# bryanboateng/animating-gaussian-splats

Measured on AMD Instinct MI355X. Metric: Msplats/sec fwd+bwd @1080p (1M gauss), higher is better.
Workload: dtype f32; 1 GPU; C3: 1000000 Gaussians, SH3, 1920x1080, 27-camera rig, 5 view(s)/GPU/step, fwd+bwd; gaussians=1000000, image=1920x1080, sh_degree=3, parallelism=camera-dp1, streams_per_gpu=3, submission=one host thread per stream, means2D=one fresh zero leaf per render (shared.py:38-41)

## Files before the change

animating-gaussian-splats_amd/csrc/gsr_api.hip:

```cpp
#include <hip/hip_runtime.h>

#include <atomic>
#include <cstdarg>
#include <cstdio>
#include <cstdlib>
#include <cmath>
#include <cstring>
#include <chrono>
#include <condition_variable>
#include <thread>
#include <map>
#include <memory>
#include <unordered_map>
#include <mutex>
#include <string>
#include <vector>

#include "../../include/gsr.h"
#include "gsr_common.h"
#include "gsr_internal.h"
#include "gsr_host.h"

using namespace gsr;

// ... 16 lines not shown
    hipEvent_t e = nullptr;
    if (hipEventCreateWithFlags(&e, hipEventDisableSystemFence) != hipSuccess) return nullptr;
    return e;
}

}

int gsr::fail(int code, const char *fmt, ...) {
    char buf[512];
    va_list ap;
    va_start(ap, fmt);
    vsnprintf(buf, sizeof(buf), fmt, ap);
    va_end(ap);
    g_err = buf;
    return code;
}

gsr::Phase::Phase(hipStream_t s_, const char *n, bool on) : s(s_), name(n) {
    if (!on || !g_prof_on) return;
    std::lock_guard<std::mutex> lk(g_prof_mu);
    if (!g_prof_sel.empty() && g_prof_sel.find("," + std::string(n) + ",") == std::string::npos) return;
    a = ev_get(); b = ev_get();
    if (a) (void)hipEventRecord(a, s);
}
gsr::Phase::~Phase() {
    if (!a || !b) return;
    (void)hipEventRecord(b, s);
    std::lock_guard<std::mutex> lk(g_prof_mu);
    g_prof.push_back({name, a, b});
}

gsr::HostPhase::HostPhase(const char *n) : name(n), t0(hclock::now()), on(g_prof_on) {}
gsr::HostPhase::~HostPhase() {
    if (!on) return;
    const double ms = std::chrono::duration<double, std::milli>(hclock::now() - t0).count();
    std::lock_guard<std::mutex> lk(g_prof_mu);
    g_host_ms[name] += ms;
    g_host_n[name] += 1;
}

namespace {

std::vector<hipEvent_t> g_gw_evpool;
struct GradEvent {
    hipEvent_t ev = nullptr;
    ~GradEvent() { if (ev) g_gw_evpool.push_back(ev); }
};
struct GradWriter { hipStream_t s = nullptr; std::shared_ptr<GradEvent> ev; };
std::mutex g_gw_mu;
std::unordered_map<const void *, GradWriter> g_gw;
constexpr size_t kGradPruneAt = 1024;

hipError_t no_launch() { return hipSuccess; }

template <typename Launch>
hipError_t ordered_grad_write(const void *const *keys, int nkeys, hipStream_t s, Launch launch) {
    std::lock_guard<std::mutex> lk(g_gw_mu);
    const GradEvent *waited[16];
    int nw = 0;
    for (int k = 0; k < nkeys; ++k) {
        if (!keys[k]) continue;
        auto it = g_gw.find(keys[k]);
        if (it == g_gw.end() || it->second.s == s) continue;
        const GradEvent *e = it->second.ev.get();
        bool seen = false;
        for (int j = 0; j < nw; ++j) seen = seen || waited[j] == e;
        if (seen) continue;
        const hipError_t r = hipStreamWaitEvent(s, e->ev, 0);
        if (r != hipSuccess) return r;
        if (nw < 16) waited[nw++] = e;
    }
    auto ev = std::make_shared<GradEvent>();
    hipError_t r = hipSuccess;
    if (!g_gw_evpool.empty()) { ev->ev = g_gw_evpool.back(); g_gw_evpool.pop_back(); }
    else r = hipEventCreateWithFlags(&ev->ev, hipEventDisableTiming);
    if (r != hipSuccess) { ev->ev = nullptr; return r; }
    r = launch();
    if (r != hipSuccess) return r;
    r = hipEventRecord(ev->ev, s);
    if (r != hipSuccess) return r;
    for (int k = 0; k < nkeys; ++k)
        if (keys[k]) g_gw[keys[k]] = GradWriter{s, ev};
    if (g_gw.size() > kGradPruneAt) {
        for (auto it = g_gw.begin(); it != g_gw.end();)
            it = hipEventQuery(it->second.ev->ev) == hipSuccess ? g_gw.erase(it) : std::next(it);
    }
    return hipSuccess;
}

struct HostWord { uint32_t *h = nullptr; uint32_t *d = nullptr; };
HostWord pinned_word() {
    thread_local HostWord w;
    if (!w.h) {
        uint32_t *h = nullptr;
        if (hipHostMalloc((void **)&h, 4 * kHostWords, hipHostMallocMapped | hipHostMallocCoherent) != hipSuccess) return w;
        uint32_t *d = nullptr;
        if (hipHostGetDevicePointer((void **)&d, h, 0) != hipSuccess) { (void)hipHostFree(h); return w; }
        w.h = h; w.d = d;
    }
    return w;
}

constexpr uint32_t kNoValue = 0xFFFFFFFFu;

int check_common(const gsr_camera *cam, const gsr_gaussians *g, bool need_opacity) {
    if (!cam || !g) return fail(GSR_ERR_ARG, "null camera or gaussians");
    if (g->P < 0) return fail(GSR_ERR_ARG, "P must be >= 0");
    if (cam->image_width <= 0 || cam->image_height <= 0)
        return fail(GSR_ERR_ARG, "image size must be positive (got %dx%d)", cam->image_width, cam->image_height);
    const int gx = div_up(cam->image_width, kTileW), gy = div_up(cam->image_height, kTileH);
    if (gx > 65535 || gy > 65535) return fail(GSR_ERR_UNSUPPORTED, "tile grid too large");
    if (g->activations & ~(GSR_ACT_SIGMOID_OPACITY | GSR_ACT_EXP_SCALES | GSR_ACT_NORMALIZE_ROTATIONS))
        return fail(GSR_ERR_ARG, "unknown activation bits 0x%x", g->activations);
    if (g->P == 0) return GSR_OK;
    if (!g->means3D || (need_opacity && !g->opacities))
        return fail(GSR_ERR_ARG, "means3D and opacities are required");
    if ((g->shs == nullptr) == (g->colors_precomp == nullptr))
        return fail(GSR_ERR_ARG, "Please provide excatly one of either SHs or precomputed colors!");
    const bool sr = g->scales && g->rotations;
    if (sr == (g->cov3D_precomp != nullptr) || ((g->scales != nullptr) != (g->rotations != nullptr)))
        return fail(GSR_ERR_ARG, "Please provide exactly one of either scale/rotation pair or precomputed 3D covariance!");
    if (g->shs && (g->sh_coeffs <= 0 || (g->sh_degree + 1) * (g->sh_degree + 1) > g->sh_coeffs || g->sh_degree > 3 || g->sh_degree < 0))
        return fail(GSR_ERR_ARG, "invalid SH configuration: degree %d with %d coefficients", g->sh_degree, g->sh_coeffs);
    if (!cam->viewmatrix || !cam->projmatrix || !cam->bg || (g->shs && !cam->campos))
        return fail(GSR_ERR_ARG, "camera matrices / bg / campos missing");
    return GSR_OK;
}

std::atomic<int> g_exact{[] {
    const char *e = getenv("GSR_EXACT_THRESHOLDS");
    return (e && e[0] == '0') ? 0 : 1;
}()};

void fill_common(ViewIn &v, const gsr_camera *cam, const gsr_gaussians *g) {
    memset(&v, 0, sizeof(v));
    v.P = g->P; v.D = g->sh_degree; v.M = g->shs ? g->sh_coeffs : 0;
    v.W = cam->image_width; v.H = cam->image_height;
    v.gx = div_up(v.W, kTileW); v.gy = div_up(v.H, kTileH);
    v.scale_modifier = g->scale_modifier;
    v.act = g->activations;
    v.tan_fovx = cam->tan_fovx; v.tan_fovy = cam->tan_fovy;
    v.focal_y = v.H / (2.0f * v.tan_fovy);
    v.focal_x = v.W / (2.0f * v.tan_fovx);
    v.means3D = g->means3D; v.scales = g->scales; v.rotations = g->rotations; v.opacities = g->opacities;
    v.shs = g->shs; v.colors_precomp = g->colors_precomp; v.cov3D_precomp = g->cov3D_precomp;
    v.viewmatrix = cam->viewmatrix; v.projmatrix = cam->projmatrix; v.campos = cam->campos; v.bg = cam->bg;
    const bool vz = !cam->viewmatrix_stride[0] && !cam->viewmatrix_stride[1];
    const bool pz = !cam->projmatrix_stride[0] && !cam->projmatrix_stride[1];
    v.cs.v0 = vz ? 4 : cam->viewmatrix_stride[0]; v.cs.v1 = vz ? 1 : cam->viewmatrix_stride[1];
    v.cs.p0 = pz ? 4 : cam->projmatrix_stride[0]; v.cs.p1 = pz ? 1 : cam->projmatrix_stride[1];
    v.cs.c0 = cam->campos_stride ? cam->campos_stride : 1;
}

template <typename A>
void carve_saved(A &a, char *geom, char *img) {
    const GeomLayout G(a.v.P);
    a.rec = (float4 *)(geom + G.rec); a.rect = (uint2 *)(geom + G.rect);
    a.goff = (uint32_t *)(geom + G.goff); a.clampm = (uint8_t *)(geom + G.clampm);
    const ImageLayout L(a.v.W, a.v.H, a.v.P);
    a.ranges = (uint2 *)(img + L.ranges); a.pix_end = (float4 *)(img + L.pix_end);
    a.n_contrib = (uint32_t *)(img + L.n_contrib); a.tile_maxc = (uint32_t *)(img + L.tile_maxc);
    a.tile_flag = (uint32_t *)(img + L.tile_flag); a.near_rec = (float4 *)(img + L.near_rec);
    a.seg_off = (uint32_t *)(img + L.seg_off); a.meta = (uint32_t *)(img + L.meta);
    a.items_ws = (uint32_t *)(img + L.items_ws);
}
void carve_forward(FwdArgs &a, char *geom, char *img) {
    carve_saved(a, geom, img);
    const GeomLayout G(a.v.P);
    a.depth = (float *)(geom + G.depth); a.tiles = (uint32_t *)(geom + G.tiles);
    const ImageLayout L(a.v.W, a.v.H, a.v.P);
    a.tile_order_f = (uint32_t *)(img + L.tile_order_f); a.sort_lists = (uint32_t *)(img + L.sort_lists);
    a.tile_count = (uint32_t *)(img + L.tile_count); a.tile_cursor = (uint32_t *)(img + L.tile_cursor);
    a.block_sums = (uint32_t *)(img + L.block_sums); a.block_off = (uint32_t *)(img + L.block_off);
    a.chunk_off = (uint32_t *)(img + L.chunk_off); a.scan_ws = (uint32_t *)(img + L.scan_ws);
    a.tile_rank = (uint32_t *)(img + L.tile_rank); a.tsat_list = (uint32_t *)(img + L.tsat_list);
}
template <typename A>
void carve_binning(A &a, char *bin, const BinningLayout &L) {
    a.point_list = (uint32_t *)(bin + L.point_list); a.slot_emit = (uint32_t *)(bin + L.slot_emit);
    a.seg_state = (float4 *)(bin + L.seg_state);
}

struct BinRegions {
    BinningLayout arrays;
    size_t items, tmp, total;
    BinRegions(int K, int P, int T, bool with_items, bool with_merge) : arrays(K, P) {
        items = arrays.total;
        tmp = items + (with_items ? bwd_items_bytes(K, T) : 0);
        total = tmp + (with_merge ? sizeof(uint4) * (size_t)K : 0);
    }
};

int enqueue_post_scan(FwdArgs a, char *bin, int layout, uint32_t n_mid, uint32_t n_vlong, uint32_t max_n,
                      bool prepare_backward, int T, hipStream_t s, const uint32_t *spec_ok, bool phases) {
    const BinRegions R(layout, a.v.P, T, prepare_backward, n_vlong != 0);
    carve_binning(a, bin, R.arrays);
    a.pairs = (uint4 *)(bin + R.arrays.pairs);
    a.spec_ok = spec_ok;
    uint4 *tmp = n_vlong ? (uint4 *)(bin + R.tmp) : nullptr;
    uint2 *items = (uint2 *)(bin + R.items);
    { Phase ph(s, "bin_emit", phases); HIP_TRY(launch_bin_emit(a, spec_ok ? 0 : layout, s)); }
    { Phase ph(s, "tile_sort", phases); HIP_TRY(launch_tile_sort(a, n_mid, n_vlong, max_n, tmp, s)); }
    { Phase ph(s, "render_fwd", phases); HIP_TRY(launch_render_fwd(a, s)); }
    if (prepare_backward) {
        Phase ph(s, "bwd_items", phases);
        HIP_TRY(launch_bwd_items_raw(layout, T, a.v.P, a.ranges, a.tile_maxc, a.tile_flag, items, a.items_ws, s, spec_ok));
    }
    return GSR_OK;
}

enum class KWait { published, stream_error, drained };
KWait wait_published(const uint32_t *word, hipStream_t s, hipError_t *err) {
    auto last = hclock::now();
    while (__atomic_load_n(word, __ATOMIC_ACQUIRE) == kNoValue) {
        __builtin_ia32_pause();
        if (hclock::now() - last > std::chrono::microseconds(500)) {
            last = hclock::now();
            const hipError_t q = hipStreamQuery(s);
            if (q == hipErrorNotReady) continue;
            *err = q;
            if (q != hipSuccess) return KWait::stream_error;
            return __atomic_load_n(word, __ATOMIC_ACQUIRE) == kNoValue ? KWait::drained : KWait::published;
        }
    }
    return KWait::published;
}

}

extern "C" {

const char *gsr_last_error(void) { return g_err.c_str(); }

int gsr_set_exact_thresholds(int on) { return g_exact.exchange(on ? 1 : 0); }
int gsr_abi_version(void) { return GSR_ABI_VERSION; }

size_t gsr_geom_bytes(int P) { return GeomLayout(P < 0 ? 0 : P).total; }
size_t gsr_image_bytes(int W, int H, int P) { return ImageLayout(W, H, P < 0 ? 0 : P).total; }
size_t gsr_binning_bytes(int K, int P) { return BinningLayout(K, P).total; }
size_t gsr_backward_items_bytes(int K, int W, int H) {
    return bwd_items_bytes(K < 0 ? 0 : K, div_up(W < 0 ? 0 : W, kTileW) * div_up(H < 0 ? 0 : H, kTileH));
}
size_t gsr_sums_bytes(int P) { return align256(sizeof(float) * (kPartial * (size_t)(P < 0 ? 0 : P) + 1)); }
size_t gsr_scratch_bytes(int K, int W, int H) {
    return ScratchLayout(K, div_up(W < 0 ? 0 : W, kTileW) * div_up(H < 0 ? 0 : H, kTileH)).total;
}

void *gsr_prealloc_alloc(void *ctx, int which, size_t bytes) {
    gsr_prealloc *pa = (gsr_prealloc *)ctx;
    if (!pa) return nullptr;
    if (which >= 0 && which < 5 && pa->ptr[which] && pa->bytes[which] >= bytes && !(pa->used & (1 << which))) {
        pa->used |= 1 << which;
        return pa->ptr[which];
    }
    return pa->fallback ? pa->fallback(pa->fallback_ctx, which, bytes) : nullptr;
}

int gsr_buffer_offsets(int P, int W, int H, int K, size_t *out, int max_out) {
    const GeomLayout g(P);
    const ImageLayout im(W, H, P);
    const BinningLayout b(K, P);
    const size_t v[16] = {g.depth, g.rec, g.rect, g.tiles, g.goff,
                          im.ranges, im.pix_end, im.n_contrib, im.tile_maxc,
                          b.pairs, b.point_list, b.slot_emit, im.seg_off, b.seg_state, im.tile_flag,
                          im.items_ws + sizeof(uint32_t) * kTSatCtr};
    int n = 0;
    for (; n < 16 && n < max_out; ++n) out[n] = v[n];
    return n;
}

}

namespace {
struct SpecKey {
    int dev, P, W, H;
    bool operator==(const SpecKey &o) const { return dev == o.dev && P == o.P && W == o.W && H == o.H; }
};
struct SpecKeyHash {
    size_t operator()(const SpecKey &k) const {
        return ((size_t)k.dev * 1000003u) ^ ((size_t)k.P * 2654435761u) ^ ((size_t)k.W << 20) ^ (size_t)k.H;
    }
};
constexpr int kSpecWindow = 16;
constexpr size_t kSpecKeys = 64;
struct SpecStat {
    uint32_t recent[kSpecWindow] = {};
    uint32_t recent_mid[kSpecWindow] = {};
    int n = 0;
    bool long_lists = false;
    uint64_t used = 0;
    uint32_t window_max() const {
        uint32_t m = 0;
        for (int k = 0; k < std::min(n, kSpecWindow); ++k) m = std::max(m, recent[k]);
        return m;
    }
};
std::mutex g_spec_mu;
std::unordered_map<SpecKey, SpecStat, SpecKeyHash> g_spec;
uint64_t g_spec_clock = 0;
int g_spec_hits = 0, g_spec_misses = 0, g_async_calls = 0;

uint32_t spec_capacity(const SpecKey &key, uint32_t *sort_blocks = nullptr) {
    std::lock_guard<std::mutex> lk(g_spec_mu);
    auto it = g_spec.find(key);
    if (it == g_spec.end() || it->second.long_lists) return 0;
    it->second.used = ++g_spec_clock;
// ... 102 lines not shown
    for (int k = 0; k < kAsyncSlots; ++k) {
        const int j = (g_slot_next + k) % kAsyncSlots;
        if (!g_slot_busy[j]) {
            g_slot_busy[j] = 1;
            g_slot_next = (j + 1) % kAsyncSlots;
            return j;
        }
    }
    return -1;
}

void async_classify(AsyncFwd &f) {
    const uint32_t *w = slot_h(f.slot);
    f.K = __atomic_load_n(w, __ATOMIC_ACQUIRE);
    const uint32_t n_vlong = __atomic_load_n(w + 2, __ATOMIC_ACQUIRE), n_mid = __atomic_load_n(w + 1, __ATOMIC_ACQUIRE);
    if (f.K <= f.cap && n_vlong == 0) {
        f.state = 1;
        f.layout = (int)f.cap;
        f.bin = f.spec_bin;
        spec_record(f.key, f.K, false, +1, n_mid);
    } else {
        f.state = 2;
        spec_record(f.key, f.K, n_vlong > 0, -1, n_mid);
    }
}

void async_reap(std::unordered_map<uint64_t, std::shared_ptr<AsyncFwd>>::iterator it) {
    AsyncFwd &f = *it->second;
    if (f.own) {
        int cur = 0;
        (void)hipGetDevice(&cur);
        if (cur != f.dev) (void)hipSetDevice(f.dev);
        (void)hipFreeAsync(f.own, f.s);
        if (cur != f.dev) (void)hipSetDevice(cur);
        f.own = nullptr;
    }
    if (f.ev_scan) g_as_evpool.push_back(f.ev_scan);
    f.ev_scan = nullptr;
    if (f.slot >= 0 && !f.err_reported && __atomic_load_n(slot_h(f.slot) + kGateErrWord, __ATOMIC_ACQUIRE) == f.seq)
        g_async_err = "an asynchronous forward's gate timed out (seq " + std::to_string(f.seq) + "), its outputs were not final";
    if (f.slot >= 0) g_slot_busy[f.slot] = 0;
    g_as.erase(it);
}

int async_redo(AsyncFwd &f, hipStream_t H) {
    (void)hipSetDevice(f.dev);
    if (!H) return fail(GSR_ERR_HIP, "asynchronous forward: no resolver stream on device %d", f.dev);
    HIP_TRY(hipStreamWaitEvent(H, f.ev_scan, 0));
    const uint32_t *w = slot_h(f.slot);
    const uint32_t K = f.K, n_mid = w[1], n_vlong = w[2], max_n = w[3];
    const size_t bytes = BinRegions((int)K, f.a.v.P, f.T, f.prep, n_vlong != 0).total;
    void *bin = nullptr;
    if (hipMallocAsync(&bin, bytes, H) != hipSuccess || !bin)
        return fail(GSR_ERR_ALLOC, "asynchronous forward: hipMallocAsync of %zu bytes failed", bytes);
    f.own = bin;
    const int rc = enqueue_post_scan(f.a, (char *)bin, (int)K, n_mid, n_vlong, max_n, f.prep, f.T, H, nullptr, false);
    if (rc) return rc;
    HIP_TRY(hipStreamSynchronize(H));
    f.bin = bin;
    f.layout = (int)K;
    return GSR_OK;
}

void resolver_main() {
    std::unique_lock<std::mutex> lk(g_as_mu);
    for (;;) {
        for (auto it = g_as.begin(); it != g_as.end();) {
            const AsyncFwd &f = *it->second;
            if (f.released && (f.state == 1 || f.state == 3 || f.state == -1)) async_reap(it++);
            else ++it;
        }
        std::shared_ptr<AsyncFwd> next;
        for (auto &kv : g_as)
            if ((kv.second->state == 0 || kv.second->state == 2) && (!next || kv.second->id < next->id)) next = kv.second;
        if (!next) {
            if (g_resolver_stop) break;
            g_as_wake.wait(lk);
            continue;
        }
        if (next->state == 0) {
            hipEvent_t ev = next->ev_scan;
            const int dev = next->dev;
            lk.unlock();
            (void)hipSetDevice(dev);
            const hipError_t r = hipEventSynchronize(ev);
            lk.lock();
            if (next->state == 0) {
                if (r != hipSuccess || __atomic_load_n(slot_h(next->slot), __ATOMIC_ACQUIRE) == kNoValue) {
                    next->state = -1;
                    next->err = r != hipSuccess ? std::string("stream error before num_rendered was published: ") +
                                                      hipGetErrorString(r)
                                                : std::string("num_rendered was not published");
                    __atomic_store_n(slot_h(next->slot) + kGateWord, next->seq, __ATOMIC_RELEASE);
                } else {
                    async_classify(*next);
                }
                g_as_done.notify_all();
            }
            continue;
        }
        hipStream_t H = g_resolver_streams.count(next->dev) ? g_resolver_streams[next->dev] : nullptr;
        lk.unlock();
        const int rc = async_redo(*next, H);
        const std::string msg = rc ? g_err : std::string();
        if (g_hold_next_redo_ms > 0) {
            std::this_thread::sleep_for(std::chrono::milliseconds(g_hold_next_redo_ms));
            g_hold_next_redo_ms = 0;
        }
        __atomic_store_n(slot_h(next->slot) + kGateWord, next->seq, __ATOMIC_RELEASE);
        lk.lock();
        next->state = rc ? -1 : 3;
        if (rc) { next->err = msg; g_async_err = "asynchronous forward redo failed: " + msg; }
        g_as_done.notify_all();
    }
}

}

extern "C" size_t gsr_spec_binning_bytes(int P, int W, int H, int prepare_backward) {
    if (P <= 0 || W <= 0 || H <= 0) return 0;
    int dev = 0;
    (void)hipGetDevice(&dev);
    const uint32_t cap = spec_capacity(SpecKey{dev, P, W, H});
    if (!cap) return 0;
    return BinRegions((int)cap, P, div_up(W, kTileW) * div_up(H, kTileH), prepare_backward != 0, false).total;
}

namespace {
int forward_impl(const gsr_camera *cam, const gsr_gaussians *g, gsr_alloc_fn alloc, void *alloc_ctx,
                 float *out_color, float *out_depth, int *out_radii, gsr_forward_info *info, int mode,
                 void *stream) {
    HostPhase host_total("host_forward");
    int rc = check_common(cam, g, true);
    if (rc) return rc;
    if (!alloc || !out_color || !out_depth || !info || (g->P > 0 && !out_radii))
        return fail(GSR_ERR_ARG, "gsr_forward: missing output or allocator");
    {
        std::lock_guard<std::mutex> lk(g_as_mu);
        if (!g_async_err.empty()) return fail(GSR_ERR_HIP, "%s", g_async_err.c_str());
    }
    hipStream_t s = (hipStream_t)stream;
    FwdArgs a;
    memset(&a, 0, sizeof(a));
    fill_common(a.v, cam, g);
    const int P = a.v.P, T = a.v.gx * a.v.gy;
    const bool prep = g->prepare_backward != 0;
    a.exact = g_exact.load(std::memory_order_relaxed);
    a.radii = out_radii; a.out_color = out_color; a.out_depth = out_depth;
    char *geom = (char *)alloc(alloc_ctx, GSR_BUF_GEOM, GeomLayout(P).total);
    char *img = (char *)alloc(alloc_ctx, GSR_BUF_IMAGE, ImageLayout(a.v.W, a.v.H, P).total);
    if (!geom || !img) return fail(GSR_ERR_ALLOC, "allocation callback failed (geom/image)");
    carve_forward(a, geom, img);
    *info = gsr_forward_info{};
    if (P == 0) {
        const size_t npix = (size_t)a.v.W * a.v.H;
        HIP_TRY(launch_zero(out_color, 3 * npix, s));
        HIP_TRY(launch_zero(out_depth, npix, s));
        char *bin = (char *)alloc(alloc_ctx, GSR_BUF_BINNING, BinningLayout(0, 0).total);
        if (!bin) return fail(GSR_ERR_ALLOC, "allocation callback failed (binning)");
        return GSR_OK;
    }
    int dev = 0;
    (void)hipGetDevice(&dev);
    const SpecKey key{dev, P, a.v.W, a.v.H};
    uint32_t sort_blocks = kSpecSortBlocks;
    const uint32_t cap = mode ? spec_capacity(key, &sort_blocks) : 0u;
    a.spec_cap = cap;
    a.spec_sort_blocks = sort_blocks;
    std::shared_ptr<AsyncFwd> af;
    uint32_t *words_h = nullptr, *words_d = nullptr;
    if (mode == 2 && cap) {
        std::lock_guard<std::mutex> lk(g_as_mu);
        if (async_init() && resolver_stream(dev)) {
            const int slot = slot_acquire();
            if (slot >= 0) {
                af = std::make_shared<AsyncFwd>();
                af->slot = slot; af->seq = ++g_as_seq;
                words_h = slot_h(slot); words_d = slot_d(slot);
                __atomic_store_n(words_h + kGateErrWord, 0u, __ATOMIC_RELAXED);
            }
        }
    }
    struct SlotGuard {
        std::shared_ptr<AsyncFwd> *f;
        ~SlotGuard() {
            if (!*f || (*f)->id) return;
            std::lock_guard<std::mutex> lk(g_as_mu);
            g_slot_busy[(*f)->slot] = 0;
            if ((*f)->ev_scan) g_as_evpool.push_back((*f)->ev_scan);
        }
    } slot_guard{&af};
    if (!af) {
        HostWord hw = pinned_word();
        if (!hw.h) return fail(GSR_ERR_HIP, "hipHostMalloc(mapped) failed");
        words_h = hw.h; words_d = hw.d;
    }
    __atomic_store_n(words_h, kNoValue, __ATOMIC_SEQ_CST);
    { Phase ph(s, "preprocess"); HIP_TRY(launch_preprocess(a, s)); }
    { Phase ph(s, "bin_count"); HIP_TRY(launch_bin_count(a, s)); }
    { Phase ph(s, "bin_scan"); HIP_TRY(launch_bin_scan(a, words_d, s)); }
    if (af) {
        {
            std::lock_guard<std::mutex> lk(g_as_mu);
            if (!g_as_evpool.empty()) { af->ev_scan = g_as_evpool.back(); g_as_evpool.pop_back(); }
        }
        if (!af->ev_scan) HIP_TRY(hipEventCreateWithFlags(&af->ev_scan, hipEventDisableTiming | hipEventBlockingSync));
        HIP_TRY(hipEventRecord(af->ev_scan, s));
    }
    char *spec_bin = nullptr;
    if (cap) {
        spec_bin = (char *)alloc(alloc_ctx, GSR_BUF_BINNING, BinRegions((int)cap, P, T, prep, false).total);
        if (!spec_bin) return fail(GSR_ERR_ALLOC, "allocation callback failed (binning, capacity %u)", cap);
        FwdArgs sa = a;
        if (af) {
            sa.gate = words_d + kGateWord; sa.gate_seq = af->seq;
            sa.gate_err = words_d + kGateErrWord; sa.gate_timeout = g_gate_timeout;
        }
        rc = enqueue_post_scan(sa, spec_bin, (int)cap, 0, 0, 0, prep, T, s, a.meta + 1, true);
        if (rc) return rc;
    }
    if (af) {
        std::lock_guard<std::mutex> lk(g_as_mu);
        af->id = g_as_next_id++;
        af->dev = dev; af->s = s; af->cap = cap; af->T = T; af->key = key;
        af->prep = prep; af->a = a; af->spec_bin = spec_bin;
        g_as[af->id] = af;
        info->num_rendered = -1; info->binning_layout = (int)cap;
        info->speculated = 1; info->pending = af->id;
        { std::lock_guard<std::mutex> lk2(g_spec_mu); ++g_async_calls; }
        g_as_wake.notify_one();
        return GSR_OK;
    }
    {
        HostPhase hp("host_wait_K");
        hipError_t q = hipSuccess;
        const KWait w = wait_published(words_h, s, &q);
        if (w == KWait::stream_error) return fail(GSR_ERR_HIP, "stream error while waiting for num_rendered: %s", hipGetErrorString(q));
        if (w == KWait::drained) return fail(GSR_ERR_HIP, "num_rendered was not published");
    }
    const uint32_t K = __atomic_load_n(words_h, __ATOMIC_ACQUIRE);
    if (K > 0x7FFFFFFFu) return fail(GSR_ERR_UNSUPPORTED, "num_rendered overflow");
    info->num_rendered = (int)K;
    const uint32_t n_mid = __atomic_load_n(words_h + 1, __ATOMIC_ACQUIRE);
    const uint32_t n_vlong = __atomic_load_n(words_h + 2, __ATOMIC_ACQUIRE);
    const uint32_t max_n = __atomic_load_n(words_h + 3, __ATOMIC_ACQUIRE);
    if (cap && K <= cap && n_vlong == 0) {
        info->binning_layout = (int)cap;
        info->speculated = 1;
        spec_record(key, K, false, +1, n_mid);
        return GSR_OK;
    }
    char *bin = (char *)alloc(alloc_ctx, GSR_BUF_BINNING, BinRegions((int)K, P, T, prep, n_vlong != 0).total);
    if (!bin) return fail(GSR_ERR_ALLOC, "allocation callback failed (binning, K=%u)", K);
    rc = enqueue_post_scan(a, bin, (int)K, n_mid, n_vlong, max_n, prep, T, s, nullptr, true);
    if (rc) return rc;
    info->binning_layout = (int)K;
    spec_record(key, K, n_vlong > 0, cap ? -1 : 0, n_mid);
    return GSR_OK;
}
}

extern "C" {

int gsr_forward(const gsr_camera *cam, const gsr_gaussians *g, gsr_alloc_fn alloc, void *alloc_ctx,
                float *out_color, float *out_depth, int *out_radii, int *out_num_rendered,
                void *stream) {
    if (!out_num_rendered) return fail(GSR_ERR_ARG, "gsr_forward: missing output or allocator");
    *out_num_rendered = 0;
    gsr_forward_info info;
    const int rc = forward_impl(cam, g, alloc, alloc_ctx, out_color, out_depth, out_radii, &info, 0, stream);
    *out_num_rendered = info.num_rendered;
    return rc;
}

int gsr_forward_info_call(const gsr_camera *cam, const gsr_gaussians *g, gsr_alloc_fn alloc, void *alloc_ctx,
                          float *out_color, float *out_depth, int *out_radii, int speculate, gsr_forward_info *info,
                          void *stream) {
    if (!info) return fail(GSR_ERR_ARG, "gsr_forward_info_call: null info");
    return forward_impl(cam, g, alloc, alloc_ctx, out_color, out_depth, out_radii, info, speculate ? 1 : 0, stream);
}

int gsr_forward_async(const gsr_camera *cam, const gsr_gaussians *g, gsr_alloc_fn alloc, void *alloc_ctx,
                      float *out_color, float *out_depth, int *out_radii, gsr_forward_info *info, void *stream) {
    if (!info) return fail(GSR_ERR_ARG, "gsr_forward_async: null info");
    return forward_impl(cam, g, alloc, alloc_ctx, out_color, out_depth, out_radii, info, 2, stream);
}

int gsr_forward_resolve(unsigned long long handle, gsr_forward_resolution *out) {
    if (!out) return fail(GSR_ERR_ARG, "gsr_forward_resolve: null output");
    HostPhase hp("host_wait_K");
    std::unique_lock<std::mutex> lk(g_as_mu);
    auto it = g_as.find(handle);
    if (it == g_as.end()) return fail(GSR_ERR_ARG, "gsr_forward_resolve: unknown or released forward %llu", handle);
    std::shared_ptr<AsyncFwd> f = it->second;
    while (f->state == 0 || f->state == 2) {
        if (f->state == 0) {
            if (__atomic_load_n(slot_h(f->slot), __ATOMIC_ACQUIRE) != kNoValue) {
                async_classify(*f);
                if (f->state == 2) g_as_wake.notify_one();
                continue;
            }
            lk.unlock();
            hipError_t q = hipSuccess;
            const KWait w = wait_published(slot_h(f->slot), f->s, &q);
            lk.lock();
            if (w != KWait::published && f->state == 0) {
                f->state = -1;
                f->err = w == KWait::drained ? std::string("num_rendered was not published")
                                             : std::string("stream error: ") + hipGetErrorString(q);
                __atomic_store_n(slot_h(f->slot) + kGateWord, f->seq, __ATOMIC_RELEASE);
            }
            continue;
        }
        g_as_done.wait(lk);
    }
    if (f->state < 0) return fail(GSR_ERR_HIP, "asynchronous forward %llu failed: %s", handle, f->err.c_str());
    if (__atomic_load_n(slot_h(f->slot) + kGateErrWord, __ATOMIC_ACQUIRE) == f->seq) {
        f->err_reported = true;
        return fail(GSR_ERR_HIP, "asynchronous forward %llu: its gate timed out before the redo opened it; the outputs "
                    "the caller used after the forward were not final", handle);
    }
    out->num_rendered = (int)f->K;
    out->binning_layout = f->layout;
    out->binning = f->bin;
    out->redone = f->state == 3;
    return GSR_OK;
}

int gsr_forward_query(unsigned long long handle) {
    std::lock_guard<std::mutex> lk(g_as_mu);
    auto it = g_as.find(handle);
    if (it == g_as.end()) return -1;
    AsyncFwd &f = *it->second;
    if (f.state == 0 && __atomic_load_n(slot_h(f.slot), __ATOMIC_ACQUIRE) != kNoValue) {
        async_classify(f);
        if (f.state == 2) g_as_wake.notify_one();
    }
    return (f.state == 1 || f.state == 3 || f.state == -1) ? 1 : 0;
}

int gsr_forward_release(unsigned long long handle) {
    std::lock_guard<std::mutex> lk(g_as_mu);
    auto it = g_as.find(handle);
    if (it == g_as.end()) return GSR_OK;
    it->second->released = true;
    const int st = it->second->state;
    if (st == 1 || st == 3 || st == -1) async_reap(it);
    else g_as_wake.notify_one();
    return GSR_OK;
}

int gsr_async_shutdown(void) {
    std::thread t;
    {
        std::lock_guard<std::mutex> lk(g_as_mu);
        if (!g_resolver_started) return GSR_OK;
        g_resolver_stop = true;
        g_resolver_started = false;
        t = std::move(g_resolver);
    }
    g_as_wake.notify_all();
    if (t.joinable()) t.join();
    return GSR_OK;
}

int gsr_async_stats(int *calls, int *pending) {
    {
        std::lock_guard<std::mutex> lk(g_spec_mu);
        if (calls) *calls = g_async_calls;
    }
    std::lock_guard<std::mutex> lk(g_as_mu);
    if (pending) *pending = (int)g_as.size();
    return GSR_OK;
}

int gsr_spec_stats(int *hits, int *misses, int reset) {
    std::lock_guard<std::mutex> lk(g_spec_mu);
    if (hits) *hits = g_spec_hits;
    if (misses) *misses = g_spec_misses;
    if (reset) { g_spec.clear(); g_spec_hits = g_spec_misses = g_async_calls = 0; }
    return GSR_OK;
}

int gsr_debug_async_fault(int hold_next_redo_ms, int gate_timeout_ms, int clear) {
    std::lock_guard<std::mutex> lk(g_as_mu);
    g_hold_next_redo_ms = hold_next_redo_ms > 0 ? hold_next_redo_ms : 0;
    g_gate_timeout = gate_timeout_ms > 0 ? (uint64_t)gate_timeout_ms * 100000ull : kGateTimeoutTicks;
    if (clear) g_async_err.clear();
    return GSR_OK;
}

int gsr_spec_keys(void) {
    std::lock_guard<std::mutex> lk(g_spec_mu);
    return (int)g_spec.size();
}

}


namespace {
int backward_render(const gsr_camera *cam, const gsr_gaussians *g, const int *radii, int num_rendered,
                    const void *geom, const void *binning, const void *image, const float *dL_dcolor,
                    gsr_alloc_fn alloc, void *alloc_ctx, hipStream_t s, BwdArgs &a, bool sums = false) {
    if (!geom || !binning || !image || !dL_dcolor || !radii || !alloc)
        return fail(GSR_ERR_ARG, "gsr_backward: missing saved buffers / dL_dcolor / allocator");
    const bool spec = num_rendered < 0;
    if (spec && g->binning_layout <= 0) return fail(GSR_ERR_ARG, "num_rendered < 0 without the forward's binning_layout");
    memset(&a, 0, sizeof(a));
    fill_common(a.v, cam, g);
    const int P = a.v.P, T = a.v.gx * a.v.gy;
    const int layout = g->binning_layout > 0 ? g->binning_layout : num_rendered;
    if (layout < num_rendered) return fail(GSR_ERR_ARG, "binning_layout %d < num_rendered %d", layout, num_rendered);
    if (spec) num_rendered = layout;
    a.K = num_rendered;
    a.radii = radii;
// ... 180 lines not shown
```

animating-gaussian-splats_amd/csrc/gsr_bind.cpp:

```cpp
#include <torch/extension.h>
#include <ATen/hip/HIPContext.h>
#include <c10/hip/HIPCachingAllocator.h>
#include <c10/hip/HIPGuard.h>

#include <map>
#include <stdexcept>
#include <string>
#include <vector>

#include "../../include/gsr.h"

namespace py = pybind11;

namespace {

struct Fns {
    decltype(&gsr_forward_info_call) forward_info_call = nullptr;
    decltype(&gsr_forward_async) forward_async = nullptr;
    decltype(&gsr_backward_render) backward_render = nullptr;
    decltype(&gsr_backward_gaussians) backward_gaussians = nullptr;
    decltype(&gsr_backward) backward = nullptr;
    decltype(&gsr_prealloc_alloc) prealloc_alloc = nullptr;
    decltype(&gsr_spec_binning_bytes) spec_binning_bytes = nullptr;
    decltype(&gsr_geom_bytes) geom_bytes = nullptr;
    decltype(&gsr_image_bytes) image_bytes = nullptr;
    decltype(&gsr_scratch_bytes) scratch_bytes = nullptr;
    decltype(&gsr_sums_bytes) sums_bytes = nullptr;
    decltype(&gsr_last_error) last_error = nullptr;
} F;

template <typename T>
void take(const std::map<std::string, int64_t> &a, const char *name, T &dst) {
    auto it = a.find(name);
    if (it == a.end() || !it->second) throw std::runtime_error(std::string("gsr_bind: missing ") + name);
    dst = reinterpret_cast<T>(it->second);
}

void set_functions(const std::map<std::string, int64_t> &a) {
    take(a, "gsr_forward_info_call", F.forward_info_call);
    take(a, "gsr_forward_async", F.forward_async);
    take(a, "gsr_backward_render", F.backward_render);
    take(a, "gsr_backward_gaussians", F.backward_gaussians);
    take(a, "gsr_backward", F.backward);
    take(a, "gsr_prealloc_alloc", F.prealloc_alloc);
    take(a, "gsr_spec_binning_bytes", F.spec_binning_bytes);
    take(a, "gsr_geom_bytes", F.geom_bytes);
    take(a, "gsr_image_bytes", F.image_bytes);
    take(a, "gsr_scratch_bytes", F.scratch_bytes);
    take(a, "gsr_sums_bytes", F.sums_bytes);
    take(a, "gsr_last_error", F.last_error);
}

void check(int rc) {
    if (rc != 0) throw std::runtime_error("libgsr error " + std::to_string(rc) + ": " + F.last_error());
}

bool present(const at::Tensor &t) { return t.defined() && t.numel() > 0; }

const char *torch_name(at::ScalarType t) {
    switch (t) {
        case at::kDouble: return "torch.float64";
        case at::kHalf: return "torch.float16";
        case at::kBFloat16: return "torch.bfloat16";
        case at::kInt: return "torch.int32";
        case at::kLong: return "torch.int64";
        case at::kShort: return "torch.int16";
        case at::kByte: return "torch.uint8";
        case at::kChar: return "torch.int8";
        case at::kBool: return "torch.bool";
        default: return c10::toString(t);
    }
}

const float *fptr(const at::Tensor &t, std::vector<at::Tensor> &keep) {
    if (!present(t)) return nullptr;
    if (!t.is_cuda()) throw std::runtime_error("diff_gaussian_rasterization: tensors must be on the GPU (no CPU path)");
    at::Tensor c = t.contiguous();
    if (c.scalar_type() != at::kFloat)
        throw std::runtime_error(std::string("diff_gaussian_rasterization: expected float32, got ") +
                                 torch_name(c.scalar_type()));
    keep.push_back(c);
    return c.data_ptr<float>();
}

const float *mat16(const at::Tensor &m0, int stride[2], std::vector<at::Tensor> &keep) {
    if (m0.numel() != 16) throw std::runtime_error("viewmatrix/projmatrix must hold 16 floats");
    at::Tensor m = m0.scalar_type() == at::kFloat ? m0 : m0.to(at::kFloat);
    const auto sz = m.sizes();
    const bool plain = (m.dim() == 2 && sz[0] == 4 && sz[1] == 4) || (m.dim() == 3 && sz[0] == 1 && sz[1] == 4 && sz[2] == 4);
    if (!plain) m = m.reshape({4, 4});
    stride[0] = (int)m.stride(-2);
    stride[1] = (int)m.stride(-1);
    if (!m.is_cuda()) throw std::runtime_error("diff_gaussian_rasterization: tensors must be on the GPU (no CPU path)");
    keep.push_back(m);
    return m.data_ptr<float>();
}

gsr_camera camera(const at::Tensor &vm, const at::Tensor &pm, double tanfovx, double tanfovy, int H, int W,
                  const at::Tensor &campos, const at::Tensor &bg, bool prefiltered, std::vector<at::Tensor> &keep) {
    gsr_camera c;
    memset(&c, 0, sizeof(c));
    c.image_width = W;
    c.image_height = H;
    c.tan_fovx = (float)tanfovx;
    c.tan_fovy = (float)tanfovy;
    c.viewmatrix = mat16(vm, c.viewmatrix_stride, keep);
    c.projmatrix = mat16(pm, c.projmatrix_stride, keep);
    at::Tensor b = (bg.scalar_type() == at::kFloat && bg.is_contiguous()) ? bg : bg.contiguous().to(at::kFloat);
    c.bg = fptr(b, keep);
    if (present(campos)) {
        at::Tensor cp = (campos.scalar_type() == at::kFloat && campos.dim() == 1) ? campos : campos.reshape({-1}).to(at::kFloat);
        if (!cp.is_cuda()) throw std::runtime_error("diff_gaussian_rasterization: tensors must be on the GPU (no CPU path)");
        keep.push_back(cp);
        c.campos = cp.data_ptr<float>();
        c.campos_stride = (int)cp.stride(0);
    }
    c.prefiltered = prefiltered ? 1 : 0;
    return c;
}

gsr_gaussians gaussians(const at::Tensor &means3D, const at::Tensor &sh, int degree, const at::Tensor &colors,
                        const at::Tensor &opacity, const at::Tensor &scales, const at::Tensor &rotations,
                        double scale_modifier, const at::Tensor &cov3D, int activations, bool prep, int layout,
                        std::vector<at::Tensor> &keep) {
    if (means3D.dim() != 2 || means3D.size(1) != 3) throw std::runtime_error("means3D must have dimensions (num_points, 3)");
    gsr_gaussians g;
    memset(&g, 0, sizeof(g));
    g.P = (int)means3D.size(0);
    g.sh_degree = degree;
    g.sh_coeffs = present(sh) ? (int)sh.size(1) : 0;
    g.scale_modifier = (float)scale_modifier;
    g.means3D = fptr(means3D, keep);
    g.shs = fptr(sh, keep);
    g.colors_precomp = fptr(colors, keep);
    g.opacities = fptr(opacity, keep);
    g.scales = fptr(scales, keep);
    g.rotations = fptr(rotations, keep);
    g.cov3D_precomp = fptr(cov3D, keep);
    g.activations = activations;
    g.prepare_backward = prep ? 1 : 0;
    g.binning_layout = layout;
    return g;
}

struct PreAlloc {
    gsr_prealloc pa;
    at::Device dev;
    struct Given { at::Tensor base; int64_t off, bytes; };
    std::map<int, Given> given;
    std::map<int, at::Tensor> fallback;
    explicit PreAlloc(at::Device d) : dev(d) { memset(&pa, 0, sizeof(pa)); }
    void group(std::initializer_list<std::pair<int, size_t>> g, bool on) {
        if (!on) return;
        int64_t total = 0;
        std::vector<std::tuple<int, int64_t, int64_t>> offs;
        for (auto &e : g) {
            offs.emplace_back(e.first, total, (int64_t)e.second);
            total += ((int64_t)e.second + 255) & ~(int64_t)255;
        }
        if (total == 0) return;
        at::Tensor buf = at::empty({total}, at::TensorOptions().dtype(at::kByte).device(dev));
        char *base = (char *)buf.data_ptr();
        for (auto &[w, o, n] : offs)
            if (n > 0) {
                given[w] = Given{buf, o, n};
                pa.ptr[w] = base + o;
                pa.bytes[w] = (size_t)n;
            }
    }
    static void *fallback_fn(void *ctx, int which, size_t bytes) {
        auto *self = static_cast<PreAlloc *>(ctx);
        try {
            at::Tensor t = at::empty({(int64_t)std::max<size_t>(bytes, 1)}, at::TensorOptions().dtype(at::kByte).device(self->dev));
            self->fallback[which] = t;
            return t.data_ptr();
        } catch (...) {
            return nullptr;
        }
    }
    void arm() {
        pa.fallback = &PreAlloc::fallback_fn;
        pa.fallback_ctx = this;
    }
    py::tuple result() const {
        py::list taken, fb;
        for (auto &[w, g] : given)
            if ((pa.used >> w) & 1) taken.append(py::make_tuple(w, g.base, g.off, g.bytes));
        for (auto &[w, t] : fallback) fb.append(py::make_tuple(w, t));
        return py::make_tuple(taken, fb);
    }
};

void *raw_stream(at::Device dev) { return (void *)c10::hip::getCurrentHIPStream(dev.index()).stream(); }

py::tuple forward(const at::Tensor &bg, const at::Tensor &means3D, const at::Tensor &colors, const at::Tensor &opacity,
                  const at::Tensor &scales, const at::Tensor &rotations, double scale_modifier, const at::Tensor &cov3D,
                  const at::Tensor &viewmatrix, const at::Tensor &projmatrix, double tanfovx, double tanfovy, int H, int W,
                  const at::Tensor &sh, int degree, const at::Tensor &campos, bool prefiltered, int activations,
                  bool prepare_backward, bool speculate, bool nonblocking, bool prealloc) {
    std::vector<at::Tensor> keep;
    gsr_gaussians g = gaussians(means3D, sh, degree, colors, opacity, scales, rotations, scale_modifier, cov3D,
                                activations, prepare_backward, 0, keep);
    gsr_camera cam = camera(viewmatrix, projmatrix, tanfovx, tanfovy, H, W, campos, bg, prefiltered, keep);
    const at::Device dev = means3D.device();
    const int P = g.P;
    auto f32 = at::TensorOptions().dtype(at::kFloat).device(dev);
    at::Tensor color = at::empty({3, H, W}, f32), depth = at::empty({1, H, W}, f32);
    at::Tensor radii = at::empty({P}, at::TensorOptions().dtype(at::kInt).device(dev));
    c10::hip::HIPGuard guard(dev.index());
    const size_t spec = (speculate || nonblocking) && P ? F.spec_binning_bytes(P, W, H, prepare_backward ? 1 : 0) : 0;
    PreAlloc pa(dev);
    pa.group({{GSR_BUF_GEOM, F.geom_bytes(P)}, {GSR_BUF_IMAGE, F.image_bytes(W, H, P)}}, prealloc);
    pa.group({{GSR_BUF_BINNING, spec}}, prealloc);
    pa.arm();
    gsr_forward_info fi;
    memset(&fi, 0, sizeof(fi));
    void *s = raw_stream(dev);
    int rc;
    {
        py::gil_scoped_release nogil;
        rc = nonblocking ? F.forward_async(&cam, &g, F.prealloc_alloc, &pa.pa, color.data_ptr<float>(),
                                           depth.data_ptr<float>(), P ? radii.data_ptr<int>() : nullptr, &fi, s)
                         : F.forward_info_call(&cam, &g, F.prealloc_alloc, &pa.pa, color.data_ptr<float>(),
                                               depth.data_ptr<float>(), P ? radii.data_ptr<int>() : nullptr,
                                               speculate ? 1 : 0, &fi, s);
    }
    check(rc);
    return py::make_tuple(fi.num_rendered, fi.binning_layout, fi.speculated, (unsigned long long)fi.pending,
                          (int64_t)(intptr_t)fi.aux_stream, color, radii, depth, pa.result());
}

py::tuple backward_render(const at::Tensor &bg, const at::Tensor &means3D, const at::Tensor &radii,
                          const at::Tensor &colors, const at::Tensor &scales, const at::Tensor &rotations,
                          double scale_modifier, const at::Tensor &cov3D, const at::Tensor &viewmatrix,
                          const at::Tensor &projmatrix, double tanfovx, double tanfovy, const at::Tensor &dL_dcolor,
                          const at::Tensor &sh, int degree, const at::Tensor &campos, int64_t geom, int R,
                          int64_t binning, int64_t image, int activations, bool prepare_backward, int binning_layout,
                          bool prealloc) {
    std::vector<at::Tensor> keep;
    gsr_gaussians g = gaussians(means3D, sh, degree, colors, at::Tensor(), scales, rotations, scale_modifier, cov3D,
                                activations, prepare_backward, binning_layout, keep);
    const int H = (int)dL_dcolor.size(-2), W = (int)dL_dcolor.size(-1);
    gsr_camera cam = camera(viewmatrix, projmatrix, tanfovx, tanfovy, H, W, campos, bg, false, keep);
    const at::Device dev = means3D.device();
    if (g.P == 0)
        return py::make_tuple(at::empty({1}, at::TensorOptions().dtype(at::kByte).device(dev)),
                              py::make_tuple(py::list(), py::list()));
    at::Tensor dpix = dL_dcolor.contiguous().to(at::kFloat);
    c10::hip::HIPGuard guard(dev.index());
    PreAlloc pa(dev);
    pa.group({{GSR_BUF_SCRATCH, F.scratch_bytes(R >= 0 ? R : binning_layout, W, H)}}, prealloc);
    pa.group({{GSR_BUF_SUMS, F.sums_bytes(g.P)}}, prealloc);
    pa.arm();
    void *s = raw_stream(dev);
    int rc;
    {
        py::gil_scoped_release nogil;
        rc = F.backward_render(&cam, &g, radii.data_ptr<int>(), R, (const void *)geom, (const void *)binning,
                               (const void *)image, dpix.data_ptr<float>(), F.prealloc_alloc, &pa.pa, s);
    }
    check(rc);
    at::Tensor sums;
    if (auto it = pa.fallback.find(GSR_BUF_SUMS); it != pa.fallback.end()) sums = it->second;
    else {
        auto &gv = pa.given.at(GSR_BUF_SUMS);
        sums = gv.base.narrow(0, gv.off, gv.bytes);
    }
    return py::make_tuple(sums, pa.result());
}

void fill_grads(gsr_grads &gr, const std::vector<c10::optional<at::Tensor>> &outs, int acc_bits) {
    memset(&gr, 0, sizeof(gr));
    float **slot[8] = {&gr.dL_dmeans2D, &gr.dL_dcolors, &gr.dL_dopacity, &gr.dL_dmeans3D,
                       &gr.dL_dcov3D, &gr.dL_dsh, &gr.dL_dscales, &gr.dL_drotations};
    for (int k = 0; k < 8 && k < (int)outs.size(); ++k)
        if (outs[k].has_value() && present(*outs[k])) *slot[k] = outs[k]->data_ptr<float>();
    gr.accumulate = acc_bits;
}

void backward(const at::Tensor &bg, const at::Tensor &means3D, const at::Tensor &radii, const at::Tensor &colors,
              const at::Tensor &scales, const at::Tensor &rotations, double scale_modifier, const at::Tensor &cov3D,
              const at::Tensor &viewmatrix, const at::Tensor &projmatrix, double tanfovx, double tanfovy,
              const at::Tensor &dL_dcolor, const at::Tensor &sh, int degree, const at::Tensor &campos, int64_t geom,
              int R, int64_t binning, int64_t image, int activations, bool prepare_backward, int binning_layout,
              const std::vector<c10::optional<at::Tensor>> &outs, int acc_bits, bool prealloc) {
    std::vector<at::Tensor> keep;
    gsr_gaussians g = gaussians(means3D, sh, degree, colors, at::Tensor(), scales, rotations, scale_modifier, cov3D,
                                activations, prepare_backward, binning_layout, keep);
    const int H = (int)dL_dcolor.size(-2), W = (int)dL_dcolor.size(-1);
    gsr_camera cam = camera(viewmatrix, projmatrix, tanfovx, tanfovy, H, W, campos, bg, false, keep);
    if (g.P == 0) return;
    const at::Device dev = means3D.device();
    at::Tensor dpix = dL_dcolor.contiguous().to(at::kFloat);
    c10::hip::HIPGuard guard(dev.index());
    PreAlloc pa(dev);
    pa.group({{GSR_BUF_SCRATCH, F.scratch_bytes(R, W, H)}}, prealloc);
    pa.arm();
    gsr_grads gr;
    fill_grads(gr, outs, acc_bits);
    void *s = raw_stream(dev);
    int rc;
    {
        py::gil_scoped_release nogil;
        rc = F.backward(&cam, &g, radii.data_ptr<int>(), R, (const void *)geom, (const void *)binning,
                        (const void *)image, dpix.data_ptr<float>(), nullptr, F.prealloc_alloc, &pa.pa, &gr, s);
    }
    check(rc);
}

void record(const at::Tensor &t, const c10::hip::HIPStream &s) {
    if (t.defined() && t.is_cuda() && t.storage().data_ptr().get())
        c10::hip::HIPCachingAllocator::recordStream(t.storage().data_ptr(), s);
}

std::string dev_str(const at::Device &d) { return d.str(); }

void backward_views(const py::list &views, const at::Tensor &means3D, const at::Tensor &colors,
                    const at::Tensor &scales, const at::Tensor &rotations, double scale_modifier, const at::Tensor &cov3D,
                    const at::Tensor &sh, int degree, int activations, const std::vector<c10::optional<at::Tensor>> &outs,
                    int acc_bits) {
    std::vector<at::Tensor> keep;
    gsr_gaussians g = gaussians(means3D, sh, degree, colors, at::Tensor(), scales, rotations, scale_modifier, cov3D,
                                activations, false, 0, keep);
    const int P = g.P;
    const int nv = (int)views.size();
    if (P == 0 || nv == 0) return;
    const at::Device dev = means3D.device();
    c10::hip::HIPGuard guard(dev.index());
    const c10::hip::HIPStream cs = c10::hip::getCurrentHIPStream(dev.index());
    std::vector<gsr_camera> cams(nv);
    std::vector<gsr_view_grad> vg(nv);
    for (int k = 0; k < nv; ++k) {
        const py::dict v = views[k].cast<py::dict>();
        cams[k] = camera(v["viewmatrix"].cast<at::Tensor>(), v["projmatrix"].cast<at::Tensor>(),
                         v["tanfovx"].cast<double>(), v["tanfovy"].cast<double>(), v["image_height"].cast<int>(),
                         v["image_width"].cast<int>(),
                         v["campos"].is_none() ? at::Tensor() : v["campos"].cast<at::Tensor>(),
                         v["bg"].cast<at::Tensor>(), false, keep);
        float *m2p = nullptr;
        if (v.contains("means2D_grad") && !v["means2D_grad"].is_none()) {
            const at::Tensor m2 = v["means2D_grad"].cast<at::Tensor>();
            if (m2.dim() != 2 || m2.size(0) != P || m2.size(1) != 3 || m2.scalar_type() != at::kFloat ||
                !m2.is_contiguous() || m2.device() != dev)
                throw std::runtime_error("views[" + std::to_string(k) + "]['means2D_grad']: expected a contiguous float32 (" +
                                         std::to_string(P) + ", 3) tensor on " + dev_str(dev));
            record(m2, cs);
            m2p = m2.data_ptr<float>();
        }
        const at::Tensor radii = v["radii"].cast<at::Tensor>(), scratch = v["scratch"].cast<at::Tensor>();
        record(radii, cs);
        record(scratch, cs);
        if (v.contains("keep"))
            for (auto h : v["keep"]) record(h.cast<at::Tensor>(), cs);
        const py::object gb = v["geomBuffer"];
        const void *geom;
        if (py::isinstance<py::int_>(gb)) geom = (const void *)gb.cast<int64_t>();
        else {
            const at::Tensor gt = gb.cast<at::Tensor>();
            record(gt, cs);
            geom = gt.data_ptr();
        }
        vg[k].cam = &cams[k];
        vg[k].radii = radii.data_ptr<int>();
        vg[k].geom = geom;
        vg[k].scratch = scratch.data_ptr();
        vg[k].num_rendered = v["num_rendered"].cast<int>();
        vg[k].dL_dmeans2D = m2p;
        vg[k].accumulate_means2D = (v.contains("accumulate_means2D") && v["accumulate_means2D"].cast<bool>()) ? 1 : 0;
    }
    gsr_grads gr;
    fill_grads(gr, outs, acc_bits);
    void *s = (void *)cs.stream();
    int rc;
    {
        py::gil_scoped_release nogil;
        rc = F.backward_gaussians(nv, vg.data(), &g, &gr, s);
    }
    check(rc);
}

}

PYBIND11_MODULE(TORCH_EXTENSION_NAME, m) {
    m.doc() = "native argument marshalling for diff_gaussian_rasterization._C (libgsr's C ABI)";
    m.def("set_functions", &set_functions);
    m.def("abi_version", []() { return (int)GSR_ABI_VERSION; });
    m.def("forward", &forward);
    m.def("backward_render", &backward_render);
    m.def("backward_views", &backward_views);
    m.def("backward", &backward);
}
```

animating-gaussian-splats_amd/csrc/gsr_forward.hip:

```cpp
#include "gsr_common.h"
#include "gsr_internal.h"

#include <algorithm>
#include <type_traits>

namespace gsr {

#ifdef GSR_TRACE
__device__ uint64_t *g_trace_fwd;
#ifdef GSR_TRACE
__device__ inline uint64_t trace_fwd_work(uint64_t batches, uint64_t walk, uint64_t evals) {
    return (batches << 40) | ((walk < 0xFFFFFull ? walk : 0xFFFFFull) << 20) | (evals < 0xFFFFFull ? evals : 0xFFFFFull);
}
#endif
__device__ uint64_t *g_trace_emit;
#define GSR_EMIT_STAMP(k)                                                                        \
    do {                                                                                         \
        if (g_trace_emit && threadIdx.x == 0)                                                    \
            g_trace_emit[4 * blockIdx.x + (k)] = __builtin_amdgcn_s_memrealtime();               \
    } while (0)
#else
#define GSR_EMIT_STAMP(k) do {} while (0)
#endif

template <int MC>
__global__ __launch_bounds__(256) void k_preprocess(
    int P, int D, int M, const float *__restrict__ means3D, const float *__restrict__ scales,
    float scale_modifier, const float *__restrict__ rotations, const float *__restrict__ opacities,
    const float *__restrict__ shs, const float *__restrict__ colors_precomp,
    const float *__restrict__ cov3D_precomp, const float *__restrict__ viewmatrix,
    const float *__restrict__ projmatrix, const float *__restrict__ campos, int W, int H,
    float tan_fovx, float tan_fovy, float focal_x, float focal_y, int gx, int gy,
    int *__restrict__ radii, float *__restrict__ depth_out, float4 *__restrict__ rec_out,
    uint2 *__restrict__ rect_out, uint32_t *__restrict__ tiles_out, int act, CamStrides cs,
    uint32_t *__restrict__ tile_count, int T, uint8_t *__restrict__ clamp_out) {
    extern __shared__ __attribute__((aligned(16))) float s_sh[];
    constexpr int RL = 3 * MC, RS = sh_row_stride(MC);
    const int i0 = blockIdx.x * kShBlock;
    const int i = i0 + threadIdx.x;
    for (int t = i; t < T; t += (int)gridDim.x * kShBlock) tile_count[t] = 0;
    const int ic = min(i, P - 1);
    const float3 p = make_float3(means3D[3 * ic], means3D[3 * ic + 1], means3D[3 * ic + 2]);
    float3 s_in = make_float3(0.f, 0.f, 0.f);
    float4 q_in = make_float4(0.f, 0.f, 0.f, 0.f);
    if (!cov3D_precomp) {
        s_in = make_float3(scales[3 * ic], scales[3 * ic + 1], scales[3 * ic + 2]);
        q_in = make_float4(rotations[4 * ic], rotations[4 * ic + 1], rotations[4 * ic + 2], rotations[4 * ic + 3]);
    }
    const float o_in = opacities[ic];
    if constexpr (MC > 0) {
        sh_rows_to_lds<MC>(shs + (size_t)i0 * RL, min(kShBlock, P - i0), s_sh);
        __syncthreads();
    }
    if (i >= P) return;
    float vm[16], pm[16];
    load_mat16(viewmatrix, cs.v0, cs.v1, vm);
    load_mat16(projmatrix, cs.p0, cs.p1, pm);
    radii[i] = 0;
    tiles_out[i] = 0;
    rect_out[i] = make_uint2(0, 0);
    const float4 ph = xform4x4(p, pm);
    const float3 pv = xform4x3(p, vm);
    if (pv.z <= 0.2f) return;
    const float pw = 1.0f / (ph.w + 0.0000001f);
    const float ppx = ph.x * pw, ppy = ph.y * pw;
    float c3[6];
    if (cov3D_precomp) {
#pragma unroll
        for (int k = 0; k < 6; ++k) c3[k] = cov3D_precomp[6 * i + k];
    } else {
        float3 s = s_in;
        float4 q = q_in;
        if (act & GSR_ACT_EXP_SCALES) s = act_exp3(s);
        if (act & GSR_ACT_NORMALIZE_ROTATIONS) q = act_normalize(q, quat_norm(q));
        cov3d_from_scale_rot(s, scale_modifier, q, c3);
    }
    const float3 cv = cov2d(p, focal_x, focal_y, tan_fovx, tan_fovy, c3, vm);
    const float det = cv.x * cv.z - cv.y * cv.y;
    if (det == 0.0f) return;
    const float det_inv = 1.f / det;
    const float mid = 0.5f * (cv.x + cv.z);
    const float l1 = mid + sqrtf(fmaxf(0.1f, mid * mid - det));
    const float l2 = mid - sqrtf(fmaxf(0.1f, mid * mid - det));
    const float my_radius = ceilf(3.f * sqrtf(fmaxf(l1, l2)));
    const float pix_x = ndc2pix(ppx, W), pix_y = ndc2pix(ppy, H);
    int x0, y0, x1, y1;
    get_rect(pix_x, pix_y, (int)my_radius, gx, gy, x0, y0, x1, y1);
    if ((x1 - x0) * (y1 - y0) == 0) return;
    float3 rgb;
    if (colors_precomp) {
        rgb = make_float3(colors_precomp[3 * i], colors_precomp[3 * i + 1], colors_precomp[3 * i + 2]);
    } else {
        bool cl[3];
        const float3 cp = load_campos(campos, cs.c0);
        if (MC > 0) rgb = sh_to_rgb(D, p, cp, s_sh + threadIdx.x * RS, cl);
        else rgb = sh_to_rgb(D, p, cp, shs + (size_t)i * M * 3, cl);
        clamp_out[i] = clamp_bits(cl);
    }
    radii[i] = (int)my_radius;
    depth_out[i] = pv.z;
    const float o = (act & GSR_ACT_SIGMOID_OPACITY) ? act_sigmoid(o_in) : o_in;
    const float ca = cv.z * det_inv, cb = -cv.y * det_inv, cc = cv.x * det_inv;
    const float tau2 = o >= 1.0f / 255.0f ? 2.f * log2f(255.f * o) : -1.f;
    float4 *r = rec_out + (size_t)kRecF4 * i;
    r[0] = make_float4(pix_x, pix_y, -0.5f * GSR_LOG2E * ca, -GSR_LOG2E * cb);
    r[1] = make_float4(-0.5f * GSR_LOG2E * cc, o, pv.z, tau2);
    r[2] = make_float4(rgb.x, rgb.y, rgb.z, pv.z);
    r[3] = make_float4(ca, cb, cc, 0.f);
    rect_out[i] = pack_rect(x0, y0, x1, y1);
    tiles_out[i] = (uint32_t)((y1 - y0) * (x1 - x0));
}

template <bool USE_LDS>
__global__ __launch_bounds__(kBinThreads) void k_bin_count(int P, int CH, int T, int gx,
                                                   const uint2 *__restrict__ rects,
                                                   const uint32_t *__restrict__ tiles,
                                                   uint32_t *__restrict__ tile_count,
                                                   uint32_t *__restrict__ block_sums,
                                                   uint32_t *__restrict__ chunk_off,
                                                   uint32_t *__restrict__ items_ws,
                                                   uint32_t *__restrict__ scan_ws) {
    extern __shared__ __attribute__((aligned(16))) uint32_t s_hist[];
    __shared__ uint32_t s_red[16];
    const int b = blockIdx.x;
    if (b == 0) {
        for (int i = threadIdx.x; i < kItemsWsWords; i += blockDim.x) items_ws[i] = 0;
        if (scan_ws)
            for (int i = threadIdx.x; i < kScanWsWords; i += blockDim.x) scan_ws[i] = 0;
    }
    const int g0 = b * CH, g1 = min(P, g0 + CH);
    if (USE_LDS) {
        for (int t = threadIdx.x; t < T; t += blockDim.x) s_hist[t] = 0;
        __syncthreads();
    }
    uint32_t my_sum = 0;
    for (int g = g0 + threadIdx.x; g < g1; g += blockDim.x) {
        const uint32_t n = tiles[g];
        if (n == 0) continue;
        my_sum += n;
        const uint2 r = rects[g];
        const int x0 = r.x & 0xFFFF, y0 = r.x >> 16, x1 = r.y & 0xFFFF, y1 = r.y >> 16;
        for (int y = y0; y < y1; ++y)
            for (int x = x0; x < x1; ++x) {
                if (USE_LDS) atomicAdd(&s_hist[y * gx + x], 1u);
                else atomicAdd(&tile_count[y * gx + x], 1u);
            }
    }
    uint32_t tot;
    block_excl_scan_u32(my_sum, s_red, &tot);
    if (threadIdx.x == 0) block_sums[b] = tot;
    if (USE_LDS) {
        __syncthreads();
        uint32_t *row = chunk_off + (size_t)b * T;
        for (int t = threadIdx.x; t < T; t += blockDim.x) row[t] = s_hist[t];
    }
}

constexpr int kColW = 32, kColG = 32, kColR = 16;
static_assert(kColG * kColR >= 512, "BinGrid makes at most 512 chunks");
static_assert(kColW <= 64 && kMaxLdsTiles <= kColW * kScanBlocksMax, "look-back: one wave per block, <= kScanBlocksMax blocks");
__global__ __launch_bounds__(kColW * kColG) void k_bin_colscan(
    int T, int NB, uint32_t *__restrict__ chunk_off, uint32_t *__restrict__ tile_count, uint2 *__restrict__ ranges,
    uint32_t *__restrict__ tile_cursor, uint32_t *__restrict__ seg_off, uint32_t *__restrict__ sort_lists,
    uint32_t *__restrict__ tile_rank, uint32_t *__restrict__ ws, const uint32_t *__restrict__ block_sums,
    uint32_t *__restrict__ block_off, uint32_t *__restrict__ meta, uint32_t *host_words, uint32_t cap, int ks) {
    __shared__ uint32_t s_part[kColG][kColW + 1];
    __shared__ uint32_t s_tile[kColW];
    __shared__ uint32_t s_blk, s_last;
    __shared__ uint32_t s_red[16];
    __shared__ uint32_t s_lpt[kOrderBuckets];
    uint64_t *look = reinterpret_cast<uint64_t *>(ws);
    uint32_t *ctr = ws + 2 * kScanBlocksMax, *lpt = ctr + kScanCtr;
    if (threadIdx.x == 0) s_blk = blockIdx.x;
    for (int i = threadIdx.x; i < kOrderBuckets; i += blockDim.x) s_lpt[i] = 0;
    __syncthreads();
    const int blk = (int)s_blk;
    const int col = threadIdx.x % kColW, grp = threadIdx.x / kColW;
    const int t = blk * kColW + col;
    const int R = div_up(NB, kColG);
    const int r0 = min(NB, grp * R), r1 = min(NB, r0 + R);
    uint32_t *p = chunk_off + t;
    uint32_t v[kColR];
    uint32_t sum = 0;
#pragma unroll
    for (int k = 0; k < kColR; ++k) {
        v[k] = (t < T && r0 + k < r1) ? p[(size_t)(r0 + k) * T] : 0u;
        sum += v[k];
    }
    s_part[grp][col] = sum;
    __syncthreads();
    uint32_t pre = 0, tot = 0;
#pragma unroll
    for (int k = 0; k < kColG; ++k) {
        const uint32_t c = s_part[k][col];
        pre += k < grp ? c : 0u;
        tot += c;
    }
    if (t < T) {
        if (grp == 0) tile_count[t] = tot;
#pragma unroll
        for (int k = 0; k < kColR; ++k) {
            if (r0 + k < r1) p[(size_t)(r0 + k) * T] = pre;
            pre += v[k];
        }
    }
    if (grp == 0) s_tile[col] = t < T ? tot : 0u;
    __syncthreads();
    if (threadIdx.x < 64) {
        const int lane = threadIdx.x;
        const uint32_t cnt = lane < kColW ? s_tile[lane] : 0u, sb = seg_bounds(cnt, ks);
        const uint32_t ic = wave_incl_scan_u32(cnt), is = wave_incl_scan_u32(sb);
        const uint32_t agg_c = (uint32_t)__builtin_amdgcn_readlane((int)ic, 63);
        const uint32_t agg_s = (uint32_t)__builtin_amdgcn_readlane((int)is, 63);
        if (lane == 0)
            __hip_atomic_store(&look[blk], (blk == 0 ? kScanInc : kScanAgg) | ((uint64_t)agg_s << 32) | agg_c,
                               __ATOMIC_RELAXED, __HIP_MEMORY_SCOPE_AGENT);
        uint32_t ex_c = 0, ex_s = 0;
        for (int base = blk - 1; base >= 0; base -= 64) {
            const int j = base - lane;
            uint64_t w;
            uint64_t inc, zero;
            for (;;) {
                w = j >= 0 ? __hip_atomic_load(&look[j], __ATOMIC_RELAXED, __HIP_MEMORY_SCOPE_AGENT) : kScanInc;
                inc = __ballot((w >> 62) == 2u);
                zero = __ballot((w >> 62) == 0u);
                const uint64_t upto = inc ? (~0ull >> (63 - __builtin_ctzll(inc))) : ~0ull;
                if (!(zero & upto)) break;
                __builtin_amdgcn_s_sleep(1);
            }
            const int first = inc ? __builtin_ctzll(inc) : 64;
            const uint32_t wc = lane <= first ? (uint32_t)w : 0u;
            const uint32_t ws_ = lane <= first ? (uint32_t)(w >> 32) & 0x3FFFFFFFu : 0u;
            ex_c += (uint32_t)__builtin_amdgcn_readlane((int)wave_incl_scan_u32(wc), 63);
            ex_s += (uint32_t)__builtin_amdgcn_readlane((int)wave_incl_scan_u32(ws_), 63);
            if (inc) break;
        }
        if (lane == 0 && blk > 0)
            __hip_atomic_store(&look[blk], kScanInc | ((uint64_t)(ex_s + agg_s) << 32) | (ex_c + agg_c),
                               __ATOMIC_RELAXED, __HIP_MEMORY_SCOPE_AGENT);
        const int tl = blk * kColW + lane;
        const uint32_t bkt = lpt_bucket(cnt);
        const bool mine = lane < kColW && tl < T;
        const uint32_t local = mine ? atomicAdd(&s_lpt[bkt], 1u) : 0u;
        wave_lds_sync();
        if (mine && local == 0) s_lpt[bkt] = atomicAdd(&lpt[bkt], s_lpt[bkt]);
        wave_lds_sync();
        if (mine) tile_rank[tl] = s_lpt[bkt] + local;
        if (mine) {
            const uint32_t ex = ex_c + ic - cnt;
            ranges[tl] = cnt ? make_uint2(ex, ex + cnt) : make_uint2(0, 0);
            tile_cursor[tl] = ex;
            seg_off[tl] = ex_s + is - sb;
            if (cnt > (uint32_t)kSortCap) {
                sort_lists[T - 1 - atomicAdd(&ctr[3], 1u)] = (uint32_t)tl;
                atomicMax(&ctr[4], cnt);
            } else if (cnt > (uint32_t)kFwdSortCap) {
                sort_lists[atomicAdd(&ctr[2], 1u)] = (uint32_t)tl;
            }
        }
    }
    drain_vmem();
    __builtin_amdgcn_fence(__ATOMIC_RELEASE, "workgroup");
    __syncthreads();
// ... 674 lines not shown
                            near_rec[(size_t)kNearCap * tile + slot] =
                                make_float4(__uint_as_float(((uint32_t)idx << 8) | pix_key), x.power, x.G, x.alpha);
                    }
                }
                take(e, ok, b, c, j);
            }
        };
#ifdef GSR_TRACE
        const uint64_t tr_w0 = __builtin_amdgcn_s_memrealtime();
        tr_batches += 1;
        tr_entries += (uint64_t)__builtin_popcountll(m);
#endif
        if (clamp) walk(std::true_type{});
        else walk(std::false_type{});
#ifdef GSR_TRACE
        tr_walk += __builtin_amdgcn_s_memrealtime() - tr_w0;
#endif
        if (((live >> wv) & 1u) && !__ballot(thr < kThrDone) && lane == 0) atomicAnd(&s_live, ~(1u << wv));
    }
    if (EXACT && inside && Tt < kTSat * (1.0f + t_window(last))) {
        const uint32_t slot = atomicAdd(tsat_n, 1u);
        if (slot < tsat_cap) {
            uint4 *r = reinterpret_cast<uint4 *>(tsat_list) + 2 * (size_t)slot;
            r[0] = make_uint4((uint32_t)(py * W + px), rg.x, (uint32_t)n, last);
            r[1] = make_uint4(__float_as_uint(C01.x), __float_as_uint(C01.y), __float_as_uint(C2D.x), __float_as_uint(C2D.y));
        }
    }
    if (inside) {
        const int pid = py * W + px;
        pix_end[pid] = make_float4(C01.x, C01.y, C2D.x, Tt);
        n_contrib[pid] = last;
        out_color[pid] = C01.x + Tt * bg[0];
        out_color[H * W + pid] = C01.y + Tt * bg[1];
        out_color[2 * H * W + pid] = C2D.x + Tt * bg[2];
        out_depth[pid] = C2D.y;
    }
    uint32_t mx = last;
#pragma unroll
    for (int d = 16; d > 0; d >>= 1) mx = max(mx, (uint32_t)__shfl_xor((int)mx, d, 64));
    __syncthreads();
    if (threadIdx.x < 4) s_u.st.q[threadIdx.x] = 0;
    __syncthreads();
    if ((lane & 31) == 0) atomicMax(&s_u.st.q[2 * (wv >> 1) + (lane >> 5)], mx);
    lds_barrier();
    if (threadIdx.x < 4) tile_maxc[4 * tile + threadIdx.x] = s_u.st.q[threadIdx.x];
    if (threadIdx.x == 0) tile_flag[tile] = EXACT ? s_near : 0u;
#ifdef GSR_TRACE
    trace_wave(g_trace_fwd, 4 * blockIdx.x + wv, t_start, trace_fwd_work(tr_batches, tr_walk, tr_entries));
    if (g_trace_fwd && lane == 0)
        g_trace_fwd[4 * (4 * blockIdx.x + wv) + 2] |= (tr_sorted - t_start) << 40;
#endif
}

#ifndef GSR_TSAT_BLOCKS
#define GSR_TSAT_BLOCKS 4096
#endif
constexpr int kTSatBlocks = GSR_TSAT_BLOCKS;
__global__ __launch_bounds__(kTSatThreads) void k_render_tsat(
    int W, int H, const uint32_t *__restrict__ point_list, const float4 *__restrict__ rec,
    const float *__restrict__ bg, float *__restrict__ out_color, float *__restrict__ out_depth,
    float4 *__restrict__ pix_end, uint32_t *__restrict__ n_contrib, const uint32_t *__restrict__ seg_off,
    float4 *__restrict__ seg_state, const uint32_t *__restrict__ tsat_n, const uint32_t *__restrict__ tsat_list,
    uint32_t tsat_cap, const uint32_t *__restrict__ spec_ok, int ks, int gx) {
    constexpr int NT = kTSatThreads;
    __shared__ float4 s_buf[(3 * NT + 4 + 3) / 4];
    __shared__ uint32_t s_rc[4];
    if (spec_ok && *spec_ok == 0u) return;
    const uint32_t cnt = min(*tsat_n, tsat_cap);
#ifdef GSR_TRACE
    const uint64_t tr_b = __builtin_amdgcn_s_memrealtime();
#endif
    float *s_q = reinterpret_cast<float *>(s_buf), *s_a = s_q + NT + 4;
    uint32_t *s_pos = reinterpret_cast<uint32_t *>(s_a + NT);
    for (uint32_t i = blockIdx.x; i < cnt; i += gridDim.x) {
#ifdef GSR_TRACE
        const uint64_t tr_i = __builtin_amdgcn_s_memrealtime();
#endif
        const uint4 *rp = reinterpret_cast<const uint4 *>(tsat_list) + 2 * (size_t)i;
        const uint4 r0 = rp[0], r1 = rp[1];
        const uint32_t pid = r0.x, start = r0.y;
        const int n = (int)r0.z, nf = (int)r0.w;
        const int px = (int)(pid % (uint32_t)W), py = (int)(pid / (uint32_t)W);
        const int tile = (py / kTileH) * gx + px / kTileW;
        float T = 1.0f;
        uint32_t nex = 0;
        float4 E = make_float4(0.f, 0.f, 0.f, 0.f);
        tsat_chain(nf, point_list + start, (float)px, (float)py, rec, s_rc, s_q, s_a, s_pos, T, nex, E);
#ifdef GSR_TRACE
        const uint64_t tr_c = __builtin_amdgcn_s_memrealtime();
#endif
        if (threadIdx.x == 0) {
            s_rc[0] = nex;
            s_rc[1] = __float_as_uint(T);
            s_q[0] = E.x; s_q[1] = E.y; s_q[2] = E.z; s_q[3] = E.w;
        }
        __syncthreads();
        tsat_store(px, py, W, H, n,
                   make_float4(__uint_as_float(r1.x), __uint_as_float(r1.y), __uint_as_float(r1.z), 0.f),
                   __uint_as_float(r1.w), __uint_as_float(s_rc[1]), s_rc[0],
                   make_float4(s_q[0], s_q[1], s_q[2], s_q[3]), bg, out_color, out_depth, pix_end, n_contrib,
                   seg_off[tile], seg_state, ks, nullptr);
        __syncthreads();
#ifdef GSR_TRACE
        const uint32_t ntile = (uint32_t)gx * (uint32_t)((H + kTileH - 1) / kTileH);
        if (g_trace_fwd && threadIdx.x == 0 && i < 4u * ntile) {
            uint64_t *o = g_trace_fwd + 16 * (size_t)ntile + 4 * (size_t)i;
            o[0] = tr_i;
            o[1] = __builtin_amdgcn_s_memrealtime();
            o[2] = (uint64_t)(uint32_t)nf | ((uint64_t)(uint32_t)n << 32);
            o[3] = (tr_c - tr_i) | ((tr_i - tr_b) << 32);
        }
#endif
    }
}

__global__ void k_zero_f32(float *p, size_t n) {
    const size_t i = (size_t)blockIdx.x * blockDim.x + threadIdx.x;
    if (i < n) p[i] = 0.f;
}

__global__ void k_mark_visible(int P, const float *__restrict__ means3D,
                               const float *__restrict__ viewmatrix, uint8_t *__restrict__ present) {
    const int i = blockIdx.x * blockDim.x + threadIdx.x;
    if (i >= P) return;
    float vm[16];
#pragma unroll
    for (int k = 0; k < 16; ++k) vm[k] = viewmatrix[k];
    const float3 pv = xform4x3(make_float3(means3D[3 * i], means3D[3 * i + 1], means3D[3 * i + 2]), vm);
    present[i] = !(pv.z <= 0.2f);
}

template <int MC>
static void preprocess_mc(const FwdArgs &a, hipStream_t s) {
    k_preprocess<MC><<<div_up(a.v.P, kShBlock), kShBlock, sizeof(float) * kShBlock * (MC ? sh_row_stride(MC) : 0), s>>>(
        a.v.P, a.v.D, a.v.M, a.v.means3D, a.v.scales, a.v.scale_modifier, a.v.rotations, a.v.opacities, a.v.shs,
        a.v.colors_precomp, a.v.cov3D_precomp, a.v.viewmatrix, a.v.projmatrix, a.v.campos, a.v.W, a.v.H, a.v.tan_fovx,
        a.v.tan_fovy, a.v.focal_x, a.v.focal_y, a.v.gx, a.v.gy, a.radii, a.depth, a.rec, a.rect, a.tiles, a.v.act, a.v.cs,
        a.tile_count, a.v.gx * a.v.gy, a.clampm);
}

hipError_t launch_preprocess(const FwdArgs &a, hipStream_t s) {
    if (a.v.P == 0) return hipSuccess;
    const int mc = a.v.shs ? a.v.M : 0;
    switch (mc) {
        case 16: preprocess_mc<16>(a, s); break;
        case 9: preprocess_mc<9>(a, s); break;
        case 4: preprocess_mc<4>(a, s); break;
        case 1: preprocess_mc<1>(a, s); break;
        default: preprocess_mc<0>(a, s); break;
    }
    return hipGetLastError();
}

hipError_t launch_bin_count(const FwdArgs &a, hipStream_t s) {
    const BinGrid bg(a.v.P);
    const int T = a.v.gx * a.v.gy;
    if (bg.NB == 0) return hipSuccess;
    if (T <= kMaxLdsTiles)
        k_bin_count<true><<<bg.NB, kBinThreads, sizeof(uint32_t) * T, s>>>(a.v.P, bg.CH, T, a.v.gx, a.rect, a.tiles, a.tile_count, a.block_sums, a.chunk_off, a.items_ws, a.scan_ws);
    else
        k_bin_count<false><<<bg.NB, kBinThreads, 0, s>>>(a.v.P, bg.CH, T, a.v.gx, a.rect, a.tiles, a.tile_count, a.block_sums, nullptr, a.items_ws, nullptr);
    return hipGetLastError();
}

hipError_t launch_bin_scan(const FwdArgs &a, uint32_t *host_words, hipStream_t s) {
    const BinGrid bg(a.v.P);
    const int T = a.v.gx * a.v.gy;
    if (T <= kMaxLdsTiles && bg.NB > 0)
        k_bin_colscan<<<div_up(T, kColW), kColW * kColG, 0, s>>>(T, bg.NB, a.chunk_off, a.tile_count, a.ranges,
                                                                a.tile_cursor, a.seg_off, a.sort_lists, a.tile_rank,
                                                                a.scan_ws, a.block_sums, a.block_off, a.meta,
                                                                host_words, a.spec_cap, seg_log2(a.v.P));
    else
        k_bin_scan<<<1, 1024, 0, s>>>(T, bg.NB, a.tile_count, a.ranges, a.tile_cursor,
                                      a.block_sums, a.block_off, a.meta, host_words, a.tile_order_f,
                                      a.sort_lists, a.seg_off, a.spec_cap, seg_log2(a.v.P));
    return hipGetLastError();
}

hipError_t launch_bin_emit(const FwdArgs &a, int K, hipStream_t s) {
    const BinGrid bg(a.v.P);
    const int T = a.v.gx * a.v.gy;
    if (bg.NB == 0) return hipSuccess;
    if (T <= kMaxLdsTiles)
        k_bin_emit<true><<<bg.NB, kBinThreads, sizeof(uint32_t) * T, s>>>(a.v.P, bg.CH, T, a.v.gx, a.rect, a.tiles, a.depth, a.block_off, a.tile_cursor, a.goff, a.pairs, (uint32_t)K, a.chunk_off, a.spec_ok,
                                                                           a.tile_count, a.tile_rank, a.scan_ws + 2 * kScanBlocksMax + kScanCtr, a.tile_order_f);
    else
        k_bin_emit<false><<<bg.NB, kBinThreads, 0, s>>>(a.v.P, bg.CH, T, a.v.gx, a.rect, a.tiles, a.depth, a.block_off, a.tile_cursor, a.goff, a.pairs, (uint32_t)K, a.chunk_off, a.spec_ok,
                                                        nullptr, nullptr, nullptr, nullptr);
    return hipGetLastError();
}

hipError_t launch_tile_sort(const FwdArgs &a, uint32_t n_mid, uint32_t n_vlong, uint32_t max_n, uint4 *tmp,
                            hipStream_t s) {
    const int T = a.v.gx * a.v.gy;
    if (a.spec_ok) {
        const int nb = a.spec_sort_blocks ? (int)a.spec_sort_blocks : kSpecSortBlocks;
        k_tile_sort<<<std::min(T, nb), 512, 0, s>>>(a.v.gx, a.sort_lists, a.ranges, a.pairs, a.point_list,
                                                                 a.slot_emit, 0u, a.spec_ok);
        return hipGetLastError();
    }
    if (n_mid) k_tile_sort<<<n_mid, 512, 0, s>>>(a.v.gx, a.sort_lists, a.ranges, a.pairs, a.point_list, a.slot_emit,
                                                 n_mid, nullptr);
    if (n_vlong) {
        const dim3 grid((unsigned)div_up((int)max_n, kSortCap), n_vlong);
        k_chunk_sort<<<grid, 512, 0, s>>>(T, a.sort_lists, a.ranges, a.pairs);
        const uint4 *src = a.pairs;
        uint4 *dst = tmp;
        for (uint32_t L = kSortCap; L < max_n; L *= 2) {
            const int final_pass = 2 * (size_t)L >= max_n;
            k_merge_pass<<<grid, 512, 0, s>>>(T, a.sort_lists, a.ranges, L, src, dst, final_pass, a.point_list,
                                              a.slot_emit);
            const uint4 *t = dst;
            dst = const_cast<uint4 *>(src);
            src = t;
        }
    }
    return hipGetLastError();
}

hipError_t launch_render_fwd(const FwdArgs &a, hipStream_t s) {
    const int T = a.v.gx * a.v.gy;
    auto k = a.exact ? k_render_fwd<true> : k_render_fwd<false>;
    k<<<T, 256, 0, s>>>(a.v.W, a.v.H, a.v.gx, T, a.tile_order_f, a.ranges, a.pairs,
                        a.point_list, a.slot_emit, a.rec, a.v.bg, a.out_color, a.out_depth, a.pix_end, a.n_contrib,
                        a.tile_maxc, a.seg_off, a.seg_state, a.spec_ok, seg_log2(a.v.P), a.gate, a.gate_seq,
                        a.gate_err, a.gate_timeout, a.tile_flag, a.near_rec, a.items_ws + kTSatCtr, a.tsat_list,
                        tsat_capacity(a.v.W * a.v.H));
    if (a.exact)
        k_render_tsat<<<kTSatBlocks, kTSatThreads, 0, s>>>(a.v.W, a.v.H, a.point_list, a.rec, a.v.bg, a.out_color, a.out_depth,
                                                 a.pix_end, a.n_contrib, a.seg_off, a.seg_state, a.items_ws + kTSatCtr,
                                                 a.tsat_list, tsat_capacity(a.v.W * a.v.H), a.spec_ok, seg_log2(a.v.P),
                                                 a.v.gx);
    return hipGetLastError();
}

hipError_t launch_zero(float *p, size_t n, hipStream_t s) {
    if (n == 0) return hipSuccess;
    k_zero_f32<<<(unsigned)((n + 255) / 256), 256, 0, s>>>(p, n);
    return hipGetLastError();
}

hipError_t launch_mark_visible(int P, const float *means3D, const float *viewmatrix, uint8_t *present,
                               hipStream_t s) {
    if (P == 0) return hipSuccess;
    k_mark_visible<<<div_up(P, 256), 256, 0, s>>>(P, means3D, viewmatrix, present);
    return hipGetLastError();
}

}

#ifdef GSR_TRACE
extern "C" int gsr_debug_trace_fwd(void *buf) {
    return hipMemcpyToSymbol(HIP_SYMBOL(gsr::g_trace_fwd), &buf, sizeof(buf)) == hipSuccess ? 0 : 2;
}
extern "C" int gsr_debug_trace_emit(void *buf) {
    return hipMemcpyToSymbol(HIP_SYMBOL(gsr::g_trace_emit), &buf, sizeof(buf)) == hipSuccess ? 0 : 2;
}
#endif
```

animating-gaussian-splats_amd/csrc/gsr_internal.h:

```cpp
#pragma once
#include <hip/hip_runtime.h>
#include <stdint.h>

namespace gsr {

struct ViewIn {
    int P, D, M, W, H, gx, gy, act;
    float scale_modifier, tan_fovx, tan_fovy, focal_x, focal_y;
    const float *means3D, *scales, *rotations, *opacities, *shs, *colors_precomp, *cov3D_precomp;
    const float *viewmatrix, *projmatrix, *campos, *bg;
    CamStrides cs;
};

struct FwdArgs {
    ViewIn v;
    float *depth; float4 *rec; uint2 *rect; uint32_t *tiles; uint32_t *goff; uint8_t *clampm;
    uint2 *ranges; float4 *pix_end; uint32_t *n_contrib; uint32_t *tile_maxc;
    uint32_t *tile_order_f; uint32_t *seg_off; uint32_t *sort_lists; uint32_t *tile_count;
    uint32_t *tile_cursor; uint32_t *block_sums; uint32_t *block_off; uint32_t *meta; uint32_t *chunk_off;
    uint32_t *items_ws; uint32_t *scan_ws; uint32_t *tile_rank;
    uint32_t *tile_flag; float4 *near_rec;
    uint32_t *tsat_list;
    uint4 *pairs; uint32_t *point_list; uint32_t *slot_emit; float4 *seg_state;
    int *radii; float *out_color; float *out_depth;
    uint32_t spec_cap; const uint32_t *spec_ok;
    uint32_t spec_sort_blocks;
    const uint32_t *gate; uint32_t gate_seq; uint32_t *gate_err; uint64_t gate_timeout;
    int exact;
};
constexpr int kSpecSortBlocks = 512;

struct BwdArgs {
    ViewIn v;
    int K;
    const int *radii;
    const float4 *rec; const uint2 *rect; const uint8_t *clampm;
    const uint32_t *goff; const uint2 *ranges; const float4 *pix_end; const uint32_t *n_contrib;
    const uint32_t *tile_maxc; const uint32_t *tile_flag; const float4 *near_rec; const uint32_t *seg_off; const uint32_t *meta; uint32_t *items_ws;
    const uint32_t *point_list; const uint32_t *slot_emit; const float4 *seg_state;
    uint2 *items; uint32_t max_items;
    float4 *part;
    const float *dL_dcolor;
    float *dL_dmeans2D, *dL_dcolors, *dL_dopacity, *dL_dmeans3D, *dL_dcov3D, *dL_dsh, *dL_dscales,
        *dL_drot;
    int accm;
    const uint32_t *spec_ok;
};

hipError_t launch_preprocess(const FwdArgs &a, hipStream_t s);
hipError_t launch_bin_count(const FwdArgs &a, hipStream_t s);
hipError_t launch_bin_scan(const FwdArgs &a, uint32_t *host_words, hipStream_t s);
hipError_t launch_bin_emit(const FwdArgs &a, int K, hipStream_t s);
hipError_t launch_tile_sort(const FwdArgs &a, uint32_t n_mid, uint32_t n_vlong, uint32_t max_n, uint4 *tmp,
                            hipStream_t s);
hipError_t launch_render_fwd(const FwdArgs &a, hipStream_t s);
hipError_t launch_zero(float *p, size_t n, hipStream_t s);
hipError_t launch_mark_visible(int P, const float *means3D, const float *viewmatrix, uint8_t *present,
                               hipStream_t s);

hipError_t launch_bwd_items(const BwdArgs &a, hipStream_t s);
hipError_t launch_bwd_items_raw(int K, int T, int P, const uint2 *ranges, const uint32_t *tile_maxc,
                                const uint32_t *tile_flag, uint2 *items, uint32_t *ws, hipStream_t s,
                                const uint32_t *spec_ok = nullptr);
hipError_t launch_render_bwd(const BwdArgs &a, hipStream_t s);
hipError_t launch_gauss_bwd(const BwdArgs &a, hipStream_t s);
hipError_t launch_sum_records(int P, const uint32_t *goff, const float4 *part, float *sums, hipStream_t s,
                              const uint32_t *spec_ok, const float *viewmatrix, const float *projmatrix,
                              const float *campos, CamStrides cs, int W, int H);

constexpr int kMultiViews = 8;
struct MultiView {
    const float *viewmatrix, *projmatrix, *campos;
    CamStrides cs;
    float tan_fovx, tan_fovy, focal_x, focal_y;
    const int *radii;
    const float4 *rec;
    const uint8_t *clampm;
    const float *sums;
    float *dL_dmeans2D;
    int acc2;
};
struct MultiArgs {
    int P, D, M, nv, act, accm;
    float scale_modifier;
    const float *means3D, *scales, *rotations, *shs, *cov3D_precomp;
    float *dL_dcolors, *dL_dopacity, *dL_dmeans3D, *dL_dcov3D, *dL_dsh, *dL_dscales, *dL_drot;
    MultiView v[kMultiViews];
};
hipError_t launch_gauss_bwd_multi(const MultiArgs &a, hipStream_t s);

struct SsimWindow { float w[11]; };
size_t ssim_partials(int planes, int H, int W);
hipError_t launch_ssim_fwd(int planes, int H, int W, const float *img1, const float *img2, const SsimWindow &w,
                           float *maps, float2 *partial, float *out_l1, float *out_ssim, hipStream_t s);
hipError_t launch_ssim_bwd(int planes, int H, int W, const float *img1, const float *img2, const SsimWindow &w,
                           const float *maps, const float *g_l1, const float *g_ssim, float *dimg1,
                           hipStream_t s);

hipError_t launch_knn(int n, const float *pts, int k, int *out_idx, double *out_d2, hipStream_t s);
int rigid_blocks(int F);
hipError_t launch_rigid_fwd(int F, int k, const float *means, const float *quats, const int *fg_rows,
                            const int *nbr_rows, const float *weights, const float *prev_off, const float *prev_inv,
                            double *partial, float *save_u, float *save_m, float *save_q, float *out_loss,
                            hipStream_t s);
hipError_t launch_rigid_bwd(int P, int F, int k, const int *row_to_fg, const int *rev_off, const int *rev_edge,
                            const float *save_u, const float *save_m, const float *save_q, const float *g_loss,
                            float *dmeans, float *dquats, hipStream_t s);

struct DensArgs {
    int P, prune_big;
    float grad_threshold, small_scale, big_scale, remove_opacity, inv_split_div;
    const float *grad_accum, *vis_count, *log_scales, *opacity_logits, *rotations;
};
struct DensColumn {
    int width, role;
    const float *src, *m_src, *v_src;
    float *dst, *m_dst, *v_dst;
};
constexpr int kDensMaxColumns = 8;
struct DensColumns { int n; DensColumn c[kDensMaxColumns]; };
struct DensWorkspace {
    int NB;
    size_t flags, bsum, boff, totals, total;
    explicit DensWorkspace(int P);
};
hipError_t launch_dens_radii(int P, const int *radii, float *max_radii, uint8_t *visible, hipStream_t s);
hipError_t launch_dens_grads(int P, const uint8_t *visible, const float *m2grad, float *grad_accum,
                             float *vis_count, hipStream_t s);
hipError_t launch_dens_plan(const DensArgs &a, char *ws, hipStream_t s);
hipError_t launch_dens_stds(const DensArgs &a, const char *ws, float *stds, hipStream_t s);
hipError_t launch_dens_apply(const DensArgs &a, const char *ws, const float *samples, const DensColumns &cols,
                             hipStream_t s);

struct AdamTensor {
    float *param; const float *grad; float *exp_avg; float *exp_avg_sq;
    long long n; float step_size, bc2_sqrt; int vec4;
};
constexpr int kAdamMaxTensors = 16;
struct AdamTable {
    int n; float w1, b2, omb2, eps;
    AdamTensor t[kAdamMaxTensors];
    int block_start[kAdamMaxTensors + 1];
};
int adam_blocks(long long n);
hipError_t launch_adam(const AdamTable &tab, hipStream_t s);

hipError_t launch_views_pack(int frames, int HW, const uint8_t *rgb, const uint8_t *seg, float *img, float *msk,
                             hipStream_t s);

}
```

animating-gaussian-splats_amd/diff_gaussian_rasterization/_C.py:

```python
from __future__ import annotations

import ctypes
import os
import threading

import torch

_HERE = os.path.dirname(os.path.abspath(__file__))
LIB_PATH = os.environ.get("GSR_LIB", os.path.join(_HERE, "libgsr.so"))

GSR_BUF_GEOM, GSR_BUF_BINNING, GSR_BUF_IMAGE, GSR_BUF_SCRATCH, GSR_BUF_SUMS = 0, 1, 2, 3, 4
EXPORTED_SYMBOLS = (
    "gsr_forward", "gsr_backward", "gsr_mark_visible", "gsr_geom_bytes", "gsr_image_bytes",
    "gsr_binning_bytes", "gsr_scratch_bytes", "gsr_last_error", "gsr_abi_version",
    "gsr_profile_enable", "gsr_profile_select", "gsr_profile_reset", "gsr_profile_read", "gsr_buffer_offsets",
    "gsr_ssim_scratch_bytes", "gsr_l1_ssim_forward", "gsr_l1_ssim_backward",
    "gsr_densify_update_radii", "gsr_densify_accumulate_grads", "gsr_densify_workspace_bytes",
    "gsr_densify_plan", "gsr_densify_split_stds", "gsr_densify_apply", "gsr_adam_step", "gsr_views_pack",
    "gsr_grad_fence", "gsr_backward_render", "gsr_backward_gaussians", "gsr_backward_items_bytes",
    "gsr_forward_info_call", "gsr_spec_stats", "gsr_sums_bytes", "gsr_prealloc_alloc", "gsr_spec_binning_bytes",
    "gsr_forward_async", "gsr_forward_resolve", "gsr_forward_release", "gsr_forward_query", "gsr_async_stats",
    "gsr_spec_keys", "gsr_async_shutdown", "gsr_debug_async_fault", "gsr_set_exact_thresholds",
    "gsr_knn", "gsr_rigidity_scratch_bytes", "gsr_rigidity_forward", "gsr_rigidity_backward",
)


class _Camera(ctypes.Structure):
    _fields_ = [("image_width", ctypes.c_int), ("image_height", ctypes.c_int),
                ("tan_fovx", ctypes.c_float), ("tan_fovy", ctypes.c_float),
                ("viewmatrix", ctypes.c_void_p), ("projmatrix", ctypes.c_void_p),
                ("campos", ctypes.c_void_p), ("bg", ctypes.c_void_p),
                ("prefiltered", ctypes.c_int), ("viewmatrix_stride", ctypes.c_int * 2),
                ("projmatrix_stride", ctypes.c_int * 2), ("campos_stride", ctypes.c_int)]


class _Gaussians(ctypes.Structure):
    _fields_ = [("P", ctypes.c_int), ("sh_degree", ctypes.c_int), ("sh_coeffs", ctypes.c_int),
                ("scale_modifier", ctypes.c_float), ("means3D", ctypes.c_void_p),
                ("shs", ctypes.c_void_p), ("colors_precomp", ctypes.c_void_p),
                ("opacities", ctypes.c_void_p), ("scales", ctypes.c_void_p),
                ("rotations", ctypes.c_void_p), ("cov3D_precomp", ctypes.c_void_p),
                ("activations", ctypes.c_int), ("prepare_backward", ctypes.c_int),
                ("binning_layout", ctypes.c_int)]


class _ForwardInfo(ctypes.Structure):
    _fields_ = [("num_rendered", ctypes.c_int), ("binning_layout", ctypes.c_int), ("speculated", ctypes.c_int),
                ("pending", ctypes.c_ulonglong), ("aux_stream", ctypes.c_void_p)]


class _Resolution(ctypes.Structure):
    _fields_ = [("num_rendered", ctypes.c_int), ("binning_layout", ctypes.c_int), ("binning", ctypes.c_void_p),
                ("redone", ctypes.c_int)]


class _Grads(ctypes.Structure):
    _fields_ = [(n, ctypes.c_void_p) for n in (
        "dL_dmeans2D", "dL_dcolors", "dL_dopacity", "dL_dmeans3D", "dL_dcov3D", "dL_dsh",
        "dL_dscales", "dL_drotations")] + [("accumulate", ctypes.c_int)]


class _ViewGrad(ctypes.Structure):
    _fields_ = [("cam", ctypes.POINTER(_Camera)), ("radii", ctypes.c_void_p), ("geom", ctypes.c_void_p),
                ("scratch", ctypes.c_void_p), ("num_rendered", ctypes.c_int),
                ("dL_dmeans2D", ctypes.c_void_p), ("accumulate_means2D", ctypes.c_int)]


_ALLOC_FN = ctypes.CFUNCTYPE(ctypes.c_void_p, ctypes.c_void_p, ctypes.c_int, ctypes.c_size_t)


class _Prealloc(ctypes.Structure):
    _fields_ = [("ptr", ctypes.c_void_p * 5), ("bytes", ctypes.c_size_t * 5), ("fallback", _ALLOC_FN),
                ("fallback_ctx", ctypes.c_void_p), ("used", ctypes.c_int)]


_lib = None
_PREALLOC_FN = None


def load_library():
    global _lib
    if _lib is not None:
        return _lib
    if not os.path.exists(LIB_PATH):
        raise RuntimeError(
            f"libgsr.so not found at {LIB_PATH}: build it with `make -C animating-gaussian-splats_amd/csrc` "
            "(or __graft_entry__.build()); the rasterizer has no CPU fallback")
    L = ctypes.CDLL(LIB_PATH)
    vp, i, f = ctypes.c_void_p, ctypes.c_int, ctypes.c_float
    L.gsr_forward.restype = i
    L.gsr_forward.argtypes = [ctypes.POINTER(_Camera), ctypes.POINTER(_Gaussians), _ALLOC_FN, vp,
                              vp, vp, vp, ctypes.POINTER(i), vp]
    L.gsr_forward_info_call.restype = i
    L.gsr_forward_info_call.argtypes = [ctypes.POINTER(_Camera), ctypes.POINTER(_Gaussians), _ALLOC_FN, vp,
                                        vp, vp, vp, i, ctypes.POINTER(_ForwardInfo), vp]
    L.gsr_spec_stats.restype = i
    L.gsr_spec_stats.argtypes = [ctypes.POINTER(i), ctypes.POINTER(i), i]
    L.gsr_spec_keys.restype = i
    L.gsr_spec_keys.argtypes = []
    L.gsr_forward_async.restype = i
    L.gsr_forward_async.argtypes = [ctypes.POINTER(_Camera), ctypes.POINTER(_Gaussians), _ALLOC_FN, vp,
                                    vp, vp, vp, ctypes.POINTER(_ForwardInfo), vp]
    L.gsr_forward_resolve.restype = i
    L.gsr_forward_resolve.argtypes = [ctypes.c_ulonglong, ctypes.POINTER(_Resolution)]
    L.gsr_forward_release.restype = i
    L.gsr_forward_release.argtypes = [ctypes.c_ulonglong]
    L.gsr_forward_query.restype = i
    L.gsr_forward_query.argtypes = [ctypes.c_ulonglong]
    L.gsr_async_stats.restype = i
    L.gsr_async_stats.argtypes = [ctypes.POINTER(i), ctypes.POINTER(i)]
    L.gsr_async_shutdown.restype = i
    L.gsr_async_shutdown.argtypes = []
    L.gsr_debug_async_fault.restype = i
    L.gsr_debug_async_fault.argtypes = [i, i, i]
    import atexit
    atexit.register(L.gsr_async_shutdown)
    L.gsr_backward.restype = i
    L.gsr_backward.argtypes = [ctypes.POINTER(_Camera), ctypes.POINTER(_Gaussians), vp, i, vp, vp, vp,
                               vp, vp, _ALLOC_FN, vp, ctypes.POINTER(_Grads), vp]
    L.gsr_backward_render.restype = i
    L.gsr_backward_render.argtypes = [ctypes.POINTER(_Camera), ctypes.POINTER(_Gaussians), vp, i, vp, vp, vp,
                                      vp, _ALLOC_FN, vp, vp]
    L.gsr_backward_gaussians.restype = i
    L.gsr_backward_gaussians.argtypes = [i, ctypes.POINTER(_ViewGrad), ctypes.POINTER(_Gaussians),
                                         ctypes.POINTER(_Grads), vp]
    L.gsr_grad_fence.restype = i
    L.gsr_grad_fence.argtypes = [ctypes.POINTER(vp), i, vp]
    L.gsr_mark_visible.restype = i
    L.gsr_mark_visible.argtypes = [i, vp, vp, vp, vp, vp]
    L.gsr_geom_bytes.restype = ctypes.c_size_t
    L.gsr_geom_bytes.argtypes = [i]
    L.gsr_binning_bytes.restype = ctypes.c_size_t
    L.gsr_binning_bytes.argtypes = [i, i]
    L.gsr_sums_bytes.restype = ctypes.c_size_t
    L.gsr_sums_bytes.argtypes = [i]
    for n in ("gsr_scratch_bytes", "gsr_backward_items_bytes"):
        getattr(L, n).restype = ctypes.c_size_t
        getattr(L, n).argtypes = [i, i, i]
    L.gsr_image_bytes.restype = ctypes.c_size_t
    L.gsr_image_bytes.argtypes = [i, i, i]
    L.gsr_last_error.restype = ctypes.c_char_p
    L.gsr_last_error.argtypes = []
    L.gsr_abi_version.restype = i
    L.gsr_profile_enable.argtypes = [i]
    L.gsr_profile_enable.restype = i
    L.gsr_profile_reset.restype = i
    L.gsr_profile_select.argtypes = [ctypes.c_char_p]
    L.gsr_profile_select.restype = i
    L.gsr_profile_read.argtypes = [ctypes.c_char_p, ctypes.POINTER(ctypes.c_double), ctypes.POINTER(i)]
    L.gsr_profile_read.restype = i
    L.gsr_buffer_offsets.restype = i
    L.gsr_buffer_offsets.argtypes = [i, i, i, i, ctypes.POINTER(ctypes.c_size_t), i]
    L.gsr_ssim_scratch_bytes.restype = ctypes.c_size_t
    L.gsr_ssim_scratch_bytes.argtypes = [i, i, i]
    L.gsr_l1_ssim_forward.restype = i
    L.gsr_l1_ssim_forward.argtypes = [i, i, i, vp, vp, vp, vp, vp, vp]
    L.gsr_l1_ssim_backward.restype = i
    L.gsr_l1_ssim_backward.argtypes = [i, i, i, vp, vp, vp, vp, vp, vp, vp]
    L.gsr_spec_binning_bytes.restype = ctypes.c_size_t
    L.gsr_spec_binning_bytes.argtypes = [i, i, i, i]
    L.gsr_set_exact_thresholds.restype = i
    L.gsr_set_exact_thresholds.argtypes = [i]
    L.gsr_knn.restype = i
    L.gsr_knn.argtypes = [i, vp, i, vp, vp, vp]
    L.gsr_rigidity_scratch_bytes.restype = ctypes.c_size_t
    L.gsr_rigidity_scratch_bytes.argtypes = [i, i, i]
    L.gsr_rigidity_forward.restype = i
    L.gsr_rigidity_forward.argtypes = [i, i, i, vp, vp, vp, vp, vp, vp, vp, vp, i, vp, vp]
    L.gsr_rigidity_backward.restype = i
    L.gsr_rigidity_backward.argtypes = [i, i, i, vp, vp, vp, vp, vp, vp, vp, vp]
    if L.gsr_abi_version() != ABI_VERSION:
        raise RuntimeError(f"libgsr.so ABI {L.gsr_abi_version()} != binding ABI {ABI_VERSION}: rebuild it")
    global _PREALLOC_FN
    _PREALLOC_FN = _ALLOC_FN(ctypes.cast(L.gsr_prealloc_alloc, ctypes.c_void_p).value)
    _lib = L
    return L


ABI_VERSION = 21
ACT_SIGMOID_OPACITY, ACT_EXP_SCALES, ACT_NORMALIZE_ROTATIONS = 1, 2, 4
ACT_ALL = ACT_SIGMOID_OPACITY | ACT_EXP_SCALES | ACT_NORMALIZE_ROTATIONS


def set_exact_thresholds(on: bool) -> bool:
    return bool(load_library().gsr_set_exact_thresholds(int(bool(on))))


def _check(rc):
    if rc != 0:
        msg = _lib.gsr_last_error().decode(errors="replace")
        raise RuntimeError(f"libgsr error {rc}: {msg}")


def _ptr(t):
    if t is None or t.numel() == 0:
        return None
    if not t.is_cuda:
        raise RuntimeError("diff_gaussian_rasterization: tensors must be on the GPU (no CPU path)")
    if t.dtype != torch.float32:
        raise RuntimeError(f"diff_gaussian_rasterization: expected float32, got {t.dtype}")
    return t.data_ptr()


def _bp(b):
    return b if isinstance(b, int) else b.data_ptr()


def _f32(t):
    return t.contiguous() if t is not None and t.numel() else t


_tls = threading.local()


def _fallback_alloc(_ctx, which, nbytes):
    try:
        t = torch.empty(max(int(nbytes), 1), dtype=torch.uint8, device=_tls.device)
    except Exception:
        return None
    _tls.buffers[int(which)] = t
    return t.data_ptr()


_FALLBACK_FN = _ALLOC_FN(_fallback_alloc)
_PREALLOC_ON = os.environ.get("GSR_PREALLOC", "1") != "0"


class _PreAllocator:

    def __init__(self, device, groups):
        self.device = device
        self.pa = _Prealloc()
        self.given = {}
        for group in groups if _PREALLOC_ON else ():
            offs, total = [], 0
            for which, nbytes in group:
                offs.append((which, total, nbytes))
                total += (int(nbytes) + 255) & ~255
            if total == 0:
                continue
            buf = torch.empty(total, dtype=torch.uint8, device=device)
            base = buf.data_ptr()
            for which, o, nbytes in offs:
                if nbytes > 0:
                    self.given[which] = (buf, o, int(nbytes))
                    self.pa.ptr[which] = base + o
                    self.pa.bytes[which] = int(nbytes)
        self.pa.fallback = _FALLBACK_FN
        self.cb = _PREALLOC_FN
        self.ctx = ctypes.byref(self.pa)
        self._views = None

    def __enter__(self):
        self.prev = getattr(_tls, "buffers", None), getattr(_tls, "device", None)
        _tls.buffers, _tls.device = {}, self.device
        return self

    def __exit__(self, *exc):
        got = _tls.buffers
        _tls.buffers, _tls.device = self.prev
        used = self.pa.used
        self._took({w: g for w, g in self.given.items() if (used >> w) & 1}, got)
        return False

    def _took(self, taken, fallback):
        self.taken, self.fallback = taken, fallback
        self.ptrs = {w: b.data_ptr() + o for w, (b, o, _) in taken.items()}
        self.ptrs.update({w: t.data_ptr() for w, t in fallback.items()})
        bases = {id(g[0]): g[0] for g in taken.values()}
        bases.update({id(t): t for t in fallback.values()})
        self.bases = list(bases.values())
        self._views = None

    def base_of(self, which):
        if which in self.fallback:
            return self.fallback[which]
        g = self.taken.get(which)
        return g[0] if g is not None else None

    @property
    def buffers(self):
        if self._views is None:
            v = {w: b.narrow(0, o, n) for w, (b, o, n) in self.taken.items()}
            v.update(self.fallback)
            self._views = v
        return self._views


class _NativeAlloc(_PreAllocator):

    def __init__(self, res):
        taken, fallback = res
        self._took({w: (b, o, n) for w, b, o, n in taken}, dict(fallback))


_native_mod = None
_NATIVE_PARTS = int(os.environ.get("GSR_NATIVE_BIND", "15"))
_EMPTY = torch.empty(0)


def _native():
    global _native_mod
    if _native_mod is None:
        _native_mod = False
        path = os.path.join(_HERE, "gsr_bind.so")
        if _NATIVE_PARTS and os.path.exists(path):
            import importlib.machinery
            import importlib.util
            L = load_library()
            import warnings
            try:
                spec = importlib.util.spec_from_file_location(
                    "gsr_bind", path, loader=importlib.machinery.ExtensionFileLoader("gsr_bind", path))
                m = importlib.util.module_from_spec(spec)
                spec.loader.exec_module(m)
                abi = m.abi_version() if hasattr(m, "abi_version") else None
            except (ImportError, OSError) as err:
                warnings.warn(f"gsr_bind.so not loadable ({err}); binding libgsr through ctypes instead")
                return None
            if abi != L.gsr_abi_version():
                warnings.warn(f"gsr_bind.so built for ABI {abi}, libgsr.so is ABI {L.gsr_abi_version()}: "
                              "binding libgsr through ctypes instead (rebuild gsr_bind)")
                return None
            m.set_functions({n: ctypes.cast(L[n], ctypes.c_void_p).value for n in (
                "gsr_forward_info_call", "gsr_forward_async", "gsr_backward_render", "gsr_backward_gaussians",
                "gsr_backward", "gsr_prealloc_alloc",
                "gsr_spec_binning_bytes", "gsr_geom_bytes", "gsr_image_bytes", "gsr_scratch_bytes",
                "gsr_sums_bytes", "gsr_last_error")})
            _native_mod = m
    return _native_mod or None


_get_device = torch._C._cuda_getDevice
_raw_stream = torch._C._cuda_getCurrentRawStream


class _device_guard:

    def __init__(self, dev):
        self.idx = dev.index if dev.index is not None else _get_device()
        self.prev = None

    def __enter__(self):
        cur = _get_device()
        if cur != self.idx:
            self.prev = cur
            torch.cuda.set_device(self.idx)
        return self

    def __exit__(self, *exc):
        if self.prev is not None:
            torch.cuda.set_device(self.prev)
        return False


def _stream_ptr(device):
    return ctypes.c_void_p(_raw_stream(device.index if device.index is not None else _get_device()))


_CAM_CACHE = {}
_CAM_CACHE_MAX = 512


def _camera(viewmatrix, projmatrix, tan_fovx, tan_fovy, image_height, image_width, campos, bg,
            prefiltered, keep):
    key = (id(viewmatrix), id(projmatrix), id(campos), id(bg), image_width, image_height, tan_fovx, tan_fovy,
           prefiltered)
    e = _CAM_CACHE.get(key)
    if e is not None:
        cam, refs, ptrs = e
        if (refs[0] is viewmatrix and refs[1] is projmatrix and refs[2] is campos and refs[3] is bg and
                ptrs == (viewmatrix.data_ptr(), projmatrix.data_ptr(),
                         campos.data_ptr() if campos is not None else 0, bg.data_ptr())):
            return cam
    vm, vs = _mat16(viewmatrix)
    pm, ps = _mat16(projmatrix)
    bg_ = bg if bg.dtype == torch.float32 and bg.is_contiguous() else bg.contiguous().float()
    cp, cs = None, 0
    if campos is not None and campos.numel():
        cp = campos if campos.dtype == torch.float32 and campos.dim() == 1 else campos.reshape(-1).float()
        cs = cp.stride(0)
    keep += [vm, pm, bg_, cp]
    cam = _Camera(int(image_width), int(image_height), float(tan_fovx), float(tan_fovy),
                  _ptr(vm), _ptr(pm), _ptr(cp) if cp is not None else None,
                  _ptr(bg_), int(bool(prefiltered)))
    cam.viewmatrix_stride[0], cam.viewmatrix_stride[1] = vs
    cam.projmatrix_stride[0], cam.projmatrix_stride[1] = ps
    cam.campos_stride = cs
    if vm is viewmatrix and pm is projmatrix and bg_ is bg and (cp is campos):
        if len(_CAM_CACHE) >= _CAM_CACHE_MAX:
            _CAM_CACHE.clear()
        _CAM_CACHE[key] = (cam, (viewmatrix, projmatrix, campos, bg),
                           (viewmatrix.data_ptr(), projmatrix.data_ptr(),
                            campos.data_ptr() if campos is not None else 0, bg.data_ptr()))
    return cam


def _mat16(m):
    if m.numel() != 16:
        raise RuntimeError("viewmatrix/projmatrix must hold 16 floats")
    if m.dtype != torch.float32:
        m = m.float()
    if m.shape in ((4, 4), (1, 4, 4)):
        return m, (m.stride(-2), m.stride(-1))
    m2 = m.reshape(4, 4)
    return m2, (m2.stride(0), m2.stride(1))


def _gaussians(means3D, sh, degree, colors, opacity, scales, rotations, scale_modifier, cov3D, keep,
               activations=0, prepare_backward=False, binning_layout=0):
    if means3D.ndimension() != 2 or means3D.size(1) != 3:
        raise RuntimeError("means3D must have dimensions (num_points, 3)")
    P = means3D.size(0)
    ts = [_f32(x) for x in (means3D, sh, colors, opacity, scales, rotations, cov3D)]
    keep += ts
    means3D, sh, colors, opacity, scales, rotations, cov3D = ts
    M = sh.size(1) if sh is not None and sh.numel() else 0
    return _Gaussians(P, int(degree), M, float(scale_modifier), _ptr(means3D), _ptr(sh), _ptr(colors),
                      _ptr(opacity), _ptr(scales), _ptr(rotations), _ptr(cov3D),
                      int(activations), int(bool(prepare_backward)), int(binning_layout or 0)), P, M


class AsyncForward:
    __slots__ = ("handle", "_res")

    def __init__(self, handle):
        self.handle = int(handle)
        self._res = None

    def __del__(self):
        _release_async(self.handle)

    def ready(self):
        return self._res is not None or load_library().gsr_forward_query(self.handle) > 0

    def resolve(self):
        if self._res is None:
            r = _Resolution()
            _check(load_library().gsr_forward_resolve(self.handle, ctypes.byref(r)))
            self._res = (r.num_rendered, r.binning_layout, r.binning, bool(r.redone))
        return self._res[:3]

    @property
    def redone(self):
        return self._res[3] if self._res is not None else None


def _release_async(handle):
    if _lib is not None:
        _lib.gsr_forward_release(handle)


def debug_async_fault(hold_next_redo_ms=0, gate_timeout_ms=0, clear=False):
    _check(load_library().gsr_debug_async_fault(int(hold_next_redo_ms), int(gate_timeout_ms), int(bool(clear))))


def async_stats():
    c, p = ctypes.c_int(0), ctypes.c_int(0)
    _check(load_library().gsr_async_stats(ctypes.byref(c), ctypes.byref(p)))
    return c.value, p.value


def rasterize_gaussians(background, means3D, colors, opacity, scales, rotations, scale_modifier,
                        cov3D_precomp, viewmatrix, projmatrix, tan_fovx, tan_fovy, image_height,
                        image_width, sh, degree, campos, prefiltered, debug=False, activations=0,
                        prepare_backward=False, speculate=False, info=None, nonblocking=False):
    fi, color, radii, depth, alloc, pending = _forward(
        background, means3D, colors, opacity, scales, rotations, scale_modifier, cov3D_precomp, viewmatrix,
        projmatrix, tan_fovx, tan_fovy, image_height, image_width, sh, degree, campos, prefiltered, activations,
        prepare_backward, speculate, nonblocking)
    if info is not None:
        info.update(num_rendered=fi.num_rendered, binning_layout=fi.binning_layout, speculated=bool(fi.speculated),
                    pending=pending)
    b = alloc.buffers
    return fi.num_rendered, color, radii, b[GSR_BUF_GEOM], b[GSR_BUF_BINNING], b[GSR_BUF_IMAGE], depth


def _forward(background, means3D, colors, opacity, scales, rotations, scale_modifier, cov3D_precomp, viewmatrix,
             projmatrix, tan_fovx, tan_fovy, image_height, image_width, sh, degree, campos, prefiltered, activations,
             prepare_backward, speculate, nonblocking):
    L = load_library()
    nat = _native() if _NATIVE_PARTS & 1 else None
    if nat is not None:
        e = _EMPTY
        (K, layout, spec, pend, aux, color, radii, depth, res) = nat.forward(
            background, means3D, e if colors is None else colors, e if opacity is None else opacity,
            e if scales is None else scales,
            e if rotations is None else rotations, float(scale_modifier), e if cov3D_precomp is None else cov3D_precomp,
            viewmatrix, projmatrix, float(tan_fovx), float(tan_fovy), int(image_height), int(image_width),
            e if sh is None else sh, int(degree), e if campos is None else campos, bool(prefiltered),
            int(activations), bool(prepare_backward), bool(speculate), bool(nonblocking), _PREALLOC_ON)
        fi = _ForwardInfo(K, layout, spec, pend, aux or None)
        alloc = _NativeAlloc(res)
    else:
        fi, color, radii, depth, alloc = _forward_ctypes(
            L, background, means3D, colors, opacity, scales, rotations, scale_modifier, cov3D_precomp, viewmatrix,
            projmatrix, tan_fovx, tan_fovy, image_height, image_width, sh, degree, campos, prefiltered, activations,
            prepare_backward, speculate, nonblocking)
    pending = AsyncForward(fi.pending) if fi.pending else None
    return fi, color, radii, depth, alloc, pending


def _forward_ctypes(L, background, means3D, colors, opacity, scales, rotations, scale_modifier, cov3D_precomp,
                    viewmatrix, projmatrix, tan_fovx, tan_fovy, image_height, image_width, sh, degree, campos,
                    prefiltered, activations, prepare_backward, speculate, nonblocking):
    keep = []
    g, P, _ = _gaussians(means3D, sh, degree, colors, opacity, scales, rotations, scale_modifier,
                         cov3D_precomp, keep, activations, prepare_backward)
    cam = _camera(viewmatrix, projmatrix, tan_fovx, tan_fovy, image_height, image_width, campos,
                  background, prefiltered, keep)
    dev = means3D.device
    H, W = int(image_height), int(image_width)
    color = torch.empty((3, H, W), dtype=torch.float32, device=dev)
    depth = torch.empty((1, H, W), dtype=torch.float32, device=dev)
    radii = torch.empty((P,), dtype=torch.int32, device=dev)
    fi = _ForwardInfo(0, 0, 0)
    with _device_guard(dev):
        spec = L.gsr_spec_binning_bytes(P, W, H, int(bool(prepare_backward))) if (speculate or nonblocking) and P else 0
        alloc = _PreAllocator(dev, [[(GSR_BUF_GEOM, L.gsr_geom_bytes(P)), (GSR_BUF_IMAGE, L.gsr_image_bytes(W, H, P))],
                                    [(GSR_BUF_BINNING, spec)]])
        with alloc:
            if nonblocking:
                _check(L.gsr_forward_async(ctypes.byref(cam), ctypes.byref(g), alloc.cb, alloc.ctx, color.data_ptr(),
                                           depth.data_ptr(), radii.data_ptr() if P else None, ctypes.byref(fi),
                                           _stream_ptr(dev)))
            else:
                _check(L.gsr_forward_info_call(ctypes.byref(cam), ctypes.byref(g), alloc.cb, alloc.ctx,
                                               color.data_ptr(), depth.data_ptr(), radii.data_ptr() if P else None,
                                               int(bool(speculate)), ctypes.byref(fi), _stream_ptr(dev)))
    return fi, color, radii, depth, alloc


_EXT_STREAMS = {}


def _external_stream(ptr, dev):
    key = (dev.index if dev.index is not None else torch.cuda.current_device(), int(ptr))
    st = _EXT_STREAMS.get(key)
    if st is None:
        d = torch.device("cuda", key[0])
        st = torch.cuda.default_stream(d) if key[1] == 0 else torch.cuda.ExternalStream(key[1], device=d)
        _EXT_STREAMS[key] = st
    return st


def speculation_stats(reset=False):
    h, m = ctypes.c_int(0), ctypes.c_int(0)
    _check(load_library().gsr_spec_stats(ctypes.byref(h), ctypes.byref(m), int(bool(reset))))
    return h.value, m.value


def _grad_outputs(P, M, dev, colors, cov3D_precomp, scales, rotations, skip_unused, accumulate_into,
                  skip=(), overwrite=()):
    e = lambda *s: torch.empty(s, dtype=torch.float32, device=dev)
    has = lambda t: t is not None and t.numel() > 0
    keep_col = not skip_unused or has(colors)
    keep_cov = not skip_unused or has(cov3D_precomp)
    keep_sr = not skip_unused or (has(scales) and has(rotations))
    shapes = [(P, 3), (P, 3) if keep_col else (0,), (P, 1), (P, 3), (P, 6) if keep_cov else (0,),
              (P, M, 3), (P, 3) if keep_sr else (0,), (P, 4) if keep_sr else (0,)]
    acc = list(accumulate_into or ()) + [None] * 8
    out = []
    acc_bits = given = 0
    for k, shp in enumerate(shapes):
        t = acc[k]
        if k in skip:
            out.append(None)
            continue
        if t is None or shp == (0,):
            out.append(e(*shp))
            continue
        if tuple(t.shape) != shp or t.dtype != torch.float32 or not t.is_contiguous() or t.device != dev:
            raise RuntimeError(f"accumulate_into[{k}]: expected a contiguous float32 {shp} tensor on {dev}")
        out.append(t)
        given |= 1 << k
        if k not in overwrite:
            acc_bits |= 1 << k
    out = tuple(out)
    if given:
        cs = torch.cuda.current_stream(dev)
        for k in range(8):
            if given >> k & 1:
                out[k].record_stream(cs)
    return out, acc_bits


def rasterize_gaussians_backward(background, means3D, radii, colors, scales, rotations,
                                 scale_modifier, cov3D_precomp, viewmatrix, projmatrix, tan_fovx,
                                 tan_fovy, dL_dout_color, sh, degree, campos, geomBuffer, R,
                                 binningBuffer, imageBuffer, debug=False, dL_dout_depth=None,
                                 activations=0, skip_unused=False, accumulate_into=None,
                                 prepare_backward=False, needed=None, binning_layout=0, binning_ptr=None):
    L = load_library()
    nat = _native() if _NATIVE_PARTS & 8 else None
    if nat is not None:
        if means3D.ndimension() != 2 or means3D.size(1) != 3:
            raise RuntimeError("means3D must have dimensions (num_points, 3)")
        P, dev = means3D.size(0), means3D.device
        M = sh.size(1) if sh is not None and sh.numel() else 0
        skip = tuple(k for k in range(8) if needed is not None and not needed[k])
        out, acc_bits = _grad_outputs(P, M, dev, colors, cov3D_precomp, scales, rotations, skip_unused,
                                      accumulate_into, skip=skip)
        e = _EMPTY
        nat.backward(background, means3D, radii, e if colors is None else colors, e if scales is None else scales,
                     e if rotations is None else rotations, float(scale_modifier),
                     e if cov3D_precomp is None else cov3D_precomp, viewmatrix, projmatrix, float(tan_fovx),
                     float(tan_fovy), dL_dout_color, e if sh is None else sh, int(degree),
                     e if campos is None else campos, _bp(geomBuffer), int(R), binning_ptr or _bp(binningBuffer),
                     _bp(imageBuffer), int(activations), bool(prepare_backward), int(binning_layout or 0),
                     list(out), int(acc_bits), _PREALLOC_ON)
        return out
    keep = []
    g, P, M = _gaussians(means3D, sh, degree, colors, torch.empty(0, device=means3D.device), scales,
                         rotations, scale_modifier, cov3D_precomp, keep, activations, prepare_backward,
                         binning_layout)
    H, W = dL_dout_color.shape[-2], dL_dout_color.shape[-1]
    cam = _camera(viewmatrix, projmatrix, tan_fovx, tan_fovy, H, W, campos, background, False, keep)
    dev = means3D.device
    skip = tuple(k for k in range(8) if needed is not None and not needed[k])
    out, acc_bits = _grad_outputs(P, M, dev, colors, cov3D_precomp, scales, rotations, skip_unused,
                                  accumulate_into, skip=skip)
    if P == 0:
        return out
    dpix = dL_dout_color.contiguous().float()
    keep.append(dpix)
    grads = _Grads(*[t.data_ptr() if t is not None and t.numel() else None for t in out], acc_bits)
    alloc = _PreAllocator(dev, [[(GSR_BUF_SCRATCH, L.gsr_scratch_bytes(int(R), W, H))]])
    with _device_guard(dev), alloc:
        _check(L.gsr_backward(ctypes.byref(cam), ctypes.byref(g), radii.data_ptr(), int(R),
                              _bp(geomBuffer), binning_ptr or _bp(binningBuffer), _bp(imageBuffer),
                              dpix.data_ptr(), None, alloc.cb, alloc.ctx, ctypes.byref(grads), _stream_ptr(dev)))
    return out


def rasterize_gaussians_backward_render(background, means3D, radii, colors, scales, rotations,
                                        scale_modifier, cov3D_precomp, viewmatrix, projmatrix, tan_fovx,
                                        tan_fovy, dL_dout_color, sh, degree, campos, geomBuffer, R,
                                        binningBuffer, imageBuffer, activations=0, prepare_backward=False,
                                        binning_layout=0, binning_ptr=None):
    L = load_library()
    nat = _native() if _NATIVE_PARTS & 2 else None
    if nat is not None:
        e = _EMPTY
        sums, _ = nat.backward_render(
            background, means3D, radii, e if colors is None else colors, e if scales is None else scales,
            e if rotations is None else rotations, float(scale_modifier), e if cov3D_precomp is None else cov3D_precomp,
            viewmatrix, projmatrix, float(tan_fovx), float(tan_fovy), dL_dout_color, e if sh is None else sh,
            int(degree), e if campos is None else campos, _bp(geomBuffer), int(R),
            binning_ptr or _bp(binningBuffer), _bp(imageBuffer), int(activations), bool(prepare_backward),
            int(binning_layout or 0), _PREALLOC_ON)
        return sums
    keep = []
    g, P, _ = _gaussians(means3D, sh, degree, colors, torch.empty(0, device=means3D.device), scales,
                         rotations, scale_modifier, cov3D_precomp, keep, activations, prepare_backward,
                         binning_layout)
    H, W = dL_dout_color.shape[-2], dL_dout_color.shape[-1]
    cam = _camera(viewmatrix, projmatrix, tan_fovx, tan_fovy, H, W, campos, background, False, keep)
    dev = means3D.device
    if P == 0:
        return torch.empty(1, dtype=torch.uint8, device=dev)
    dpix = dL_dout_color.contiguous().float()
    keep.append(dpix)
    alloc = _PreAllocator(dev, [[(GSR_BUF_SCRATCH, L.gsr_scratch_bytes(int(R) if R >= 0 else int(binning_layout), W, H))],
                                [(GSR_BUF_SUMS, L.gsr_sums_bytes(P))]])
    with _device_guard(dev), alloc:
        _check(L.gsr_backward_render(ctypes.byref(cam), ctypes.byref(g), radii.data_ptr(), int(R),
                                     _bp(geomBuffer), binning_ptr or _bp(binningBuffer), _bp(imageBuffer),
                                     dpix.data_ptr(), alloc.cb, alloc.ctx, _stream_ptr(dev)))
    return alloc.buffers[GSR_BUF_SUMS]


def rasterize_gaussians_backward_views(views, means3D, colors, scales, rotations, scale_modifier,
                                       cov3D_precomp, sh, degree, activations=0, skip_unused=True,
                                       accumulate_into=None, overwrite=(), needed=None):
    L = load_library()
    keep = []
    dev = means3D.device
    g, P, M = _gaussians(means3D, sh, degree, colors, torch.empty(0, device=dev), scales, rotations,
                         scale_modifier, cov3D_precomp, keep, activations)
    skip = (0,) + tuple(k for k in range(1, 8) if needed is not None and not needed[k])
    out, acc_bits = _grad_outputs(P, M, dev, colors, cov3D_precomp, scales, rotations, skip_unused,
                                  accumulate_into, skip=skip, overwrite=overwrite)
    if P == 0 or not views:
# ... 114 lines not shown
```

animating-gaussian-splats_amd/diff_gaussian_rasterization/__init__.py:

```python
from __future__ import annotations

import os
import threading
import weakref
from typing import NamedTuple

import torch
import torch.nn as nn
from torch.autograd.graph import get_gradient_edge

from . import _C

__all__ = ["GaussianRasterizationSettings", "GaussianRasterizer", "rasterize_gaussians",
           "rasterize_parameters", "set_deferred_backward", "set_speculative_forward", "set_async_forward", "async_forward", "set_exact_thresholds",
           "pending_views", "clear_pending"]


class GaussianRasterizationSettings(NamedTuple):
    image_height: int
    image_width: int
    tanfovx: float
    tanfovy: float
    bg: torch.Tensor
    scale_modifier: float
    viewmatrix: torch.Tensor
    projmatrix: torch.Tensor
    sh_degree: int
    campos: torch.Tensor
    prefiltered: bool
    debug: bool = False


def _engine_accumulates(t, node=None):
    try:
        return bool(torch._C._will_engine_execute_node(node if node is not None else get_gradient_edge(t).node))
    except RuntimeError:
        return False


def _tensor_positions(args):
    pos, k = {}, 0
    for i, a in enumerate(args):
        if isinstance(a, torch.Tensor):
            pos[i] = k
            k += 1
    return pos


def _input_nodes(ctx, inputs):
    nf = ctx.next_functions
    pos = ctx.tensor_pos
    return [nf[pos[i]][0] if i in pos and pos[i] < len(nf) else None for i in inputs]


def _accumulation_target(t, node=None, create=False):
    if t is None or not isinstance(t, torch.Tensor) or t.numel() == 0 or not t.is_leaf or not t.requires_grad:
        return None
    g = t.grad
    if g is None and not (create and t.dtype == torch.float32 and t.is_contiguous()):
        return None
    if g is not None and (g.dtype != torch.float32 or not g.is_contiguous() or g.shape != t.shape or g.requires_grad):
        return None
    if t._backward_hooks or getattr(t, "_post_accumulate_grad_hooks", None):
        return None
    if torch.is_grad_enabled() or not _engine_accumulates(t, node):
        return None
    if g is None:
        if not _defer["fresh"]:
            t.grad = g = torch.zeros_like(t)
            return g
        return _Fresh(t)
    return g


class _Fresh:
    __slots__ = ("leaf",)

    def __init__(self, leaf):
        self.leaf = leaf


def _fresh_target(t, created, post):
    if not isinstance(t, _Fresh):
        return t, False
    leaf = t.leaf
    g = leaf.grad
    if g is None:
        leaf.grad = g = torch.empty_like(leaf, memory_format=torch.contiguous_format)
        created.add(id(leaf))
    elif id(leaf) not in created and (g.dtype != torch.float32 or not g.is_contiguous() or
                                      g.shape != leaf.shape or g.requires_grad):
        tmp = torch.zeros_like(leaf, memory_format=torch.contiguous_format)
        post.append((leaf, tmp))
        return tmp, False
    return g, id(leaf) in created


_defer = {"on": os.environ.get("GSR_DEFER_BACKWARD", "1") != "0",
          "fresh": os.environ.get("GSR_FRESH_GRADS", "1") != "0",
          "speculate": os.environ.get("GSR_SPECULATE", "1") != "0",
          "async": os.environ.get("GSR_ASYNC_FORWARD", "0") == "1",
          "spec_half": os.environ.get("GSR_SPEC_RENDER_HALF", "1") != "0"}
_async_tls = threading.local()
_pending_lock = threading.Lock()
_pending = {}
_queued = set()
_spec_half_stats = {"queued": 0, "redone": 0}


def set_deferred_backward(on: bool) -> bool:
    prev = _defer["on"]
    _defer["on"] = bool(on)
    return prev


def set_speculative_forward(on: bool) -> bool:
    prev = _defer["speculate"]
    _defer["speculate"] = bool(on)
    return prev


def set_exact_thresholds(on: bool) -> bool:
    return _C.set_exact_thresholds(on)


def set_async_forward(on: bool) -> bool:
    prev = _defer["async"]
    _defer["async"] = bool(on)
    return prev


class async_forward:

    def __init__(self, on: bool = True):
        self.on = bool(on)

    def __enter__(self):
        self.prev = getattr(_async_tls, "on", None)
        _async_tls.on = self.on
        return self

    def __exit__(self, *exc):
        _async_tls.on = self.prev
        return False


def _async_on():
    o = getattr(_async_tls, "on", None)
    return _defer["async"] if o is None else o


def _buffer_ptrs(alloc):
    p = alloc.ptrs
    return p[_C.GSR_BUF_GEOM], p[_C.GSR_BUF_BINNING], p[_C.GSR_BUF_IMAGE]


def _resolved(ctx):
    if ctx.pending is not None:
        return ctx.pending.resolve()
    return ctx.num_rendered, ctx.binning_layout, None


def pending_views() -> int:
    with _pending_lock:
        return sum(len(g["views"]) for g in _pending.values())


def clear_pending() -> None:
    with _pending_lock:
        _pending.clear()
        _queued.clear()


def _drop_task(task):
    with _pending_lock:
        for k in [k for k in _pending if k[0] == task]:
            del _pending[k]
        _queued.discard(task)


class _TaskFlush:
    __slots__ = ("task", "__weakref__")

    def __init__(self, task):
        self.task = task

    def __call__(self):
        _flush_pending(self.task)


def _queue_flush(task):
    cb = _TaskFlush(task)
    weakref.finalize(cb, _drop_task, task)
    torch.autograd.Variable._execution_engine.queue_callback(cb)


def _flush_pending(task):
    with _pending_lock:
        groups = [g for (t, _), g in _pending.items() if t == task]
        for k in [k for k in _pending if k[0] == task]:
            del _pending[k]
        _queued.discard(task)
    created, post = set(), []
    for grp in groups:
        _run_group(grp, created, post)
    for leaf, tmp in post:
        leaf.grad = leaf.grad + tmp


def _run_group(grp, created, post):
    dev = grp["device"]
    with torch.cuda.device(dev):
        cur = torch.cuda.current_stream(dev)
        for v in grp["views"]:
            pend = v.pop("spec", None)
            if pend is not None:
                K, _, _ = pend.resolve()
                if pend.redone:
                    v["scratch"] = None
                    _spec_half_stats["redone"] += 1
                else:
                    v["num_rendered"] = K
                    v.pop("render_fn")
            if v["scratch"] is None:
                with torch.cuda.stream(_C._external_stream(v["stream"], dev)):
                    v["scratch"], v["num_rendered"] = v.pop("render_fn")()
        cur_ptr = cur.cuda_stream
        for s in grp["streams"]:
            if s != cur_ptr:
                cur.wait_stream(_C._external_stream(s, dev))
        (means3D, colors, scales, rotations, scale_modifier, cov3D, sh, degree, act) = grp["gauss"]
        targets, over = [None] * 8, []
        for k in range(1, 8):
            targets[k], ow = _fresh_target(grp["targets"][k], created, post)
            if ow:
                over.append(k)
        views = []
        for v in grp["views"]:
            m2, ow = _fresh_target(v["means2D_grad"], created, post)
            views.append(dict(v, means2D_grad=m2, accumulate_means2D=not ow))
            if ow:
                created.discard(id(v["means2D_grad"].leaf))
        needed = [k == 0 or grp["targets"][k] is not None for k in range(8)]
        _C.rasterize_gaussians_backward_views(views, means3D, colors, scales, rotations,
                                              scale_modifier, cov3D, sh, degree, activations=act,
                                              skip_unused=True, accumulate_into=targets, overwrite=over,
                                              needed=needed)
        for k in over:
            created.discard(id(grp["targets"][k].leaf))


def _try_defer(ctx, gauss, radii, geomBuffer, leaf_inputs, nodes, need, render_fn, keep=()):
    if not _defer["on"]:
        return False
    means3D, colors, scales, rotations, scale_modifier, cov3D, sh, degree, act = gauss
    P = means3D.shape[0]
    if P == 0 or not means3D.is_cuda or (sh.numel() and sh.shape[1] not in (1, 4, 9, 16)):
        return False
    task = torch._C._current_graph_task_id()
    if task < 0:
        return False
    op = ctx.leaves[2]
    if need[leaf_inputs[2]] and (op is None or tuple(op.shape) != (P, 1)):
        return False
    targets = [None] * 8
    for k, (t, i, node) in enumerate(zip(ctx.leaves, leaf_inputs, nodes)):
        if i is None or not need[i]:
            continue
        tgt = _accumulation_target(t, node, create=True)
        if tgt is None:
            return False
        targets[k] = tgt
    rs = ctx.raster_settings
    dix = means3D.device.index
    stream = _C._raw_stream(dix if dix is not None else _C._get_device())
    spec = None
    if ctx.pending is None or ctx.pending.ready():
        scratch, K = render_fn()
    elif _defer["spec_half"]:
        scratch, K = render_fn(True)
        spec = ctx.pending
        _spec_half_stats["queued"] += 1
    else:
        scratch, K = None, -1
    ptr = lambda t: t.data_ptr() if t is not None and t.numel() else 0
    tkey = lambda t: ("fresh", id(t.leaf)) if isinstance(t, _Fresh) else ptr(t)
    key = (means3D.device, P, ptr(means3D), ptr(scales), ptr(rotations), ptr(cov3D), ptr(sh), ptr(colors),
           int(degree), float(scale_modifier), int(act)) + tuple(tkey(t) for t in targets[1:])
    view = {"viewmatrix": rs.viewmatrix, "projmatrix": rs.projmatrix, "tanfovx": rs.tanfovx,
            "tanfovy": rs.tanfovy, "image_height": rs.image_height, "image_width": rs.image_width,
            "campos": rs.campos, "bg": rs.bg, "radii": radii, "geomBuffer": geomBuffer, "scratch": scratch,
            "num_rendered": K, "means2D_grad": targets[0], "accumulate_means2D": True, "stream": stream,
            "keep": keep}
    if scratch is None or spec is not None:
        view["render_fn"] = render_fn
    if spec is not None:
        view["spec"] = spec
    with _pending_lock:
        grp = _pending.get((task, key))
        if grp is None:
            grp = _pending[(task, key)] = {"device": means3D.device, "views": [], "gauss": gauss,
                                           "targets": targets, "streams": []}
        grp["views"].append(view)
        if stream not in grp["streams"]:
            grp["streams"].append(stream)
        queue = task not in _queued
        _queued.add(task)
    if queue:
        _queue_flush(task)
    return True


def rasterize_gaussians(means3D, means2D, sh, colors_precomp, opacities, scales, rotations,
                        cov3Ds_precomp, raster_settings):
    args = (means3D, means2D, sh, colors_precomp, opacities, scales, rotations, cov3Ds_precomp)
    return _RasterizeGaussians.apply(*args, raster_settings, torch.is_grad_enabled())


class _RasterizeGaussians(torch.autograd.Function):
    @staticmethod
    def forward(ctx, means3D, means2D, sh, colors_precomp, opacities, scales, rotations,
                cov3Ds_precomp, raster_settings, grad_mode=False):
        rs = raster_settings
        args = (rs.bg, means3D, colors_precomp, opacities, scales, rotations, rs.scale_modifier,
                cov3Ds_precomp, rs.viewmatrix, rs.projmatrix, rs.tanfovx, rs.tanfovy,
                rs.image_height, rs.image_width, sh, rs.sh_degree, rs.campos, rs.prefiltered)
        ctx.prep = bool(grad_mode) and any(ctx.needs_input_grad)
        fi, color, radii, depth, alloc, pending = _C._forward(
            *args, 0, ctx.prep, _defer["speculate"], _async_on())
        ctx.raster_settings = rs
        ctx.num_rendered = fi.num_rendered
        ctx.binning_layout = fi.binning_layout
        ctx.pending = pending
        ctx.bufs = _buffer_ptrs(alloc)
        ctx.leaves = (means2D, colors_precomp, opacities, means3D, cov3Ds_precomp, sh, scales, rotations)
        ctx.tensor_pos = _tensor_positions((means3D, means2D, sh, colors_precomp, opacities, scales,
                                            rotations, cov3Ds_precomp))
        ctx.save_for_backward(colors_precomp, means3D, scales, rotations, cov3Ds_precomp, radii, sh,
                              *alloc.bases)
        ctx.mark_non_differentiable(radii)
        ctx.set_materialize_grads(False)
        return color, radii, depth

    @staticmethod
    def backward(ctx, grad_out_color, _grad_radii, grad_depth):
        if grad_out_color is None:
            return (None,) * 10
        rs = ctx.raster_settings
        saved = ctx.saved_tensors
        colors_precomp, means3D, scales, rotations, cov3Ds_precomp, radii, sh = saved[:7]
        bases = saved[7:]
        geomBuffer, binningBuffer, imgBuffer = ctx.bufs

        def args_kw(spec=False):
            K, layout, bptr = (-1, ctx.binning_layout, None) if spec else _resolved(ctx)
            return ((rs.bg, means3D, radii, colors_precomp, scales, rotations, rs.scale_modifier,
                     cov3Ds_precomp, rs.viewmatrix, rs.projmatrix, rs.tanfovx, rs.tanfovy, grad_out_color,
                     sh, rs.sh_degree, rs.campos, geomBuffer, K, binningBuffer, imgBuffer),
                    {"prepare_backward": ctx.prep, "binning_layout": layout, "binning_ptr": bptr})

        def render_half(spec=False):
            a, k = args_kw(spec)
            return _C.rasterize_gaussians_backward_render(*a, **k), a[17]
        inputs = (1, 3, 4, 0, 7, 2, 5, 6)
        nodes = _input_nodes(ctx, inputs)
        gauss = (means3D, colors_precomp, scales, rotations, rs.scale_modifier, cov3Ds_precomp, sh,
                 rs.sh_degree, 0)
        if _try_defer(ctx, gauss, radii, geomBuffer, inputs, nodes, ctx.needs_input_grad, render_half, bases):
            return (None,) * 10
        args, kw = args_kw()
        need = [ctx.needs_input_grad[i] for i in inputs]
        acc = [_accumulation_target(t, node) if n else None for t, n, node in zip(ctx.leaves, need, nodes)]
        g = list(_C.rasterize_gaussians_backward(*args, skip_unused=True, accumulate_into=acc, needed=need, **kw))
        for k, t in enumerate(acc):
            if t is not None:
                g[k] = None
        (grad_means2D, grad_colors_precomp, grad_opacities, grad_means3D, grad_cov3Ds_precomp,
         grad_sh, grad_scales, grad_rotations) = g
        return (grad_means3D, grad_means2D, grad_sh, grad_colors_precomp, grad_opacities,
                grad_scales, grad_rotations, grad_cov3Ds_precomp, None, None)


class GaussianRasterizer(nn.Module):
    def __init__(self, raster_settings):
        super().__init__()
        self.raster_settings = raster_settings

    def markVisible(self, positions):
        with torch.no_grad():
            rs = self.raster_settings
            visible = _C.mark_visible(positions, rs.viewmatrix, rs.projmatrix)
        return visible

    def forward(self, means3D, means2D, opacities, shs=None, colors_precomp=None, scales=None,
                rotations=None, cov3D_precomp=None):
        rs = self.raster_settings
        if (shs is None and colors_precomp is None) or (shs is not None and colors_precomp is not None):
            raise Exception('Please provide excatly one of either SHs or precomputed colors!')
        if ((scales is None or rotations is None) and cov3D_precomp is None) or \
                ((scales is not None or rotations is not None) and cov3D_precomp is not None):
            raise Exception('Please provide exactly one of either scale/rotation pair or precomputed 3D covariance!')
        empty = torch.Tensor([])
        if shs is None:
            shs = empty
        if colors_precomp is None:
            colors_precomp = empty
        if scales is None:
            scales = empty
        if rotations is None:
            rotations = empty
        if cov3D_precomp is None:
            cov3D_precomp = empty
        return rasterize_gaussians(means3D, means2D, shs, colors_precomp, opacities, scales,
                                   rotations, cov3D_precomp, rs)


def rasterize_parameters(params, raster_settings, means2D=None, shs=None):
    means = params["means"]
    if means2D is None:
        means2D = torch.empty(0, device=means.device)
    colors = params["colors"] if shs is None else torch.empty(0, device=means.device)
    if shs is None:
        shs = torch.empty(0, device=means.device)
    return _RasterizeGaussianParameters.apply(means, means2D, shs, colors, params["opacity_logits"],
                                              params["log_scales"], params["rotation_quaternions"],
                                              raster_settings, torch.is_grad_enabled())


class _RasterizeGaussianParameters(torch.autograd.Function):
    @staticmethod
    def forward(ctx, means, means2D, sh, colors, opacity_logits, log_scales, quaternions, raster_settings,
                grad_mode=False):
        rs = raster_settings
        empty = torch.empty(0, device=means.device)
        ctx.prep = bool(grad_mode) and any(ctx.needs_input_grad)
        fi, color, radii, depth, alloc, pending = _C._forward(
            rs.bg, means, colors, opacity_logits, log_scales, quaternions, rs.scale_modifier, empty,
            rs.viewmatrix, rs.projmatrix, rs.tanfovx, rs.tanfovy, rs.image_height, rs.image_width, sh,
            rs.sh_degree, rs.campos, rs.prefiltered, _C.ACT_ALL, ctx.prep, _defer["speculate"], _async_on())
        ctx.raster_settings = rs
        ctx.num_rendered = fi.num_rendered
        ctx.binning_layout = fi.binning_layout
        ctx.pending = pending
        ctx.bufs = _buffer_ptrs(alloc)
        ctx.opacity_shape = opacity_logits.shape
        ctx.leaves = (means2D, colors, opacity_logits, means, None, sh, log_scales, quaternions)
        ctx.tensor_pos = _tensor_positions((means, means2D, sh, colors, opacity_logits, log_scales, quaternions))
        ctx.save_for_backward(colors, means, log_scales, quaternions, radii, sh, *alloc.bases)
        ctx.mark_non_differentiable(radii)
        ctx.set_materialize_grads(False)
        return color, radii, depth

    @staticmethod
    def backward(ctx, grad_out_color, _grad_radii, _grad_depth):
        if grad_out_color is None:
            return (None,) * 9
        rs = ctx.raster_settings
        saved = ctx.saved_tensors
        colors, means, log_scales, quaternions, radii, sh = saved[:6]
        bases = saved[6:]
        geomBuffer, binningBuffer, imgBuffer = ctx.bufs
        empty = torch.empty(0, device=means.device)
        need = ctx.needs_input_grad
        inputs = (1, 3, 4, 0, None, 2, 5, 6)
        nodes = _input_nodes(ctx, [i for i in inputs if i is not None])
        nodes.insert(4, None)
        gauss = (means, colors, log_scales, quaternions, rs.scale_modifier, empty, sh, rs.sh_degree, _C.ACT_ALL)
        def render_half(spec=False):
            K, layout, bptr = (-1, ctx.binning_layout, None) if spec else _resolved(ctx)
            return _C.rasterize_gaussians_backward_render(
                rs.bg, means, radii, colors, log_scales, quaternions, rs.scale_modifier, empty,
                rs.viewmatrix, rs.projmatrix, rs.tanfovx, rs.tanfovy, grad_out_color, sh,
                rs.sh_degree, rs.campos, geomBuffer, K, binningBuffer, imgBuffer,
                activations=_C.ACT_ALL, prepare_backward=ctx.prep, binning_layout=layout, binning_ptr=bptr), K
        if _try_defer(ctx, gauss, radii, geomBuffer, inputs, nodes, need, render_half, bases):
            return (None,) * 9
        K, layout, bptr = _resolved(ctx)
        acc = [_accumulation_target(t, node) if i is not None and need[i] else None
               for t, i, node in zip(ctx.leaves, inputs, nodes)]
        if acc[2] is not None and acc[2].shape != (means.shape[0], 1):
            acc[2] = None
        needed = [i is not None and need[i] for i in inputs]
        (g_means2D, g_colors, g_opacity, g_means, _g_cov3D, g_sh, g_scales, g_rot) = \
            _C.rasterize_gaussians_backward(
                rs.bg, means, radii, colors, log_scales, quaternions, rs.scale_modifier, empty,
                rs.viewmatrix, rs.projmatrix, rs.tanfovx, rs.tanfovy, grad_out_color, sh, rs.sh_degree,
                rs.campos, geomBuffer, K, binningBuffer, imgBuffer,
                activations=_C.ACT_ALL, skip_unused=True, accumulate_into=acc, prepare_backward=ctx.prep,
                needed=needed, binning_layout=layout, binning_ptr=bptr)
        done = [t is not None or not n for t, n in zip(acc, needed)]
        return (None if done[3] else g_means, None if (done[0] or not need[1]) else g_means2D,
                None if (done[5] or not sh.numel()) else g_sh,
                None if (done[1] or not colors.numel()) else g_colors,
                None if done[2] else g_opacity.view(ctx.opacity_shape),
                None if done[6] else g_scales, None if done[7] else g_rot, None, None)
```

animating-gaussian-splats_amd/splat_step.py:

```python
from __future__ import annotations

import os
from concurrent.futures import ThreadPoolExecutor
from contextlib import nullcontext as _nullcontext
from typing import Callable, Sequence

import torch

from diff_gaussian_rasterization import GaussianRasterizer, async_forward


class RenderStep:
    def __init__(self, device, cams: Sequence, inputs_of: Callable, dl: torch.Tensor, streams: Sequence,
                 threads: bool = True, shape: str = "summed", rotate: bool | None = None):
        if shape not in ("summed", "per_view"):
            raise ValueError(f"shape: 'summed' or 'per_view', got {shape!r}")
        self.device, self.cams, self.inputs_of, self.dl = device, cams, inputs_of, dl
        self.streams = list(streams)
        self.shape = shape
        self.rotate = os.environ.get("GSR_STREAM_ROTATE", "1") != "0" if rotate is None else rotate
        self.calls = 0
        self.pool = ([ThreadPoolExecutor(max_workers=1) for _ in self.streams]
                     if threads and len(self.streams) > 1 else None)

    def close(self):
        if self.pool is not None:
            for ex in self.pool:
                ex.shutdown()
            self.pool = None

    def _forwards(self, vs, s):
        torch.cuda.set_device(self.device)
        with torch.cuda.stream(s):
            return [GaussianRasterizer(raster_settings=self.cams[ci])(**self.inputs_of(ci))[0] for ci in vs]

    def _fwd_bwd(self, vs, s):
        torch.cuda.set_device(self.device)
        with torch.cuda.stream(s):
            for ci in vs:
                img = GaussianRasterizer(raster_settings=self.cams[ci])(**self.inputs_of(ci))[0]
                img.backward(self.dl)

    def __call__(self, views: Sequence[int], solo: bool = False):
        ns = 1 if solo else len(self.streams)
        pool = None if solo else self.pool
        off = self.calls % ns if self.rotate else 0
        self.calls += 1
        streams = self.streams[off:ns] + self.streams[:off] if ns > 1 else self.streams[:1]
        with async_forward(True) if pool is None and ns > 1 else _nullcontext():
            return self._run(views, ns, pool, streams)

    def _run(self, views, ns, pool, streams):
        if self.shape == "summed":
            if pool is not None:
                futs = [pool[self.streams.index(streams[k])].submit(self._forwards, views[k::ns], streams[k])
                        for k in range(min(ns, len(views)))]
                imgs = [None] * len(views)
                for k, f in enumerate(futs):
                    imgs[k::ns] = f.result()
            else:
                imgs = []
                prev_dev = torch.cuda.current_device()
                torch.cuda.set_device(self.device)
                cur = torch.cuda.current_stream(self.device)
                try:
                    for k, ci in enumerate(views):
                        torch.cuda.set_stream(streams[k % ns])
                        imgs.append(GaussianRasterizer(raster_settings=self.cams[ci])(**self.inputs_of(ci))[0])
                finally:
                    torch.cuda.set_stream(cur)
                    torch.cuda.set_device(prev_dev)
            torch.autograd.backward(imgs, [self.dl] * len(imgs))
            return [img.detach() for img in imgs]
        elif pool is not None:
            futs = [pool[self.streams.index(streams[k])].submit(self._fwd_bwd, views[k::ns], streams[k])
                    for k in range(min(ns, len(views)))]
            for f in futs:
                f.result()
        else:
            for k, ci in enumerate(views):
                self._fwd_bwd([ci], streams[k % ns])
        return None
```

include/gsr.h:

```cpp
#ifndef GSR_H
#define GSR_H

#include <stddef.h>
#include <stdint.h>

#ifdef __cplusplus
extern "C" {
#endif

#define GSR_ABI_VERSION 21

enum gsr_status {
    GSR_OK = 0,
    GSR_ERR_ARG = 1,
    GSR_ERR_HIP = 2,
    GSR_ERR_ALLOC = 3,
    GSR_ERR_UNSUPPORTED = 4
};

enum gsr_buffer { GSR_BUF_GEOM = 0, GSR_BUF_BINNING = 1, GSR_BUF_IMAGE = 2, GSR_BUF_SCRATCH = 3,
                  GSR_BUF_SUMS = 4  };

typedef void *(*gsr_alloc_fn)(void *ctx, int which, size_t bytes);

typedef struct gsr_camera {
    int image_width;
    int image_height;
    float tan_fovx;
    float tan_fovy;
    const float *viewmatrix;
    const float *projmatrix;
    const float *campos;
    const float *bg;
    int prefiltered;
    int viewmatrix_stride[2];
    int projmatrix_stride[2];
    int campos_stride;
} gsr_camera;

enum gsr_activation {
    GSR_ACT_NONE = 0,
    GSR_ACT_SIGMOID_OPACITY = 1,
    GSR_ACT_EXP_SCALES = 2,
    GSR_ACT_NORMALIZE_ROTATIONS = 4
};

typedef struct gsr_gaussians {
    int P;
    int sh_degree;
    int sh_coeffs;
    float scale_modifier;
    const float *means3D;
    const float *shs;
    const float *colors_precomp;
    const float *opacities;
    const float *scales;
    const float *rotations;
    const float *cov3D_precomp;
    int activations;
    int prepare_backward;
    int binning_layout;
} gsr_gaussians;

enum gsr_grad_bits {
    GSR_GRAD_MEANS2D = 1, GSR_GRAD_COLORS = 2, GSR_GRAD_OPACITY = 4, GSR_GRAD_MEANS3D = 8,
    GSR_GRAD_COV3D = 16, GSR_GRAD_SH = 32, GSR_GRAD_SCALES = 64, GSR_GRAD_ROTATIONS = 128
};

typedef struct gsr_grads {
    float *dL_dmeans2D;
    float *dL_dcolors;
    float *dL_dopacity;
    float *dL_dmeans3D;
    float *dL_dcov3D;
    float *dL_dsh;
    float *dL_dscales;
    float *dL_drotations;
    int accumulate;
} gsr_grads;

int gsr_forward(const gsr_camera *cam, const gsr_gaussians *g, gsr_alloc_fn alloc, void *alloc_ctx,
                float *out_color, float *out_depth, int *out_radii, int *out_num_rendered,
                void *stream);

typedef struct gsr_forward_info {
    int num_rendered;
    int binning_layout;
    int speculated;
    unsigned long long pending;
    void *aux_stream;
} gsr_forward_info;
int gsr_forward_info_call(const gsr_camera *cam, const gsr_gaussians *g, gsr_alloc_fn alloc, void *alloc_ctx,
                          float *out_color, float *out_depth, int *out_radii, int speculate, gsr_forward_info *info,
                          void *stream);
int gsr_spec_stats(int *hits, int *misses, int reset);
int gsr_spec_keys(void);

typedef struct gsr_forward_resolution {
    int num_rendered;
    int binning_layout;
    void *binning;
    int redone;
} gsr_forward_resolution;
int gsr_forward_async(const gsr_camera *cam, const gsr_gaussians *g, gsr_alloc_fn alloc, void *alloc_ctx,
                      float *out_color, float *out_depth, int *out_radii, gsr_forward_info *info, void *stream);
int gsr_forward_resolve(unsigned long long handle, gsr_forward_resolution *out);
int gsr_forward_release(unsigned long long handle);
int gsr_forward_query(unsigned long long handle);
int gsr_async_stats(int *calls, int *pending);
int gsr_async_shutdown(void);
int gsr_debug_async_fault(int hold_next_redo_ms, int gate_timeout_ms, int clear);

int gsr_backward(const gsr_camera *cam, const gsr_gaussians *g, const int *radii, int num_rendered,
                 const void *geom, const void *binning, const void *image, const float *dL_dcolor,
                 const float *dL_ddepth, gsr_alloc_fn alloc, void *alloc_ctx, gsr_grads *out,
                 void *stream);

typedef struct gsr_view_grad {
    const gsr_camera *cam;
    const int *radii;
    const void *geom;
    const void *scratch;
    int num_rendered;
    float *dL_dmeans2D;
    int accumulate_means2D;
} gsr_view_grad;

int gsr_backward_render(const gsr_camera *cam, const gsr_gaussians *g, const int *radii, int num_rendered,
                        const void *geom, const void *binning, const void *image, const float *dL_dcolor,
                        gsr_alloc_fn alloc, void *alloc_ctx, void *stream);
int gsr_backward_gaussians(int nviews, const gsr_view_grad *views, const gsr_gaussians *g, gsr_grads *out,
                           void *stream);

int gsr_grad_fence(const void *const *grads, int n, void *stream);

int gsr_mark_visible(int P, const float *means3D, const float *viewmatrix, const float *projmatrix,
                     uint8_t *present, void *stream);

size_t gsr_geom_bytes(int P);
size_t gsr_image_bytes(int width, int height, int P);
size_t gsr_binning_bytes(int num_rendered, int P);
size_t gsr_scratch_bytes(int num_rendered, int width, int height);
size_t gsr_sums_bytes(int P);
size_t gsr_backward_items_bytes(int num_rendered, int width, int height);

typedef struct gsr_prealloc {
    void *ptr[5];
    size_t bytes[5];
    gsr_alloc_fn fallback;
    void *fallback_ctx;
    int used;
} gsr_prealloc;
void *gsr_prealloc_alloc(void *ctx, int which, size_t bytes);
size_t gsr_spec_binning_bytes(int P, int width, int height, int prepare_backward);

int gsr_buffer_offsets(int P, int width, int height, int num_rendered, size_t *out, int max_out);

const char *gsr_last_error(void);
int gsr_abi_version(void);

int gsr_set_exact_thresholds(int on);

size_t gsr_ssim_scratch_bytes(int planes, int height, int width);
int gsr_l1_ssim_forward(int planes, int height, int width, const float *img1, const float *img2,
                        void *scratch, float *out_l1, float *out_ssim, void *stream);
int gsr_l1_ssim_backward(int planes, int height, int width, const float *img1, const float *img2,
                         const void *scratch, const float *dL_dl1, const float *dL_dssim,
                         float *dL_dimg1, void *stream);

int gsr_knn(int n, const float *points, int k, int *out_indices, double *out_sq_distances, void *stream);
size_t gsr_rigidity_scratch_bytes(int F, int k, int save_for_backward);
int gsr_rigidity_forward(int P, int F, int k, const float *means, const float *rotation_quaternions,
                         const int *foreground_rows, const int *neighbor_rows, const float *weights,
                         const float *previous_offsets, const float *previous_inverted_rotations, void *scratch,
                         int save_for_backward, float *out_loss, void *stream);
int gsr_rigidity_backward(int P, int F, int k, const int *row_to_foreground, const int *reverse_offsets,
                          const int *reverse_edges, const void *scratch, const float *dL_dloss, float *dL_dmeans,
                          float *dL_drotation_quaternions, void *stream);

enum gsr_densify_role {
    GSR_DENS_OTHER = 0,
    GSR_DENS_MEANS = 1,
    GSR_DENS_LOG_SCALES = 2
};

typedef struct gsr_densify_settings {
    int P;
    float grad_threshold;
    float small_scale;
    float big_scale;
    float remove_opacity;
    int prune_big;
    float split_divisor;
    const float *grad_accum;
    const float *vis_count;
    const float *log_scales;
    const float *opacity_logits;
    const float *rotation_quaternions;
} gsr_densify_settings;

typedef struct gsr_densify_counts {
    int n_keep_orig;
    int n_keep_clone;
    int n_split;
    int n_keep_split;
    int P_out;
} gsr_densify_counts;

typedef struct gsr_densify_column {
    int width;
    int role;
    const float *src, *exp_avg, *exp_avg_sq;
    float *dst, *dst_exp_avg, *dst_exp_avg_sq;
} gsr_densify_column;

int gsr_densify_update_radii(int P, const int *radii, float *max_radii, uint8_t *visible, void *stream);
int gsr_densify_accumulate_grads(int P, const uint8_t *visible, const float *means2D_grad,
                                 float *grad_accum, float *vis_count, void *stream);
size_t gsr_densify_workspace_bytes(int P);
int gsr_densify_plan(const gsr_densify_settings *s, void *workspace, gsr_densify_counts *counts,
                     void *stream);
int gsr_densify_split_stds(const gsr_densify_settings *s, const void *workspace, float *stds, void *stream);
int gsr_densify_apply(const gsr_densify_settings *s, const void *workspace, const gsr_densify_counts *counts,
                      const float *samples, int ncols, const gsr_densify_column *cols, void *stream);

typedef struct gsr_adam_tensor {
    float *param;
    const float *grad;
    float *exp_avg;
    float *exp_avg_sq;
    long long numel;
    double lr;
    double step;
} gsr_adam_tensor;

int gsr_adam_step(int ntensors, const gsr_adam_tensor *tensors, double beta1, double beta2, double eps,
                  void *stream);

int gsr_views_pack(int frames, int H, int W, const uint8_t *rgb, const uint8_t *seg, float *images,
                   float *seg_masks, void *stream);

int gsr_profile_enable(int on);
int gsr_profile_select(const char *phases);
int gsr_profile_reset(void);
int gsr_profile_read(const char *phase, double *total_ms, int *count);

#ifdef __cplusplus
}
#endif
#endif
```

Baseline: 1420 Msplats/s.

## Batch per-view preprocessing into one multi-view kernel shared across streams

Adds gsr_preprocess_views, which runs preprocessing for several cameras in one multi-view kernel launch. Each Gaussian's per-Gaussian data (covariance, SH) is loaded once and projected into several views, filling each view's geometry buffer. Forward calls then pick up the prefilled buffer through an event wait instead of launching their own preprocess, and signature checks guard against rendering stale geometry. The aim is fewer launches and less repeated reading of Gaussian attributes. In exchange, preprocessing is serialized on the first stream ahead of all views, so it can delay the other streams, and it adds host-side bookkeeping.

```diff
diff --git a/animating-gaussian-splats_amd/csrc/gsr_api.hip b/animating-gaussian-splats_amd/csrc/gsr_api.hip
--- a/animating-gaussian-splats_amd/csrc/gsr_api.hip
+++ b/animating-gaussian-splats_amd/csrc/gsr_api.hip
@@ -192,6 +192,62 @@
     v.cs.c0 = cam->campos_stride ? cam->campos_stride : 1;
 }
 
+std::mutex g_pre_pool_mu;
+std::vector<hipEvent_t> g_pre_evpool;
+struct PreEvent {
+    hipEvent_t ev = nullptr;
+    ~PreEvent() {
+        if (!ev) return;
+        std::lock_guard<std::mutex> lk(g_pre_pool_mu);
+        g_pre_evpool.push_back(ev);
+    }
+};
+struct PreSig {
+    gsr_camera cam;
+    gsr_gaussians g;
+    const int *radii;
+};
+void pre_sig(PreSig &sg, const gsr_camera *cam, const gsr_gaussians *g, const int *radii) {
+    memset(&sg, 0, sizeof(sg));
+    sg.cam.image_width = cam->image_width; sg.cam.image_height = cam->image_height;
+    sg.cam.tan_fovx = cam->tan_fovx; sg.cam.tan_fovy = cam->tan_fovy;
+    sg.cam.viewmatrix = cam->viewmatrix; sg.cam.projmatrix = cam->projmatrix;
+    sg.cam.campos = g->shs ? cam->campos : nullptr;
+    for (int k = 0; k < 2; ++k) {
+        sg.cam.viewmatrix_stride[k] = cam->viewmatrix_stride[k];
+        sg.cam.projmatrix_stride[k] = cam->projmatrix_stride[k];
+    }
+    sg.cam.campos_stride = g->shs ? cam->campos_stride : 0;
+    sg.g.P = g->P; sg.g.sh_degree = g->shs ? g->sh_degree : 0; sg.g.sh_coeffs = g->shs ? g->sh_coeffs : 0;
+    sg.g.scale_modifier = g->scale_modifier;
+    sg.g.means3D = g->means3D; sg.g.shs = g->shs; sg.g.colors_precomp = g->colors_precomp;
+    sg.g.opacities = g->opacities; sg.g.scales = g->scales; sg.g.rotations = g->rotations;
+    sg.g.cov3D_precomp = g->cov3D_precomp;
+    sg.g.activations = g->activations;
+    sg.radii = radii;
+}
+struct PreFill { hipStream_t s = nullptr; std::shared_ptr<PreEvent> ev; PreSig sig; };
+std::mutex g_pre_mu;
+std::unordered_map<const void *, PreFill> g_pre;
+int g_pre_launches = 0, g_pre_consumed = 0;
+
+int pre_take(const void *geom, const gsr_camera *cam, const gsr_gaussians *g, const int *radii, PreFill *out) {
+    std::lock_guard<std::mutex> lk(g_pre_mu);
+    auto it = g_pre.find(geom);
+    if (it == g_pre.end()) return GSR_OK;
+    PreSig sg;
+    pre_sig(sg, cam, g, radii);
+    *out = std::move(it->second);
+    g_pre.erase(it);
+    if (memcmp(&sg, &out->sig, sizeof(sg)) != 0) {
+        out->ev.reset();
+        return fail(GSR_ERR_ARG, "the GEOM buffer was preprocessed (gsr_preprocess_views) from other cameras / Gaussians / "
+                                 "radii than this forward's: refusing to render stale geometry");
+    }
+    ++g_pre_consumed;
+    return GSR_OK;
+}
+
 template <typename A>
 void carve_saved(A &a, char *geom, char *img) {
     const GeomLayout G(a.v.P);
@@ -600,6 +656,9 @@
     if (!geom || !img) return fail(GSR_ERR_ALLOC, "allocation callback failed (geom/image)");
     carve_forward(a, geom, img);
     *info = gsr_forward_info{};
+    PreFill pre;
+    rc = pre_take(geom, cam, g, out_radii, &pre);
+    if (rc) return rc;
     if (P == 0) {
         const size_t npix = (size_t)a.v.W * a.v.H;
         HIP_TRY(launch_zero(out_color, 3 * npix, s));
@@ -644,7 +703,13 @@
         words_h = hw.h; words_d = hw.d;
     }
     __atomic_store_n(words_h, kNoValue, __ATOMIC_SEQ_CST);
-    { Phase ph(s, "preprocess"); HIP_TRY(launch_preprocess(a, s)); }
+    if (pre.ev) {
+        if (pre.s != s) HIP_TRY(hipStreamWaitEvent(s, pre.ev->ev, 0));
+        if (T > kMaxLdsTiles) HIP_TRY(hipMemsetAsync(a.tile_count, 0, sizeof(uint32_t) * (size_t)T, s));
+    } else {
+        Phase ph(s, "preprocess");
+        HIP_TRY(launch_preprocess(a, s));
+    }
     { Phase ph(s, "bin_count"); HIP_TRY(launch_bin_count(a, s)); }
     { Phase ph(s, "bin_scan"); HIP_TRY(launch_bin_scan(a, words_d, s)); }
     if (af) {
@@ -709,6 +774,87 @@
 }
 
 extern "C" {
+
+int gsr_preprocess_views(int nviews, const gsr_camera *const *cams, const gsr_gaussians *g, void *const *geom,
+                         int *const *radii, void *stream) {
+    HostPhase host_total("host_preprocess");
+    if (nviews < 0 || (nviews > 0 && (!cams || !geom || !radii)))
+        return fail(GSR_ERR_ARG, "gsr_preprocess_views: bad view list");
+    for (int v = 0; v < nviews; ++v) {
+        const int rc = check_common(cams[v], g, true);
+        if (rc) return rc;
+        if (g->P > 0 && (!geom[v] || !radii[v])) return fail(GSR_ERR_ARG, "gsr_preprocess_views: view %d lacks geom / radii", v);
+        for (int w = 0; w < v; ++w)
+            if (g->P > 0 && (geom[w] == geom[v] || radii[w] == radii[v]))
+                return fail(GSR_ERR_ARG, "gsr_preprocess_views: views %d and %d share a geom / radii buffer", w, v);
+    }
+    if (nviews == 0 || g->P == 0) return GSR_OK;
+    hipStream_t s = (hipStream_t)stream;
+    PreMultiArgs m;
+    memset(&m, 0, sizeof(m));
+    m.P = g->P; m.D = g->sh_degree; m.M = g->shs ? g->sh_coeffs : 0; m.act = g->activations;
+    m.scale_modifier = g->scale_modifier;
+    m.means3D = g->means3D; m.scales = g->scales; m.rotations = g->rotations; m.opacities = g->opacities;
+    m.shs = g->shs; m.colors_precomp = g->colors_precomp; m.cov3D_precomp = g->cov3D_precomp;
+    const GeomLayout G(g->P);
+    int launches = 0;
+    for (int v0 = 0; v0 < nviews; v0 += kMultiViews) {
+        m.nv = std::min(kMultiViews, nviews - v0);
+        for (int k = 0; k < m.nv; ++k) {
+            ViewIn f;
+            fill_common(f, cams[v0 + k], g);
+            PreView &pv = m.v[k];
+            pv.viewmatrix = f.viewmatrix; pv.projmatrix = f.projmatrix; pv.campos = f.campos; pv.cs = f.cs;
+            pv.W = f.W; pv.H = f.H; pv.gx = f.gx; pv.gy = f.gy;
+            pv.tan_fovx = f.tan_fovx; pv.tan_fovy = f.tan_fovy; pv.focal_x = f.focal_x; pv.focal_y = f.focal_y;
+            char *gb = (char *)geom[v0 + k];
+            pv.radii = radii[v0 + k];
+            pv.depth = (float *)(gb + G.depth); pv.rec = (float4 *)(gb + G.rec); pv.rect = (uint2 *)(gb + G.rect);
+            pv.tiles = (uint32_t *)(gb + G.tiles); pv.clampm = (uint8_t *)(gb + G.clampm);
+        }
+        Phase ph(s, "preprocess");
+        HIP_TRY(launch_preprocess_multi(m, s));
+        ++launches;
+    }
+    auto ev = std::make_shared<PreEvent>();
+    {
+        std::lock_guard<std::mutex> lk(g_pre_pool_mu);
+        if (!g_pre_evpool.empty()) { ev->ev = g_pre_evpool.back(); g_pre_evpool.pop_back(); }
+    }
+    if (!ev->ev) HIP_TRY(hipEventCreateWithFlags(&ev->ev, hipEventDisableTiming));
+    HIP_TRY(hipEventRecord(ev->ev, s));
+    std::vector<PreFill> dropped;
+    {
+        std::lock_guard<std::mutex> lk(g_pre_mu);
+        g_pre_launches += launches;
+        for (int v = 0; v < nviews; ++v) {
+            PreFill f;
+            f.s = s; f.ev = ev;
+            pre_sig(f.sig, cams[v], g, radii[v]);
+            auto it = g_pre.find(geom[v]);
+            if (it != g_pre.end()) { dropped.push_back(std::move(it->second)); it->second = std::move(f); }
+            else g_pre.emplace(geom[v], std::move(f));
+        }
+    }
+    return GSR_OK;
+}
+
+int gsr_preprocess_release(const void *geom) {
+    PreFill f;
+    std::lock_guard<std::mutex> lk(g_pre_mu);
+    auto it = g_pre.find(geom);
+    if (it == g_pre.end()) return GSR_OK;
+    f = std::move(it->second);
+    g_pre.erase(it);
+    return GSR_OK;
+}
+
+int gsr_preprocess_stats(int *launches, int *consumed) {
+    std::lock_guard<std::mutex> lk(g_pre_mu);
+    if (launches) *launches = g_pre_launches;
+    if (consumed) *consumed = g_pre_consumed;
+    return GSR_OK;
+}
 
 int gsr_forward(const gsr_camera *cam, const gsr_gaussians *g, gsr_alloc_fn alloc, void *alloc_ctx,
                 float *out_color, float *out_depth, int *out_radii, int *out_num_rendered,
diff --git a/animating-gaussian-splats_amd/csrc/gsr_bind.cpp b/animating-gaussian-splats_amd/csrc/gsr_bind.cpp
--- a/animating-gaussian-splats_amd/csrc/gsr_bind.cpp
+++ b/animating-gaussian-splats_amd/csrc/gsr_bind.cpp
@@ -17,6 +17,7 @@
 struct Fns {
     decltype(&gsr_forward_info_call) forward_info_call = nullptr;
     decltype(&gsr_forward_async) forward_async = nullptr;
+    decltype(&gsr_preprocess_views) preprocess_views = nullptr;
     decltype(&gsr_backward_render) backward_render = nullptr;
     decltype(&gsr_backward_gaussians) backward_gaussians = nullptr;
     decltype(&gsr_backward) backward = nullptr;
@@ -39,6 +40,7 @@
 void set_functions(const std::map<std::string, int64_t> &a) {
     take(a, "gsr_forward_info_call", F.forward_info_call);
     take(a, "gsr_forward_async", F.forward_async);
+    take(a, "gsr_preprocess_views", F.preprocess_views);
     take(a, "gsr_backward_render", F.backward_render);
     take(a, "gsr_backward_gaussians", F.backward_gaussians);
     take(a, "gsr_backward", F.backward);
@@ -191,26 +193,47 @@
     }
 };
 
+void record(const at::Tensor &t, const c10::hip::HIPStream &s) {
+    if (t.defined() && t.is_cuda() && t.storage().data_ptr().get())
+        c10::hip::HIPCachingAllocator::recordStream(t.storage().data_ptr(), s);
+}
+
 void *raw_stream(at::Device dev) { return (void *)c10::hip::getCurrentHIPStream(dev.index()).stream(); }
 
 py::tuple forward(const at::Tensor &bg, const at::Tensor &means3D, const at::Tensor &colors, const at::Tensor &opacity,
                   const at::Tensor &scales, const at::Tensor &rotations, double scale_modifier, const at::Tensor &cov3D,
                   const at::Tensor &viewmatrix, const at::Tensor &projmatrix, double tanfovx, double tanfovy, int H, int W,
                   const at::Tensor &sh, int degree, const at::Tensor &campos, bool prefiltered, int activations,
-                  bool prepare_backward, bool speculate, bool nonblocking, bool prealloc) {
+                  bool prepare_backward, bool speculate, bool nonblocking, bool prealloc,
+                  const c10::optional<at::Tensor> &pre_geom, const c10::optional<at::Tensor> &pre_radii) {
     std::vector<at::Tensor> keep;
     gsr_gaussians g = gaussians(means3D, sh, degree, colors, opacity, scales, rotations, scale_modifier, cov3D,
                                 activations, prepare_backward, 0, keep);
     gsr_camera cam = camera(viewmatrix, projmatrix, tanfovx, tanfovy, H, W, campos, bg, prefiltered, keep);
     const at::Device dev = means3D.device();
     const int P = g.P;
+    const bool pre = pre_geom.has_value() && pre_radii.has_value() && P > 0;
     auto f32 = at::TensorOptions().dtype(at::kFloat).device(dev);
     at::Tensor color = at::empty({3, H, W}, f32), depth = at::empty({1, H, W}, f32);
-    at::Tensor radii = at::empty({P}, at::TensorOptions().dtype(at::kInt).device(dev));
+    at::Tensor radii = pre ? *pre_radii : at::empty({P}, at::TensorOptions().dtype(at::kInt).device(dev));
     c10::hip::HIPGuard guard(dev.index());
     const size_t spec = (speculate || nonblocking) && P ? F.spec_binning_bytes(P, W, H, prepare_backward ? 1 : 0) : 0;
     PreAlloc pa(dev);
-    pa.group({{GSR_BUF_GEOM, F.geom_bytes(P)}, {GSR_BUF_IMAGE, F.image_bytes(W, H, P)}}, prealloc);
+    if (pre) {
+        const size_t gb = F.geom_bytes(P);
+        if ((size_t)pre_geom->numel() < gb || pre_geom->scalar_type() != at::kByte || pre_radii->numel() != P ||
+            pre_radii->scalar_type() != at::kInt || pre_geom->device() != dev || pre_radii->device() != dev)
+            throw std::runtime_error("preprocessed view: GEOM / radii do not fit this forward's Gaussians");
+        const c10::hip::HIPStream cs = c10::hip::getCurrentHIPStream(dev.index());
+        record(*pre_geom, cs);
+        record(*pre_radii, cs);
+        pa.given[GSR_BUF_GEOM] = PreAlloc::Given{*pre_geom, 0, (int64_t)gb};
+        pa.pa.ptr[GSR_BUF_GEOM] = pre_geom->data_ptr();
+        pa.pa.bytes[GSR_BUF_GEOM] = gb;
+        pa.group({{GSR_BUF_IMAGE, F.image_bytes(W, H, P)}}, true);
+    } else {
+        pa.group({{GSR_BUF_GEOM, F.geom_bytes(P)}, {GSR_BUF_IMAGE, F.image_bytes(W, H, P)}}, prealloc);
+    }
     pa.group({{GSR_BUF_BINNING, spec}}, prealloc);
     pa.arm();
     gsr_forward_info fi;
@@ -228,6 +251,44 @@
     check(rc);
     return py::make_tuple(fi.num_rendered, fi.binning_layout, fi.speculated, (unsigned long long)fi.pending,
                           (int64_t)(intptr_t)fi.aux_stream, color, radii, depth, pa.result());
+}
+
+py::list preprocess_views(const py::list &cams, const at::Tensor &means3D, const at::Tensor &colors,
+                          const at::Tensor &opacity, const at::Tensor &scales, const at::Tensor &rotations,
+                          double scale_modifier, const at::Tensor &cov3D, const at::Tensor &sh, int degree,
+                          int activations) {
+    std::vector<at::Tensor> keep;
+    gsr_gaussians g = gaussians(means3D, sh, degree, colors, opacity, scales, rotations, scale_modifier, cov3D,
+                                activations, false, 0, keep);
+    const int nv = (int)cams.size(), P = g.P;
+    const at::Device dev = means3D.device();
+    c10::hip::HIPGuard guard(dev.index());
+    std::vector<gsr_camera> cs(nv);
+    std::vector<const gsr_camera *> cp(nv);
+    std::vector<void *> geom(nv);
+    std::vector<int *> rad(nv);
+    py::list out;
+    const int64_t gb = (int64_t)F.geom_bytes(P);
+    for (int k = 0; k < nv; ++k) {
+        const py::tuple c = cams[k].cast<py::tuple>();
+        cs[k] = camera(c[0].cast<at::Tensor>(), c[1].cast<at::Tensor>(), c[2].cast<double>(), c[3].cast<double>(),
+                       c[4].cast<int>(), c[5].cast<int>(), c[6].is_none() ? at::Tensor() : c[6].cast<at::Tensor>(),
+                       c[7].cast<at::Tensor>(), false, keep);
+        cp[k] = &cs[k];
+        at::Tensor gt = at::empty({std::max<int64_t>(gb, 1)}, at::TensorOptions().dtype(at::kByte).device(dev));
+        at::Tensor rt = at::empty({P}, at::TensorOptions().dtype(at::kInt).device(dev));
+        geom[k] = gt.data_ptr();
+        rad[k] = P ? rt.data_ptr<int>() : nullptr;
+        out.append(py::make_tuple(gt, rt));
+    }
+    void *s = raw_stream(dev);
+    int rc;
+    {
+        py::gil_scoped_release nogil;
+        rc = F.preprocess_views(nv, cp.data(), &g, geom.data(), rad.data(), s);
+    }
+    check(rc);
+    return out;
 }
 
 py::tuple backward_render(const at::Tensor &bg, const at::Tensor &means3D, const at::Tensor &radii,
@@ -306,11 +367,6 @@
                         (const void *)image, dpix.data_ptr<float>(), nullptr, F.prealloc_alloc, &pa.pa, &gr, s);
     }
     check(rc);
-}
-
-void record(const at::Tensor &t, const c10::hip::HIPStream &s) {
-    if (t.defined() && t.is_cuda() && t.storage().data_ptr().get())
-        c10::hip::HIPCachingAllocator::recordStream(t.storage().data_ptr(), s);
 }
 
 std::string dev_str(const at::Device &d) { return d.str(); }
@@ -386,6 +442,7 @@
     m.def("set_functions", &set_functions);
     m.def("abi_version", []() { return (int)GSR_ABI_VERSION; });
     m.def("forward", &forward);
+    m.def("preprocess_views", &preprocess_views);
     m.def("backward_render", &backward_render);
     m.def("backward_views", &backward_views);
     m.def("backward", &backward);
diff --git a/animating-gaussian-splats_amd/csrc/gsr_forward.hip b/animating-gaussian-splats_amd/csrc/gsr_forward.hip
--- a/animating-gaussian-splats_amd/csrc/gsr_forward.hip
+++ b/animating-gaussian-splats_amd/csrc/gsr_forward.hip
@@ -22,6 +22,63 @@
 #else
 #define GSR_EMIT_STAMP(k) do {} while (0)
 #endif
+
+template <typename ShPtr, typename Cov3, typename Opa>
+__device__ inline void preprocess_view(int i, int D, const float3 p, const float *__restrict__ colors_precomp, ShPtr sh,
+                                       const float *__restrict__ viewmatrix, const float *__restrict__ projmatrix,
+                                       const float *__restrict__ campos, CamStrides cs, int W, int H, float tan_fovx,
+                                       float tan_fovy, float focal_x, float focal_y, int gx, int gy,
+                                       int *__restrict__ radii, float *__restrict__ depth_out,
+                                       float4 *__restrict__ rec_out, uint2 *__restrict__ rect_out,
+                                       uint32_t *__restrict__ tiles_out, uint8_t *__restrict__ clamp_out, Cov3 cov3,
+                                       Opa opa) {
+    float vm[16], pm[16];
+    load_mat16(viewmatrix, cs.v0, cs.v1, vm);
+    load_mat16(projmatrix, cs.p0, cs.p1, pm);
+    radii[i] = 0;
+    tiles_out[i] = 0;
+    rect_out[i] = make_uint2(0, 0);
+    const float4 ph = xform4x4(p, pm);
+    const float3 pv = xform4x3(p, vm);
+    if (pv.z <= 0.2f) return;
+    const float pw = 1.0f / (ph.w + 0.0000001f);
+    const float ppx = ph.x * pw, ppy = ph.y * pw;
+    float c3[6];
+    cov3(c3);
+    const float3 cv = cov2d(p, focal_x, focal_y, tan_fovx, tan_fovy, c3, vm);
+    const float det = cv.x * cv.z - cv.y * cv.y;
+    if (det == 0.0f) return;
+    const float det_inv = 1.f / det;
+    const float mid = 0.5f * (cv.x + cv.z);
+    const float l1 = mid + sqrtf(fmaxf(0.1f, mid * mid - det));
+    const float l2 = mid - sqrtf(fmaxf(0.1f, mid * mid - det));
+    const float my_radius = ceilf(3.f * sqrtf(fmaxf(l1, l2)));
+    const float pix_x = ndc2pix(ppx, W), pix_y = ndc2pix(ppy, H);
+    int x0, y0, x1, y1;
+    get_rect(pix_x, pix_y, (int)my_radius, gx, gy, x0, y0, x1, y1);
+    if ((x1 - x0) * (y1 - y0) == 0) return;
+    float3 rgb;
+    if (colors_precomp) {
+        rgb = make_float3(colors_precomp[3 * i], colors_precomp[3 * i + 1], colors_precomp[3 * i + 2]);
+    } else {
+        bool cl[3];
+        const float3 cp = load_campos(campos, cs.c0);
+        rgb = sh_to_rgb(D, p, cp, sh, cl);
+        clamp_out[i] = clamp_bits(cl);
+    }
+    radii[i] = (int)my_radius;
+    depth_out[i] = pv.z;
+    const float o = opa();
+    const float ca = cv.z * det_inv, cb = -cv.y * det_inv, cc = cv.x * det_inv;
+    const float tau2 = o >= 1.0f / 255.0f ? 2.f * log2f(255.f * o) : -1.f;
+    float4 *r = rec_out + (size_t)kRecF4 * i;
+    r[0] = make_float4(pix_x, pix_y, -0.5f * GSR_LOG2E * ca, -GSR_LOG2E * cb);
+    r[1] = make_float4(-0.5f * GSR_LOG2E * cc, o, pv.z, tau2);
+    r[2] = make_float4(rgb.x, rgb.y, rgb.z, pv.z);
+    r[3] = make_float4(ca, cb, cc, 0.f);
+    rect_out[i] = pack_rect(x0, y0, x1, y1);
+    tiles_out[i] = (uint32_t)((y1 - y0) * (x1 - x0));
+}
 
 template <int MC>
 __global__ __launch_bounds__(256) void k_preprocess(
@@ -53,62 +110,79 @@
         __syncthreads();
     }
     if (i >= P) return;
-    float vm[16], pm[16];
-    load_mat16(viewmatrix, cs.v0, cs.v1, vm);
-    load_mat16(projmatrix, cs.p0, cs.p1, pm);
-    radii[i] = 0;
-    tiles_out[i] = 0;
-    rect_out[i] = make_uint2(0, 0);
-    const float4 ph = xform4x4(p, pm);
-    const float3 pv = xform4x3(p, vm);
-    if (pv.z <= 0.2f) return;
-    const float pw = 1.0f / (ph.w + 0.0000001f);
-    const float ppx = ph.x * pw, ppy = ph.y * pw;
-    float c3[6];
-    if (cov3D_precomp) {
-#pragma unroll
-        for (int k = 0; k < 6; ++k) c3[k] = cov3D_precomp[6 * i + k];
+    auto cov3 = [&](float (&c3)[6]) {
+        if (cov3D_precomp) {
+#pragma unroll
+            for (int k = 0; k < 6; ++k) c3[k] = cov3D_precomp[6 * i + k];
+        } else {
+            float3 s = s_in;
+            float4 q = q_in;
+            if (act & GSR_ACT_EXP_SCALES) s = act_exp3(s);
+            if (act & GSR_ACT_NORMALIZE_ROTATIONS) q = act_normalize(q, quat_norm(q));
+            cov3d_from_scale_rot(s, scale_modifier, q, c3);
+        }
+    };
+    auto opa = [&]() { return (act & GSR_ACT_SIGMOID_OPACITY) ? act_sigmoid(o_in) : o_in; };
+    if constexpr (MC > 0)
+        preprocess_view(i, D, p, colors_precomp, (const float *)(s_sh + threadIdx.x * RS), viewmatrix, projmatrix, campos,
+                        cs, W, H, tan_fovx, tan_fovy, focal_x, focal_y, gx, gy, radii, depth_out, rec_out, rect_out,
+                        tiles_out, clamp_out, cov3, opa);
+    else
+        preprocess_view(i, D, p, colors_precomp, shs + (size_t)i * M * 3, viewmatrix, projmatrix, campos, cs, W, H,
+                        tan_fovx, tan_fovy, focal_x, focal_y, gx, gy, radii, depth_out, rec_out, rect_out, tiles_out,
+                        clamp_out, cov3, opa);
+}
+
+template <int MC>
+__global__ __launch_bounds__(kShBlock) void k_preprocess_multi(const PreMultiArgs a) {
+    extern __shared__ __attribute__((aligned(16))) float s_sh[];
+    constexpr int RL = 3 * MC, RS = sh_row_stride(MC);
+    const int P = a.P;
+    const int i0 = blockIdx.x * kShBlock;
+    const int i = i0 + threadIdx.x;
+    const int ic = min(i, P - 1);
+    const float3 p = make_float3(a.means3D[3 * ic], a.means3D[3 * ic + 1], a.means3D[3 * ic + 2]);
+    float3 s_in = make_float3(0.f, 0.f, 0.f);
+    float4 q_in = make_float4(0.f, 0.f, 0.f, 0.f);
+    float c3v[6] = {0.f, 0.f, 0.f, 0.f, 0.f, 0.f};
+    if (a.cov3D_precomp) {
+#pragma unroll
+        for (int k = 0; k < 6; ++k) c3v[k] = a.cov3D_precomp[6 * ic + k];
     } else {
+        s_in = make_float3(a.scales[3 * ic], a.scales[3 * ic + 1], a.scales[3 * ic + 2]);
+        q_in = make_float4(a.rotations[4 * ic], a.rotations[4 * ic + 1], a.rotations[4 * ic + 2], a.rotations[4 * ic + 3]);
+    }
+    const float o_in = a.opacities[ic];
+    if constexpr (MC > 0) {
+        sh_rows_to_lds<MC>(a.shs + (size_t)i0 * RL, min(kShBlock, P - i0), s_sh);
+        __syncthreads();
+    }
+    if (i >= P) return;
+    if (!a.cov3D_precomp) {
         float3 s = s_in;
         float4 q = q_in;
-        if (act & GSR_ACT_EXP_SCALES) s = act_exp3(s);
-        if (act & GSR_ACT_NORMALIZE_ROTATIONS) q = act_normalize(q, quat_norm(q));
-        cov3d_from_scale_rot(s, scale_modifier, q, c3);
-    }
-    const float3 cv = cov2d(p, focal_x, focal_y, tan_fovx, tan_fovy, c3, vm);
-    const float det = cv.x * cv.z - cv.y * cv.y;
-    if (det == 0.0f) return;
-    const float det_inv = 1.f / det;
-    const float mid = 0.5f * (cv.x + cv.z);
-    const float l1 = mid + sqrtf(fmaxf(0.1f, mid * mid - det));
-    const float l2 = mid - sqrtf(fmaxf(0.1f, mid * mid - det));
-    const float my_radius = ceilf(3.f * sqrtf(fmaxf(l1, l2)));
-    const float pix_x = ndc2pix(ppx, W), pix_y = ndc2pix(ppy, H);
-    int x0, y0, x1, y1;
-    get_rect(pix_x, pix_y, (int)my_radius, gx, gy, x0, y0, x1, y1);
-    if ((x1 - x0) * (y1 - y0) == 0) return;
-    float3 rgb;
-    if (colors_precomp) {
-        rgb = make_float3(colors_precomp[3 * i], colors_precomp[3 * i + 1], colors_precomp[3 * i + 2]);
-    } else {
-        bool cl[3];
-        const float3 cp = load_campos(campos, cs.c0);
-        if (MC > 0) rgb = sh_to_rgb(D, p, cp, s_sh + threadIdx.x * RS, cl);
-        else rgb = sh_to_rgb(D, p, cp, shs + (size_t)i * M * 3, cl);
-        clamp_out[i] = clamp_bits(cl);
-    }
-    radii[i] = (int)my_radius;
-    depth_out[i] = pv.z;
-    const float o = (act & GSR_ACT_SIGMOID_OPACITY) ? act_sigmoid(o_in) : o_in;
-    const float ca = cv.z * det_inv, cb = -cv.y * det_inv, cc = cv.x * det_inv;
-    const float tau2 = o >= 1.0f / 255.0f ? 2.f * log2f(255.f * o) : -1.f;
-    float4 *r = rec_out + (size_t)kRecF4 * i;
-    r[0] = make_float4(pix_x, pix_y, -0.5f * GSR_LOG2E * ca, -GSR_LOG2E * cb);
-    r[1] = make_float4(-0.5f * GSR_LOG2E * cc, o, pv.z, tau2);
-    r[2] = make_float4(rgb.x, rgb.y, rgb.z, pv.z);
-    r[3] = make_float4(ca, cb, cc, 0.f);
-    rect_out[i] = pack_rect(x0, y0, x1, y1);
-    tiles_out[i] = (uint32_t)((y1 - y0) * (x1 - x0));
+        if (a.act & GSR_ACT_EXP_SCALES) s = act_exp3(s);
+        if (a.act & GSR_ACT_NORMALIZE_ROTATIONS) q = act_normalize(q, quat_norm(q));
+        cov3d_from_scale_rot(s, a.scale_modifier, q, c3v);
+    }
+    const float o_act = (a.act & GSR_ACT_SIGMOID_OPACITY) ? act_sigmoid(o_in) : o_in;
+    auto cov3 = [&](float (&c3)[6]) {
+#pragma unroll
+        for (int k = 0; k < 6; ++k) c3[k] = c3v[k];
+    };
+    auto opa = [&]() { return o_act; };
+#pragma unroll 1
+    for (int t = 0; t < a.nv; ++t) {
+        const PreView &V = a.v[t];
+        if constexpr (MC > 0)
+            preprocess_view(i, a.D, p, a.colors_precomp, (const float *)(s_sh + threadIdx.x * RS), V.viewmatrix,
+                            V.projmatrix, V.campos, V.cs, V.W, V.H, V.tan_fovx, V.tan_fovy, V.focal_x, V.focal_y, V.gx,
+                            V.gy, V.radii, V.depth, V.rec, V.rect, V.tiles, V.clampm, cov3, opa);
+        else
+            preprocess_view(i, a.D, p, a.colors_precomp, a.shs + (size_t)i * a.M * 3, V.viewmatrix, V.projmatrix,
+                            V.campos, V.cs, V.W, V.H, V.tan_fovx, V.tan_fovy, V.focal_x, V.focal_y, V.gx, V.gy, V.radii,
+                            V.depth, V.rec, V.rect, V.tiles, V.clampm, cov3, opa);
+    }
 }
 
 template <bool USE_LDS>
@@ -1089,6 +1163,24 @@
     return hipGetLastError();
 }
 
+template <int MC>
+static void preprocess_multi_mc(const PreMultiArgs &a, hipStream_t s) {
+    k_preprocess_multi<MC><<<div_up(a.P, kShBlock), kShBlock, sizeof(float) * kShBlock * (MC ? sh_row_stride(MC) : 0), s>>>(a);
+}
+
+hipError_t launch_preprocess_multi(const PreMultiArgs &a, hipStream_t s) {
+    if (a.P == 0 || a.nv == 0) return hipSuccess;
+    const int mc = a.shs ? a.M : 0;
+    switch (mc) {
+        case 16: preprocess_multi_mc<16>(a, s); break;
+        case 9: preprocess_multi_mc<9>(a, s); break;
+        case 4: preprocess_multi_mc<4>(a, s); break;
+        case 1: preprocess_multi_mc<1>(a, s); break;
+        default: preprocess_multi_mc<0>(a, s); break;
+    }
+    return hipGetLastError();
+}
+
 hipError_t launch_bin_count(const FwdArgs &a, hipStream_t s) {
     const BinGrid bg(a.v.P);
     const int T = a.v.gx * a.v.gy;
diff --git a/animating-gaussian-splats_amd/csrc/gsr_internal.h b/animating-gaussian-splats_amd/csrc/gsr_internal.h
--- a/animating-gaussian-splats_amd/csrc/gsr_internal.h
+++ b/animating-gaussian-splats_amd/csrc/gsr_internal.h
@@ -89,6 +89,21 @@
 };
 hipError_t launch_gauss_bwd_multi(const MultiArgs &a, hipStream_t s);
 
+struct PreView {
+    const float *viewmatrix, *projmatrix, *campos;
+    CamStrides cs;
+    int W, H, gx, gy;
+    float tan_fovx, tan_fovy, focal_x, focal_y;
+    int *radii; float *depth; float4 *rec; uint2 *rect; uint32_t *tiles; uint8_t *clampm;
+};
+struct PreMultiArgs {
+    int P, D, M, nv, act;
+    float scale_modifier;
+    const float *means3D, *scales, *rotations, *opacities, *shs, *colors_precomp, *cov3D_precomp;
+    PreView v[kMultiViews];
+};
+hipError_t launch_preprocess_multi(const PreMultiArgs &a, hipStream_t s);
+
 struct SsimWindow { float w[11]; };
 size_t ssim_partials(int planes, int H, int W);
 hipError_t launch_ssim_fwd(int planes, int H, int W, const float *img1, const float *img2, const SsimWindow &w,
diff --git a/animating-gaussian-splats_amd/diff_gaussian_rasterization/_C.py b/animating-gaussian-splats_amd/diff_gaussian_rasterization/_C.py
--- a/animating-gaussian-splats_amd/diff_gaussian_rasterization/_C.py
+++ b/animating-gaussian-splats_amd/diff_gaussian_rasterization/_C.py
@@ -22,6 +22,7 @@
     "gsr_forward_async", "gsr_forward_resolve", "gsr_forward_release", "gsr_forward_query", "gsr_async_stats",
     "gsr_spec_keys", "gsr_async_shutdown", "gsr_debug_async_fault", "gsr_set_exact_thresholds",
     "gsr_knn", "gsr_rigidity_scratch_bytes", "gsr_rigidity_forward", "gsr_rigidity_backward",
+    "gsr_preprocess_views", "gsr_preprocess_release", "gsr_preprocess_stats",
 )
 
 
@@ -101,6 +102,13 @@
     L.gsr_forward_async.restype = i
     L.gsr_forward_async.argtypes = [ctypes.POINTER(_Camera), ctypes.POINTER(_Gaussians), _ALLOC_FN, vp,
                                     vp, vp, vp, ctypes.POINTER(_ForwardInfo), vp]
+    L.gsr_preprocess_views.restype = i
+    L.gsr_preprocess_views.argtypes = [i, ctypes.POINTER(ctypes.POINTER(_Camera)), ctypes.POINTER(_Gaussians),
+                                       ctypes.POINTER(vp), ctypes.POINTER(vp), vp]
+    L.gsr_preprocess_release.restype = i
+    L.gsr_preprocess_release.argtypes = [vp]
+    L.gsr_preprocess_stats.restype = i
+    L.gsr_preprocess_stats.argtypes = [ctypes.POINTER(i), ctypes.POINTER(i)]
     L.gsr_forward_resolve.restype = i
     L.gsr_forward_resolve.argtypes = [ctypes.c_ulonglong, ctypes.POINTER(_Resolution)]
     L.gsr_forward_release.restype = i
@@ -228,10 +236,14 @@
 
 class _PreAllocator:
 
-    def __init__(self, device, groups):
+    def __init__(self, device, groups, fixed=None):
         self.device = device
         self.pa = _Prealloc()
         self.given = {}
+        for which, (buf, nbytes) in (fixed or {}).items():
+            self.given[which] = (buf, 0, int(nbytes))
+            self.pa.ptr[which] = buf.data_ptr()
+            self.pa.bytes[which] = int(nbytes)
         for group in groups if _PREALLOC_ON else ():
             offs, total = [], 0
             for which, nbytes in group:
@@ -324,7 +336,7 @@
                 return None
             m.set_functions({n: ctypes.cast(L[n], ctypes.c_void_p).value for n in (
                 "gsr_forward_info_call", "gsr_forward_async", "gsr_backward_render", "gsr_backward_gaussians",
-                "gsr_backward", "gsr_prealloc_alloc",
+                "gsr_backward", "gsr_prealloc_alloc", "gsr_preprocess_views",
                 "gsr_spec_binning_bytes", "gsr_geom_bytes", "gsr_image_bytes", "gsr_scratch_bytes",
                 "gsr_sums_bytes", "gsr_last_error")})
             _native_mod = m
@@ -464,11 +476,11 @@
 def rasterize_gaussians(background, means3D, colors, opacity, scales, rotations, scale_modifier,
                         cov3D_precomp, viewmatrix, projmatrix, tan_fovx, tan_fovy, image_height,
                         image_width, sh, degree, campos, prefiltered, debug=False, activations=0,
-                        prepare_backward=False, speculate=False, info=None, nonblocking=False):
+                        prepare_backward=False, speculate=False, info=None, nonblocking=False, pre=None):
     fi, color, radii, depth, alloc, pending = _forward(
         background, means3D, colors, opacity, scales, rotations, scale_modifier, cov3D_precomp, viewmatrix,
         projmatrix, tan_fovx, tan_fovy, image_height, image_width, sh, degree, campos, prefiltered, activations,
-        prepare_backward, speculate, nonblocking)
+        prepare_backward, speculate, nonblocking, pre)
     if info is not None:
         info.update(num_rendered=fi.num_rendered, binning_layout=fi.binning_layout, speculated=bool(fi.speculated),
                     pending=pending)
@@ -478,8 +490,14 @@
 
 def _forward(background, means3D, colors, opacity, scales, rotations, scale_modifier, cov3D_precomp, viewmatrix,
              projmatrix, tan_fovx, tan_fovy, image_height, image_width, sh, degree, campos, prefiltered, activations,
-             prepare_backward, speculate, nonblocking):
+             prepare_backward, speculate, nonblocking, pre=None):
     L = load_library()
+    pg = pr = None
+    if pre is not None:
+        pre.claim(_pre_key((means3D, colors, opacity, scales, rotations, cov3D_precomp, sh), scale_modifier, degree,
+                           activations), _pre_cam_key(viewmatrix, projmatrix, tan_fovx, tan_fovy, image_height,
+                                                      image_width, campos))
+        pg, pr = pre.geom, pre.radii
     nat = _native() if _NATIVE_PARTS & 1 else None
     if nat is not None:
         e = _EMPTY
@@ -489,21 +507,21 @@
             e if rotations is None else rotations, float(scale_modifier), e if cov3D_precomp is None else cov3D_precomp,
             viewmatrix, projmatrix, float(tan_fovx), float(tan_fovy), int(image_height), int(image_width),
             e if sh is None else sh, int(degree), e if campos is None else campos, bool(prefiltered),
-            int(activations), bool(prepare_backward), bool(speculate), bool(nonblocking), _PREALLOC_ON)
+            int(activations), bool(prepare_backward), bool(speculate), bool(nonblocking), _PREALLOC_ON, pg, pr)
         fi = _ForwardInfo(K, layout, spec, pend, aux or None)
         alloc = _NativeAlloc(res)
     else:
         fi, color, radii, depth, alloc = _forward_ctypes(
             L, background, means3D, colors, opacity, scales, rotations, scale_modifier, cov3D_precomp, viewmatrix,
             projmatrix, tan_fovx, tan_fovy, image_height, image_width, sh, degree, campos, prefiltered, activations,
-            prepare_backward, speculate, nonblocking)
+            prepare_backward, speculate, nonblocking, pg, pr)
     pending = AsyncForward(fi.pending) if fi.pending else None
     return fi, color, radii, depth, alloc, pending
 
 
 def _forward_ctypes(L, background, means3D, colors, opacity, scales, rotations, scale_modifier, cov3D_precomp,
                     viewmatrix, projmatrix, tan_fovx, tan_fovy, image_height, image_width, sh, degree, campos,
-                    prefiltered, activations, prepare_backward, speculate, nonblocking):
+                    prefiltered, activations, prepare_backward, speculate, nonblocking, pre_geom=None, pre_radii=None):
     keep = []
     g, P, _ = _gaussians(means3D, sh, degree, colors, opacity, scales, rotations, scale_modifier,
                          cov3D_precomp, keep, activations, prepare_backward)
@@ -513,12 +531,20 @@
     H, W = int(image_height), int(image_width)
     color = torch.empty((3, H, W), dtype=torch.float32, device=dev)
     depth = torch.empty((1, H, W), dtype=torch.float32, device=dev)
-    radii = torch.empty((P,), dtype=torch.int32, device=dev)
+    shared = pre_geom is not None and P > 0
+    radii = pre_radii if shared else torch.empty((P,), dtype=torch.int32, device=dev)
     fi = _ForwardInfo(0, 0, 0)
     with _device_guard(dev):
         spec = L.gsr_spec_binning_bytes(P, W, H, int(bool(prepare_backward))) if (speculate or nonblocking) and P else 0
-        alloc = _PreAllocator(dev, [[(GSR_BUF_GEOM, L.gsr_geom_bytes(P)), (GSR_BUF_IMAGE, L.gsr_image_bytes(W, H, P))],
-                                    [(GSR_BUF_BINNING, spec)]])
+        if shared:
+            cs = torch.cuda.current_stream(dev)
+            pre_geom.record_stream(cs)
+            pre_radii.record_stream(cs)
+            alloc = _PreAllocator(dev, [[(GSR_BUF_IMAGE, L.gsr_image_bytes(W, H, P))], [(GSR_BUF_BINNING, spec)]],
+                                  fixed={GSR_BUF_GEOM: (pre_geom, L.gsr_geom_bytes(P))})
+        else:
+            alloc = _PreAllocator(dev, [[(GSR_BUF_GEOM, L.gsr_geom_bytes(P)), (GSR_BUF_IMAGE, L.gsr_image_bytes(W, H, P))],
+                                        [(GSR_BUF_BINNING, spec)]])
         with alloc:
             if nonblocking:
                 _check(L.gsr_forward_async(ctypes.byref(cam), ctypes.byref(g), alloc.cb, alloc.ctx, color.data_ptr(),
@@ -529,6 +555,81 @@
                                                color.data_ptr(), depth.data_ptr(), radii.data_ptr() if P else None,
                                                int(bool(speculate)), ctypes.byref(fi), _stream_ptr(dev)))
     return fi, color, radii, depth, alloc
+
+
+def _pre_key(tensors, scale_modifier, degree, activations):
+    k = [(0,) if t is None or t.numel() == 0 else
+         (t.data_ptr(), tuple(t.shape), tuple(t.stride()), t.dtype, t._version) for t in tensors]
+    return tuple(k) + (float(scale_modifier), int(degree), int(activations))
+
+
+def _pre_cam_key(viewmatrix, projmatrix, tan_fovx, tan_fovy, image_height, image_width, campos):
+    c = (0, 0) if campos is None or campos.numel() == 0 else (campos.data_ptr(), campos._version)
+    return (viewmatrix.data_ptr(), viewmatrix._version, projmatrix.data_ptr(), projmatrix._version, c,
+            float(tan_fovx), float(tan_fovy), int(image_height), int(image_width))
+
+
+class PreprocessedView:
+    __slots__ = ("geom", "radii", "key", "cam_key", "consumed")
+
+    def __init__(self, geom, radii, key, cam_key):
+        self.geom, self.radii, self.key, self.cam_key, self.consumed = geom, radii, key, cam_key, False
+
+    def matches(self, key, cam_key=None):
+        return not self.consumed and key == self.key and (cam_key is None or cam_key == self.cam_key)
+
+    def claim(self, key, cam_key):
+        if self.consumed:
+            raise RuntimeError("preprocessed view: already consumed by a forward (one forward per handle)")
+        if key != self.key or cam_key != self.cam_key:
+            raise RuntimeError("preprocessed view: the forward's inputs are not the tensors, values and camera it "
+                               "was preprocessed from (stale geometry is refused); call preprocess_views again")
+        self.consumed = True
+
+    def release(self):
+        if _lib is not None and self.geom is not None:
+            _lib.gsr_preprocess_release(self.geom.data_ptr())
+
+    def __del__(self):
+        self.release()
+
+
+def preprocess_stats():
+    a, b = ctypes.c_int(0), ctypes.c_int(0)
+    _check(load_library().gsr_preprocess_stats(ctypes.byref(a), ctypes.byref(b)))
+    return a.value, b.value
+
+
+def preprocess_views(cameras, means3D, colors, opacity, scales, rotations, scale_modifier, cov3D_precomp, sh,
+                     degree, activations=0):
+    L = load_library()
+    if means3D.ndimension() != 2 or means3D.size(1) != 3:
+        raise RuntimeError("means3D must have dimensions (num_points, 3)")
+    dev = means3D.device
+    key = _pre_key((means3D, colors, opacity, scales, rotations, cov3D_precomp, sh), scale_modifier, degree, activations)
+    cam_keys = [_pre_cam_key(c[0], c[1], c[2], c[3], c[4], c[5], c[6]) for c in cameras]
+    nat = _native() if _NATIVE_PARTS & 1 else None
+    if nat is not None:
+        e = _EMPTY
+        bufs = nat.preprocess_views(
+            [tuple(c) for c in cameras], means3D, e if colors is None else colors, e if opacity is None else opacity,
+            e if scales is None else scales, e if rotations is None else rotations, float(scale_modifier),
+            e if cov3D_precomp is None else cov3D_precomp, e if sh is None else sh, int(degree), int(activations))
+    else:
+        keep = []
+        g, P, _ = _gaussians(means3D, sh, degree, colors, opacity, scales, rotations, scale_modifier, cov3D_precomp,
+                             keep, activations)
+        cams = [_camera(c[0], c[1], c[2], c[3], c[4], c[5], c[6], c[7], False, keep) for c in cameras]
+        n = len(cams)
+        gb = L.gsr_geom_bytes(P)
+        bufs = [(torch.empty(max(gb, 1), dtype=torch.uint8, device=dev), torch.empty((P,), dtype=torch.int32, device=dev))
+                for _ in range(n)]
+        cp = (ctypes.POINTER(_Camera) * n)(*[ctypes.pointer(c) for c in cams])
+        gp = (ctypes.c_void_p * n)(*[b[0].data_ptr() for b in bufs])
+        rp = (ctypes.c_void_p * n)(*[b[1].data_ptr() if P else None for b in bufs])
+        with _device_guard(dev):
+            _check(L.gsr_preprocess_views(n, cp, ctypes.byref(g), gp, rp, _stream_ptr(dev)))
+    return [PreprocessedView(gt, rt, key, ck) for (gt, rt), ck in zip(bufs, cam_keys)]
 
 
 _EXT_STREAMS = {}
diff --git a/animating-gaussian-splats_amd/diff_gaussian_rasterization/__init__.py b/animating-gaussian-splats_amd/diff_gaussian_rasterization/__init__.py
--- a/animating-gaussian-splats_amd/diff_gaussian_rasterization/__init__.py
+++ b/animating-gaussian-splats_amd/diff_gaussian_rasterization/__init__.py
@@ -13,7 +13,7 @@
 
 __all__ = ["GaussianRasterizationSettings", "GaussianRasterizer", "rasterize_gaussians",
            "rasterize_parameters", "set_deferred_backward", "set_speculative_forward", "set_async_forward", "async_forward", "set_exact_thresholds",
-           "pending_views", "clear_pending"]
+           "pending_views", "clear_pending", "preprocess_views", "use_preprocessed"]
 
 
 class GaussianRasterizationSettings(NamedTuple):
@@ -148,6 +148,43 @@
 def _async_on():
     o = getattr(_async_tls, "on", None)
     return _defer["async"] if o is None else o
+
+
+_pre_tls = threading.local()
+
+
+def preprocess_views(raster_settings_list, means3D, opacities, shs=None, colors_precomp=None, scales=None,
+                     rotations=None, cov3D_precomp=None, activations=0):
+    rs0 = raster_settings_list[0]
+    for rs in raster_settings_list:
+        if rs.scale_modifier != rs0.scale_modifier or rs.sh_degree != rs0.sh_degree:
+            raise ValueError("preprocess_views: the views must share scale_modifier and sh_degree")
+    cams = [(rs.viewmatrix, rs.projmatrix, rs.tanfovx, rs.tanfovy, rs.image_height, rs.image_width, rs.campos, rs.bg)
+            for rs in raster_settings_list]
+    return _C.preprocess_views(cams, means3D, colors_precomp, opacities, scales, rotations, rs0.scale_modifier,
+                               cov3D_precomp, shs, rs0.sh_degree, activations)
+
+
+class use_preprocessed:
+
+    def __init__(self, handle):
+        self.handle = handle
+
+    def __enter__(self):
+        self.prev = getattr(_pre_tls, "handle", None)
+        _pre_tls.handle = self.handle
+        return self
+
+    def __exit__(self, *exc):
+        _pre_tls.handle = self.prev
+        return False
+
+
+def _take_preprocessed():
+    h = getattr(_pre_tls, "handle", None)
+    if h is not None:
+        _pre_tls.handle = None
+    return h
 
 
 def _buffer_ptrs(alloc):
@@ -327,7 +364,7 @@
                 rs.image_height, rs.image_width, sh, rs.sh_degree, rs.campos, rs.prefiltered)
         ctx.prep = bool(grad_mode) and any(ctx.needs_input_grad)
         fi, color, radii, depth, alloc, pending = _C._forward(
-            *args, 0, ctx.prep, _defer["speculate"], _async_on())
+            *args, 0, ctx.prep, _defer["speculate"], _async_on(), _take_preprocessed())
         ctx.raster_settings = rs
         ctx.num_rendered = fi.num_rendered
         ctx.binning_layout = fi.binning_layout
@@ -437,7 +474,8 @@
         fi, color, radii, depth, alloc, pending = _C._forward(
             rs.bg, means, colors, opacity_logits, log_scales, quaternions, rs.scale_modifier, empty,
             rs.viewmatrix, rs.projmatrix, rs.tanfovx, rs.tanfovy, rs.image_height, rs.image_width, sh,
-            rs.sh_degree, rs.campos, rs.prefiltered, _C.ACT_ALL, ctx.prep, _defer["speculate"], _async_on())
+            rs.sh_degree, rs.campos, rs.prefiltered, _C.ACT_ALL, ctx.prep, _defer["speculate"], _async_on(),
+            _take_preprocessed())
         ctx.raster_settings = rs
         ctx.num_rendered = fi.num_rendered
         ctx.binning_layout = fi.binning_layout
diff --git a/animating-gaussian-splats_amd/splat_step.py b/animating-gaussian-splats_amd/splat_step.py
--- a/animating-gaussian-splats_amd/splat_step.py
+++ b/animating-gaussian-splats_amd/splat_step.py
@@ -7,12 +7,20 @@
 
 import torch
 
-from diff_gaussian_rasterization import GaussianRasterizer, async_forward
+from diff_gaussian_rasterization import GaussianRasterizer, _C, async_forward, preprocess_views, use_preprocessed
+
+_SHARED = ("means3D", "opacities", "shs", "colors_precomp", "scales", "rotations", "cov3D_precomp")
+
+
+def _shared_key(inputs, rs):
+    return _C._pre_key(tuple(inputs.get(k) for k in ("means3D", "colors_precomp", "opacities", "scales", "rotations",
+                                                     "cov3D_precomp", "shs")), rs.scale_modifier, rs.sh_degree, 0)
 
 
 class RenderStep:
     def __init__(self, device, cams: Sequence, inputs_of: Callable, dl: torch.Tensor, streams: Sequence,
-                 threads: bool = True, shape: str = "summed", rotate: bool | None = None):
+                 threads: bool = True, shape: str = "summed", rotate: bool | None = None,
+                 share: bool | None = None):
         if shape not in ("summed", "per_view"):
             raise ValueError(f"shape: 'summed' or 'per_view', got {shape!r}")
         self.device, self.cams, self.inputs_of, self.dl = device, cams, inputs_of, dl
@@ -20,6 +28,9 @@
         self.shape = shape
         self.rotate = os.environ.get("GSR_STREAM_ROTATE", "1") != "0" if rotate is None else rotate
         self.calls = 0
+        self.share = os.environ.get("GSR_SHARED_PREPROCESS", "1") != "0" if share is None else share
+        self.share_rule = share is None
+        self.shared_calls = 0
         self.pool = ([ThreadPoolExecutor(max_workers=1) for _ in self.streams]
                      if threads and len(self.streams) > 1 else None)
 
@@ -29,10 +40,37 @@
                 ex.shutdown()
             self.pool = None
 
-    def _forwards(self, vs, s):
+    def _render(self, ci, inputs=None, handle=None):
+        if inputs is None:
+            inputs = self.inputs_of(ci)
+        rs = self.cams[ci]
+        if handle is not None and not handle.matches(_shared_key(inputs, rs)):
+            handle = None
+        with use_preprocessed(handle):
+            return GaussianRasterizer(raster_settings=rs)(**inputs)[0]
+
+    def _share(self, views, s0):
+        with torch.cuda.stream(s0):
+            first = self.inputs_of(views[0])
+            ts = [first.get(k) for k in _SHARED]
+            if not all(t is None or (isinstance(t, torch.Tensor) and t.is_leaf) for t in ts):
+                self.share = False
+                return None, None
+            if self.share_rule and first.get("shs") is None:
+                self.share = False
+                return first, None
+            rs = [self.cams[ci] for ci in views]
+            if any(r.scale_modifier != rs[0].scale_modifier or r.sh_degree != rs[0].sh_degree for r in rs):
+                return first, None
+            handles = preprocess_views(rs, first["means3D"], first["opacities"], **{k: first.get(k) for k in _SHARED[2:]})
+        self.shared_calls += 1
+        return first, handles
+
+    def _forwards(self, vs, s, first=None, handles=None):
         torch.cuda.set_device(self.device)
         with torch.cuda.stream(s):
-            return [GaussianRasterizer(raster_settings=self.cams[ci])(**self.inputs_of(ci))[0] for ci in vs]
+            return [self._render(ci, first if k == 0 else None, handles[k] if handles else None)
+                    for k, ci in enumerate(vs)]
 
     def _fwd_bwd(self, vs, s):
         torch.cuda.set_device(self.device)
@@ -48,12 +86,22 @@
         self.calls += 1
         streams = self.streams[off:ns] + self.streams[:off] if ns > 1 else self.streams[:1]
         with async_forward(True) if pool is None and ns > 1 else _nullcontext():
-            return self._run(views, ns, pool, streams)
+            return self._run(views, ns, pool, streams, self.share and not solo)
 
-    def _run(self, views, ns, pool, streams):
+    def _run(self, views, ns, pool, streams, share=False):
         if self.shape == "summed":
+            first = handles = None
+            if share and len(views) > 1:
+                prev_dev = torch.cuda.current_device()
+                torch.cuda.set_device(self.device)
+                try:
+                    first, handles = self._share(views, streams[0])
+                finally:
+                    torch.cuda.set_device(prev_dev)
             if pool is not None:
-                futs = [pool[self.streams.index(streams[k])].submit(self._forwards, views[k::ns], streams[k])
+                futs = [pool[self.streams.index(streams[k])].submit(
+                            self._forwards, views[k::ns], streams[k], first if k == 0 else None,
+                            handles[k::ns] if handles else None)
                         for k in range(min(ns, len(views)))]
                 imgs = [None] * len(views)
                 for k, f in enumerate(futs):
@@ -66,7 +114,7 @@
                 try:
                     for k, ci in enumerate(views):
                         torch.cuda.set_stream(streams[k % ns])
-                        imgs.append(GaussianRasterizer(raster_settings=self.cams[ci])(**self.inputs_of(ci))[0])
+                        imgs.append(self._render(ci, first if k == 0 else None, handles[k] if handles else None))
                 finally:
                     torch.cuda.set_stream(cur)
                     torch.cuda.set_device(prev_dev)
diff --git a/include/gsr.h b/include/gsr.h
--- a/include/gsr.h
+++ b/include/gsr.h
@@ -132,6 +132,11 @@
 int gsr_backward_gaussians(int nviews, const gsr_view_grad *views, const gsr_gaussians *g, gsr_grads *out,
                            void *stream);
 
+int gsr_preprocess_views(int nviews, const gsr_camera *const *cams, const gsr_gaussians *g, void *const *geom,
+                         int *const *radii, void *stream);
+int gsr_preprocess_release(const void *geom);
+int gsr_preprocess_stats(int *launches, int *consumed);
+
 int gsr_grad_fence(const void *const *grads, int n, void *stream);
 
 int gsr_mark_visible(int P, const float *means3D, const float *viewmatrix, const float *projmatrix,
```

Measured after the change: 1421 Msplats/s (median of 3 runs). About the same (+0.0%).
